# osmr/pytorchcv

Measured on AMD Instinct MI355X. Metric: images/sec @224x224 (resnet50 bs=256/GPU), higher is better.
Workload: dtype bf16; 1 GPU; resnet50_bs256; per_gpu_batch=256, global_batch=256, input=fp32 NCHW 224x224 resident in HBM, parallelism=batch-sharded replicas x1, launcher_choice=timed at capture on this GPU

## Files before the change

include/pcv_amd.h:

```cpp
#ifndef PCV_AMD_H
#define PCV_AMD_H

#include <stddef.h>
#include <stdint.h>

#ifdef __cplusplus
extern "C" {
#endif

#define PCV_ABI_VERSION 5

typedef struct pcv_ctx pcv_ctx;

typedef enum pcv_status {
    PCV_OK = 0,
    PCV_ERR_INVALID = -1,
    PCV_ERR_HIP = -2,
    PCV_ERR_NO_DEVICE = -3,
    PCV_ERR_TOO_LARGE = -4
} pcv_status;

typedef enum pcv_dtype { PCV_F32 = 0, PCV_BF16 = 1, PCV_F16 = 2 } pcv_dtype;

typedef enum pcv_act {
    PCV_ACT_NONE = 0, PCV_ACT_RELU = 1, PCV_ACT_RELU6 = 2, PCV_ACT_SIGMOID = 3,
    PCV_ACT_SWISH = 4, PCV_ACT_HSIGMOID = 5, PCV_ACT_HSWISH = 6
} pcv_act;

typedef struct pcv_conv_desc {
    int32_t struct_size;
    int32_t N, H, W;
    int32_t Cin, Cout;
    int32_t kh, kw;
    int32_t stride_h, stride_w;
    int32_t pad_t, pad_l, pad_b, pad_r;
    int32_t dil_h, dil_w;
    int32_t groups;
    int32_t act;
    int32_t post_act;
    int32_t has_residual;
    int32_t dtype;
    int32_t out_dtype;
    int32_t x_cpitch;
    int32_t x_wpitch;
    int32_t y_cpitch;
} pcv_conv_desc;

int pcv_abi_version(void);
size_t pcv_conv_desc_size(void);
int pcv_create(pcv_ctx** out, int device);
int pcv_destroy(pcv_ctx* ctx);
const char* pcv_last_error(const pcv_ctx* ctx);
int pcv_set_tuning(pcv_ctx* ctx, const char* key, int value);

int pcv_fp16_guard_begin(pcv_ctx* ctx, unsigned* slot, void* stream);
int pcv_fp16_guard_end(pcv_ctx* ctx, const unsigned* slot, float* y, long count, void* stream);
int pcv_fp16_overflow_count(pcv_ctx* ctx, unsigned* count, void* stream);

int pcv_nchw_to_nhwc(pcv_ctx* ctx, const float* x, void* y, int N, int C, int H, int W,
                     int cpitch, int wpitch, int dtype, void* stream);
int pcv_nhwc_to_nchw(pcv_ctx* ctx, const void* x, float* y, int N, int C, int H, int W, int cpitch, int dtype,
                     void* stream);

int pcv_preprocess_u8(pcv_ctx* ctx, const unsigned char* x, void* y, int N, int Hs, int Ws, int C, int top, int left,
                      int H, int W, int wpitch, const float* mean, const float* inv_std, int dtype, void* stream);

int pcv_conv_packed_bytes(const pcv_conv_desc* d, size_t* bytes);
int pcv_conv_pack(pcv_ctx* ctx, const pcv_conv_desc* d, const float* w, void* packed, void* stream);
int pcv_dwconv_packed_bytes(const pcv_conv_desc* d, size_t* bytes);
int pcv_dwconv_pack(pcv_ctx* ctx, const pcv_conv_desc* d, const float* w, void* packed, void* stream);
int pcv_bn_fold(pcv_ctx* ctx, int C, const float* gamma, const float* beta, const float* mean, const float* var,
                float eps, const float* conv_bias, float* scale, float* shift, void* stream);

int pcv_conv2d_fused(pcv_ctx* ctx, const pcv_conv_desc* d, const void* x, const void* packed,
                     const float* scale, const float* shift, const void* residual, void* y, void* stream);

int pcv_conv2d_gated_fused(pcv_ctx* ctx, const pcv_conv_desc* d, const void* x, const void* packed, const float* scale,
                           const float* shift, const float* gate, const void* residual, void* y, void* stream);
int pcv_fc_f32(pcv_ctx* ctx, const float* in, const float* w, const float* b, float* out, int N, int K, int J, int act,
               void* stream);
int pcv_conv2d_maxpool_supported(const pcv_conv_desc* d, int k, int s, int p, int ceil_mode);
int pcv_conv2d_maxpool_fused(pcv_ctx* ctx, const pcv_conv_desc* d, const void* x, const void* packed, const float* scale,
                             const float* shift, void* y, int k, int s, int p, int ceil_mode, void* stream);

int pcv_conv2d_nchw_stem_supported(const pcv_conv_desc* d, int pool);
int pcv_conv2d_nchw_stem_fused(pcv_ctx* ctx, const pcv_conv_desc* d, const float* x_nchw, const void* packed, const float* scale,
                               const float* shift, void* y, int pool, void* stream);
int pcv_dwconv2d_fused(pcv_ctx* ctx, const pcv_conv_desc* d, const void* x, const void* packed,
                       const float* scale, const float* shift, const void* residual, void* y, void* stream);
int pcv_maxpool2d(pcv_ctx* ctx, const void* x, void* y, int N, int H, int W, int C, int k, int s, int p,
                  int ceil_mode, int dtype, void* stream);
int pcv_channel_slice(pcv_ctx* ctx, const void* x, void* y, long rows, int C, int offset, int x_cpitch, int y_cpitch,
                      int dtype, void* stream);
int pcv_channel_interleave2(pcv_ctx* ctx, const void* a, const void* b, void* y, long rows, int Ch, int a_cpitch,
                            int b_cpitch, int y_cpitch, int dtype, void* stream);
int pcv_channel_concat(pcv_ctx* ctx, const void* x, void* y, long rows, int C, int x_cpitch, int y_cpitch, int y_offset,
                       int dtype, void* stream);
// ... 58 lines not shown
```

pytorchcv_amd/_lib.py:

```python

__all__ = ['lib', 'ctx_for', 'check', 'ConvDesc', 'LIB_PATH', 'PcvError', 'PCV_ERR_TOO_LARGE']

import os
import ctypes
import threading

LIB_PATH = os.path.join(os.path.dirname(os.path.abspath(__file__)), "csrc", "libpcv_amd.so")
PCV_ERR_TOO_LARGE = -4

_c = ctypes
_VP = ctypes.c_void_p
_I = ctypes.c_int


class PcvError(RuntimeError):
    def __init__(self, code, msg):
        super(PcvError, self).__init__("pcv_amd error {}: {}".format(code, msg))
        self.code = code


PCV_ABI_VERSION = 5


class ConvDesc(ctypes.Structure):
    _fields_ = [(n, ctypes.c_int32) for n in (
        "struct_size", "N", "H", "W", "Cin", "Cout", "kh", "kw", "stride_h", "stride_w", "pad_t", "pad_l", "pad_b", "pad_r",
        "dil_h", "dil_w", "groups", "act", "post_act", "has_residual", "dtype", "out_dtype", "x_cpitch", "x_wpitch",
        "y_cpitch")]


    def __init__(self, *args, **kw):
        super(ConvDesc, self).__init__(*args, **kw)
        self.struct_size = ctypes.sizeof(ConvDesc)


_SIGS = {
    "pcv_abi_version": (_I, []),
    "pcv_conv_desc_size": (ctypes.c_size_t, []),
    "pcv_create": (_I, [ctypes.POINTER(_VP), _I]),
    "pcv_destroy": (_I, [_VP]),
    "pcv_last_error": (ctypes.c_char_p, [_VP]),
    "pcv_set_tuning": (_I, [_VP, ctypes.c_char_p, _I]),
    "pcv_fp16_guard_begin": (_I, [_VP, _VP, _VP]),
    "pcv_fp16_guard_end": (_I, [_VP, _VP, _VP, ctypes.c_long, _VP]),
    "pcv_fp16_overflow_count": (_I, [_VP, ctypes.POINTER(ctypes.c_uint), _VP]),
    "pcv_rccl_available": (_I, []),
    "pcv_rccl_broadcast": (_I, [_VP, _VP, ctypes.POINTER(_VP), ctypes.POINTER(ctypes.c_size_t), _I, _I, _VP]),
    "pcv_rccl_allgather": (_I, [_VP, _VP, _VP, _VP, ctypes.c_size_t, _VP]),
    "pcv_nchw_to_nhwc": (_I, [_VP, _VP, _VP, _I, _I, _I, _I, _I, _I, _I, _VP]),
    "pcv_nhwc_to_nchw": (_I, [_VP, _VP, _VP, _I, _I, _I, _I, _I, _I, _VP]),
    "pcv_preprocess_u8": (_I, [_VP, _VP, _VP, _I, _I, _I, _I, _I, _I, _I, _I, _I, _VP, _VP, _I, _VP]),
    "pcv_conv_packed_bytes": (_I, [ctypes.POINTER(ConvDesc), ctypes.POINTER(ctypes.c_size_t)]),
    "pcv_conv_pack": (_I, [_VP, ctypes.POINTER(ConvDesc), _VP, _VP, _VP]),
    "pcv_dwconv_packed_bytes": (_I, [ctypes.POINTER(ConvDesc), ctypes.POINTER(ctypes.c_size_t)]),
    "pcv_dwconv_pack": (_I, [_VP, ctypes.POINTER(ConvDesc), _VP, _VP, _VP]),
    "pcv_bn_fold": (_I, [_VP, _I, _VP, _VP, _VP, _VP, ctypes.c_float, _VP, _VP, _VP, _VP]),
    "pcv_conv2d_fused": (_I, [_VP, ctypes.POINTER(ConvDesc), _VP, _VP, _VP, _VP, _VP, _VP, _VP]),
    "pcv_dwconv2d_fused": (_I, [_VP, ctypes.POINTER(ConvDesc), _VP, _VP, _VP, _VP, _VP, _VP, _VP]),
    "pcv_maxpool2d": (_I, [_VP, _VP, _VP, _I, _I, _I, _I, _I, _I, _I, _I, _I, _VP]),
    "pcv_channel_slice": (_I, [_VP, _VP, _VP, ctypes.c_long, _I, _I, _I, _I, _I, _VP]),
    "pcv_channel_interleave2": (_I, [_VP, _VP, _VP, _VP, ctypes.c_long, _I, _I, _I, _I, _I, _VP]),
    "pcv_channel_concat": (_I, [_VP, _VP, _VP, ctypes.c_long, _I, _I, _I, _I, _I, _VP]),
    "pcv_interpolate": (_I, [_VP, _VP, _VP, _I, _I, _I, _I, _I, _I, _I, _I, _I, _VP]),
    "pcv_avgpool2d": (_I, [_VP, _VP, _VP, _I, _I, _I, _I, _I, _I, _I, _I, _VP]),
    "pcv_global_avgpool": (_I, [_VP, _VP, _VP, _I, _I, _I, _I, _I, _VP]),
    "pcv_gemm_bias": (_I, [_VP, _VP, _VP, _VP, _VP, _I, _I, _I, _I, _I, _VP]),
    "pcv_se_squeeze": (_I, [_VP, _VP, _VP, _I, _I, _I, _I, _VP]),
    "pcv_se_excite": (_I, [_VP, _VP, _VP, _VP, _VP, _VP, _VP, _VP, _I, _I, _I, _I, _I, _VP]),
    "pcv_conv2d_gated_fused": (_I, [_VP, ctypes.POINTER(ConvDesc), _VP, _VP, _VP, _VP, _VP, _VP, _VP, _VP]),
    "pcv_fc_f32": (_I, [_VP, _VP, _VP, _VP, _VP, _I, _I, _I, _I, _VP]),
    "pcv_conv2d_maxpool_supported": (_I, [ctypes.POINTER(ConvDesc), _I, _I, _I, _I]),
    "pcv_conv2d_maxpool_fused": (_I, [_VP, ctypes.POINTER(ConvDesc), _VP, _VP, _VP, _VP, _VP, _I, _I, _I, _I, _VP]),
    "pcv_conv2d_nchw_stem_supported": (_I, [ctypes.POINTER(ConvDesc), _I]),
    "pcv_conv2d_nchw_stem_fused": (_I, [_VP, ctypes.POINTER(ConvDesc), _VP, _VP, _VP, _VP, _VP, _I, _VP]),
    "pcv_conv1x1_pair_supported": (_I, [ctypes.POINTER(ConvDesc), ctypes.POINTER(ConvDesc)]),
    "pcv_conv1x1_pair_fused": (_I, [_VP, ctypes.POINTER(ConvDesc), ctypes.POINTER(ConvDesc), _VP, _VP, _VP, _VP, _VP, _VP, _VP,
                                    _VP, _VP, _VP, _VP]),
    "pcv_conv1x1_pair_gated_supported": (_I, [ctypes.POINTER(ConvDesc), ctypes.POINTER(ConvDesc)]),
    "pcv_conv1x1_pair_gated_fused": (_I, [_VP, ctypes.POINTER(ConvDesc), ctypes.POINTER(ConvDesc), _VP, _VP, _VP, _VP, _VP, _VP, _VP,
                                          _VP, _VP, _VP, _VP, _VP]),
    "pcv_conv1x1_pair_idconv_supported": (_I, [ctypes.POINTER(ConvDesc), ctypes.POINTER(ConvDesc), ctypes.POINTER(ConvDesc)]),
# ... 65 lines not shown
```

pytorchcv_amd/csrc/d3q_conv.hpp:

```cpp
#pragma once
#include <type_traits>
#include "pcv_common.hpp"
#include "igemm_conv.hpp"

struct D3Params {
    const void* x;
    const void* w;
    const void* res;
    void* y;
    const float* scale;
    const float* shift;
    uint32_t x_bytes, w_bytes, y_bytes, res_bytes;
    int M;
    int Cout, Ypitch;
    int H, W, Cin, HW;
    FastDiv div_hw, div_w;
    int nk;
    int slices;
    int Kpad;
    int act, post_act;
    int nChTiles, nTiles;
    uint32_t* dbg;
    int stride, Hin, Win;
    uint32_t* ovf;
    int tailN;
    int dbgflags;
};

#ifdef PCV_DBG_FLAGS
#define D3_DBG(bits) ((p.dbgflags & (bits)) != 0)
#else
#define D3_DBG(bits) false
#endif
#ifdef D3X3_STAMPS
#define D3_STAMP(slot)                                                                                     \
    do {                                                                                                   \
        const int q__ = s - 4;                                                                             \
        if (q__ >= -1 && q__ < 27) {                                                                       \
            const int sel__ = (q__ + 9) % 9;                                                               \
            int l__ = -1;                                                                                  \
            if (q__ >= 0 && (slot) == sel__) l__ = 2 * q__ + 1;                                            \
            else if (q__ >= 0 && sel__ > 0 && (slot) == sel__ - 1) l__ = 2 * q__;                          \
            else if ((slot) == 8 && (q__ + 1) % 9 == 0 && q__ + 1 < 27) l__ = 2 * (q__ + 1);               \
            if (l__ >= 0) {                                                                                \
                const uint64_t t__ = __builtin_amdgcn_s_memtime();                                         \
                const int v__ = __builtin_amdgcn_readfirstlane((int)(uint32_t)t__);                        \
                const int i__ = __builtin_amdgcn_readfirstlane(l__);                                       \
                asm volatile("s_mov_b32 m0, %2\n\tv_writelane_b32 %0, %1, m0" : "+v"(stamps) : "s"(v__), "s"(i__) : "m0"); \
            }                                                                                              \
        }                                                                                                  \
    } while (0)
#else
#define D3_STAMP(slot) do { } while (0)
#endif

template <int WC, int WP, int CBW, int PBW, int KS, bool ONE = false> struct D3Cfg {
    static constexpr int NLOAD = 4;
    static constexpr int THREADS = 64 * (8 + NLOAD);
    static constexpr int BM = 16 * CBW * WC;
    static constexpr int BP = 16 * PBW * WP;
    static constexpr int NPA = BM / 8;
    static constexpr int WLW = NPA / NLOAD;
    static constexpr int BROWS = (BP + 2 + 7) / 8 * 8;
    static constexpr int NPB = BROWS / 8;
    static constexpr int XLW = (NPB + NLOAD - 1) / NLOAD;
    static constexpr int NB0 = (XLW + 1) / 2, NB1 = XLW / 2;
    static constexpr int ASZ = BM * 128;
    static constexpr int BSZ = NPB * 1024;
    static constexpr int NSA = 3;
    static constexpr int NSB = ONE ? 3 : 2;
    static constexpr int ZOFF = (NSA * ASZ + NSB * BSZ + 2047) / 2048 * 2048;
    static constexpr int DUMP = ZOFF + 2048;
    static constexpr int LDS = DUMP + 1024;
    static_assert(WC * WP == 8, "eight compute waves");
    static_assert(KS == 1 || KS == 2, "one or two K-halves per section");
    static_assert(NPA % NLOAD == 0 && CBW % 2 == 0, "weight pieces split evenly over the loaders; channel pairs per wave");
    static_assert(LDS <= 160 * 1024, "three weight tiles + two activation tiles must fit the LDS");
    static_assert(XLW <= 20, "row masks of the activation pieces are packed 3 bits each, ten per register, two registers");
};
// ... 285 lines not shown
            for (int j = 0; j < PBW; ++j) {
                lds_cptr bj = bp;
                if constexpr (Q != 1) {
                    const uint32_t t = (uint32_t)__builtin_amdgcn_sbfe((int)(Q == 0 ? hm0 : hm2), j, 1);
                    bj = (lds_cptr)(size_t)((t & (zsel - (uint32_t)(j * 2048))) | (~t & (uint32_t)(size_t)bp));
                }
                b[u][j] = *reinterpret_cast<lds_fptr>(bj + j * 2048);
            }
        }
    };
    auto mfmas = [&]() __attribute__((always_inline)) {
        __builtin_amdgcn_s_setprio(1);
#pragma unroll
        for (int u = 0; u < KS; ++u)
#pragma unroll
            for (int j = 0; j < PBW; ++j)
#pragma unroll
                for (int i = 0; i < CBW; ++i) acc[i][j] = Mma<DT>::run(a[u][i], b[u][j], acc[i][j]);
        __builtin_amdgcn_s_setprio(0);
    };
    auto reads_done = [&]() __attribute__((always_inline)) { __builtin_amdgcn_s_waitcnt(0xC07F); };

    const ActClamp act = make_act(p.act), pact = make_act(p.post_act);
    const bool has_res = p.res != nullptr;
    f32x4 es0[CBW / 2], es1[CBW / 2], eh0[CBW / 2], eh1[CBW / 2];
    auto ep_prefetch = [&](int t) __attribute__((always_inline)) {
        const int chTile = t % p.nChTiles;
#pragma unroll
        for (int ip = 0; ip < CBW / 2; ++ip) {
            const int ch0 = chTile * BM + wc * 16 * CBW + 32 * ip + 8 * fq;
            const int chl = ch0 < p.Cout ? ch0 : 0;
            es0[ip] = *reinterpret_cast<const f32x4*>(p.scale + chl); es1[ip] = *reinterpret_cast<const f32x4*>(p.scale + chl + 4);
            eh0[ip] = *reinterpret_cast<const f32x4*>(p.shift + chl); eh1[ip] = *reinterpret_cast<const f32x4*>(p.shift + chl + 4);
        }
    };
    auto epilogue = [&](int t) __attribute__((always_inline)) {
        if (D3_DBG(2)) return;
        const int chTile = t % p.nChTiles;
        const int tileP0 = (t / p.nChTiles) * BP;
        const int mBase = tileP0 + wp * 16 * PBW + fr;
        F16Guard<DT> guard;
#pragma unroll
        for (int ip = 0; ip < CBW / 2; ++ip) {
            const int ch0 = chTile * BM + wc * 16 * CBW + 32 * ip + 8 * fq;
            const bool chok = ch0 < p.Cout;
            const f32x4 s0 = es0[ip], s1 = es1[ip], h0 = eh0[ip], h1 = eh1[ip];
            u32x4 rr[PBW];
#pragma unroll
            for (int j = 0; j < PBW; ++j) rr[j] = (u32x4){0u, 0u, 0u, 0u};
            if (has_res) {
#pragma unroll
                for (int j = 0; j < PBW; ++j) {
                    const int m = mBase + 16 * j;
                    const uint32_t roff = (chok && m < p.M) ? (uint32_t)(((size_t)m * p.Cout + ch0) * 2) : 0x80000000u;
                    rr[j] = __builtin_amdgcn_raw_buffer_load_b128(rrsrc, roff, 0, 0);
                }
            }
#pragma unroll
            for (int j = 0; j < PBW; ++j) {
                const int m = mBase + 16 * j;
                float v[8];
#pragma unroll
                for (int e = 0; e < 4; ++e) {
                    v[e] = acc[2 * ip][j][e] * s0[e] + h0[e];
                    v[4 + e] = acc[2 * ip + 1][j][e] * s1[e] + h1[e];
                }
                clampn<8>(v, act);
#pragma unroll
                for (int e = 0; e < 4; ++e) {
                    float lo, hi;
                    unpack2<DT>(rr[j][e], lo, hi);
                    v[2 * e] += lo;
                    v[2 * e + 1] += hi;
                }
                clampn<8>(v, pact);
                guard.see(v);
                u32x4 o;
#pragma unroll
                for (int e = 0; e < 4; ++e) o[e] = pack2<DT>(v[2 * e], v[2 * e + 1]);
                const bool ok = chok && m < p.M && !D3_DBG(1);
                const uint32_t boff = ok ? (uint32_t)(((size_t)m * p.Ypitch + ch0) * 2) : 0x80000000u;
                __builtin_amdgcn_raw_buffer_store_b128(o, yrsrc, boff, 0, 0);
            }
        }
        guard.commit(p.ovf);
    };

    zero_acc();
    if constexpr (!ONE) setup_masks(T.tile0);
    d3q_sync();

    int sa = 0, sb = 0, k = 0, cur_tile = T.tile0, ep_tile = T.tile0;
    bool ep = false;
#ifdef D3X3_STAMPS
    int stamps = 0;
#endif
    auto kstep = [&](int s, auto Qc) __attribute__((always_inline)) -> bool {
        constexpr int Q = decltype(Qc)::value;
        if constexpr (GRP == 1) {
            if (s > 0) mfmas();
        }
        if constexpr (ONE || Q == 0) {
            if (ep) {
                epilogue(ep_tile);
                zero_acc();
                if constexpr (!ONE) {
                    if (!D3_DBG(8)) {
// ... 95 lines not shown
```

pytorchcv_amd/csrc/igemm_conv.hpp:

```cpp
#pragma once
#include "pcv_common.hpp"

#define IGEMM_MAX_TAPS 16

struct IgemmParams {
    const void* x;
    const void* w;
    const uint32_t* ktab;
    const void* res;
    void* y;
    const float* scale;
    const float* shift;
    uint32_t x_bytes;
    uint32_t w_bytes;
    uint32_t y_bytes;
    int M;
    int Cout;
    int Cout_total;
    int Ypitch;
    int cout_blk;
    int cin_blk;
    int wrows_blk;
    FastDiv div_howo, div_wo;
    int HoWo, Wo;
    int H, W, Wpitch, Cpitch;
    int sh, sw, pt, pl;
    int nR, nQ;
    int dy[IGEMM_MAX_TAPS];
    int dx[IGEMM_MAX_TAPS];
    int nk;
    int Kpad;
    int act, post_act;
    int nPixTiles, nChTiles;
    int ngb;
    int nTiles;
    int Cin;
    int ksteps_per_tap;
    int korder;
    int wstat;
    const float* gate;
    uint32_t* ovf;
};

template <int DT> struct Mma;
template <> struct Mma<PCV_BF16> {
    typedef s16x8 frag;
    static __device__ __forceinline__ f32x4 run(const frag& a, const frag& b, f32x4 c) {
        return __builtin_amdgcn_mfma_f32_16x16x32_bf16(a, b, c, 0, 0, 0);
    }
};
template <> struct Mma<PCV_F16> {
    typedef f16x8 frag;
    static __device__ __forceinline__ f32x4 run(const frag& a, const frag& b, f32x4 c) {
        return __builtin_amdgcn_mfma_f32_16x16x32_f16(a, b, c, 0, 0, 0);
    }
};
template <> struct Mma<PCV_F32> {
    typedef f32x4 frag;
    static __device__ __forceinline__ f32x4 run(const frag& a, const frag& b, f32x4 c) {
        c = __builtin_amdgcn_mfma_f32_16x16x4f32(a[0], b[0], c, 0, 0, 0);
        c = __builtin_amdgcn_mfma_f32_16x16x4f32(a[1], b[1], c, 0, 0, 0);
        c = __builtin_amdgcn_mfma_f32_16x16x4f32(a[2], b[2], c, 0, 0, 0);
        c = __builtin_amdgcn_mfma_f32_16x16x4f32(a[3], b[3], c, 0, 0, 0);
        return c;
    }
};

template <int DT, int OT, int CB, int PB, int WC, int WP, bool RAGGED, int KHW>
__global__ __launch_bounds__(64 * WC * WP, 2) void igemm_conv_kernel(const IgemmParams p) {
#if defined(__HIP_DEVICE_COMPILE__)
    constexpr int NW = WC * WP;
    constexpr int BM = 16 * CB * WC;
    constexpr int BP = 16 * PB * WP;
    constexpr int ES = Elem<DT>::BYTES;
    constexpr int CE = 16 / ES;
    constexpr int STAGE = (BM + BP) * 128;
    constexpr int WLOADS = BM / (8 * NW);
    constexpr int XLOADS = BP / (8 * NW);
    constexpr int NPAIR = CB / 2;
    static_assert(BM % (8 * NW) == 0 && BP % (8 * NW) == 0, "tile rows must split evenly over the waves");
    typedef typename Mma<DT>::frag frag;

    extern __shared__ __attribute__((aligned(16))) char smem[];

    const int tid = threadIdx.x;
    const int lane = tid & 63;
    const int wave = __builtin_amdgcn_readfirstlane(tid >> 6);
    const int wc = wave / WP, wp = wave % WP;

    const int perXcd = (p.nTiles + 7) >> 3;
    const int xcd = blockIdx.x & 7;
    const int tstride = gridDim.x >> 3;
    int tile = xcd * perXcd + (int)(blockIdx.x >> 3);
    const int tend = min(p.nTiles, (xcd + 1) * perXcd);
    if (tile >= tend) return;

    const int lrow = lane >> 3;
    const int cs = (lane & 7) ^ lrow;
    const int nR = KHW == 9 ? 3 : (KHW == 1 ? 1 : p.nR);
    const int nQ = KHW == 9 ? 3 : (KHW == 1 ? 1 : p.nQ);
    const int fr = lane & 15, fq = lane >> 4;

    struct TileState {
        int rbase[XLOADS];
        uint32_t rmask[XLOADS];
        uint32_t woff[WLOADS];
        int chTile, gb, tileP0;
    };
    auto setup = [&](int t, TileState& S) {
        S.chTile = t % p.nChTiles;
        const int t2 = t / p.nChTiles;
        S.gb = t2 % p.ngb;
        S.tileP0 = (t2 / p.ngb) * BP;
#pragma unroll
        for (int i = 0; i < XLOADS; ++i) {
            const int m = S.tileP0 + 8 * (i * NW + wave) + lrow;
            uint32_t mask = 0;
            int base = 0;
            if (m < p.M) {
                const uint32_t n = fastdiv((uint32_t)m, p.div_howo);
                const uint32_t rem = (uint32_t)m - n * (uint32_t)p.HoWo;
// ... 64 lines not shown
                q = (uint32_t)(k - 3 * grp);
                r = (uint32_t)(grp / p.ksteps_per_tap);
                cslice = grp - (int)r * p.ksteps_per_tap;
            }
            const int c0 = cslice * (8 * CE) + cs * CE;
            koff = ((int)r * p.Wpitch + (int)q) * p.Cpitch + c0;
        } else {
            const u32x2 kd = kd_next;
            const int c0 = (int)(kd[0] & 0xFFFFu);
            r = (kd[0] >> 16) & 15u;
            q = (kd[0] >> 20) & 15u;
            const int dy = (int)(short)(kd[1] & 0xFFFFu), dx = (int)(short)(kd[1] >> 16);
            koff = (dy * p.Wpitch + dx) * p.Cpitch + c0;
        }
#pragma unroll
        for (int i = 0; i < XLOADS; ++i) {
            char* dst = sbase + (BM + 8 * (i * NW + wave)) * 128;
            const bool ok = chunk_ok && (((S.rmask[i] >> r) & (S.rmask[i] >> (16 + q)) & 1u) != 0);
            const uint32_t voff = ok ? (uint32_t)((S.rbase[i] + koff) * ES) : 0x80000000u;
            __builtin_amdgcn_raw_ptr_buffer_load_lds(xrsrc, PCV_LDS(dst), 16, voff, 0, 0, 0);
        }
    };

    const int swz0 = ((fq) ^ (fr & 7)) << 4;
    const int swz1 = ((fq + 4) ^ (fr & 7)) << 4;
    const int wfrag = (wc * 16 * CB + fr) * 128;
    const int xfrag = (BM + wp * 16 * PB + fr) * 128;

    f32x4 acc[CB][PB];
    auto zero_acc = [&]() {
#pragma unroll
        for (int i = 0; i < CB; ++i)
#pragma unroll
            for (int j = 0; j < PB; ++j) acc[i][j] = (f32x4){0.f, 0.f, 0.f, 0.f};
    };
    auto compute = [&](int buf) {
        const char* sbase = smem + buf * STAGE;
        const char* wsbase = wstat ? smem : sbase;
#pragma unroll
        for (int kk = 0; kk < 2; ++kk) {
            const int swz = kk == 0 ? swz0 : swz1;
            frag a[CB], b[PB];
#pragma unroll
            for (int i = 0; i < CB; ++i) a[i] = *reinterpret_cast<const frag*>(wsbase + wfrag + i * 2048 + swz);
#pragma unroll
            for (int j = 0; j < PB; ++j) b[j] = *reinterpret_cast<const frag*>(sbase + xfrag + j * 2048 + swz);
#pragma unroll
            for (int i = 0; i < CB; ++i)
#pragma unroll
                for (int j = 0; j < PB; ++j) acc[i][j] = Mma<DT>::run(a[i], b[j], acc[i][j]);
        }
    };

    const ActClamp act = make_act(p.act), pact = make_act(p.post_act);
    const bool bounded = act_bounded(p.post_act) || (p.post_act == PCV_ACT_NONE && p.res == nullptr && p.gate == nullptr && act_bounded(p.act));
    zero_acc();
    TileState cur, nxt;
    setup(tile, cur);
    const int nk = p.nk;
    if constexpr (KHW == 0) kd_next = load_kdesc(0);
    stage(cur, 0, 0);
    if constexpr (KHW == 0) kd_next = load_kdesc(nk > 1 ? 1 : 0);
    int buf = 0;

    while (true) {
        for (int k = 0; k + 1 < nk; ++k) {
            asm volatile("s_waitcnt vmcnt(0)" ::: "memory");
            __syncthreads();
            stage(cur, k + 1, buf ^ 1);
            if constexpr (KHW == 0) kd_next = load_kdesc(k + 2 < nk ? k + 2 : 0);
            compute(buf);
            buf ^= 1;
        }
        const int ntile = tile + tstride;
        const bool has_next = ntile < tend;
        if (has_next) setup(ntile, nxt);
        asm volatile("s_waitcnt vmcnt(0)" ::: "memory");
        __syncthreads();

        const int chBlk = cur.chTile * BM + wc * 16 * CB;
        const int chGlob0 = cur.gb * p.cout_blk;
        const int mBase = cur.tileP0 + wp * 16 * PB + fr;
        float sc[NPAIR][8], sf[NPAIR][8];
        u32x4 rres[NPAIR][PB];
        f32x4 rres32[DT == PCV_F32 ? NPAIR : 1][DT == PCV_F32 ? PB : 1][2];
        if constexpr (!RAGGED) {
#pragma unroll
            for (int ip = 0; ip < NPAIR; ++ip) {
                const int ch0 = chBlk + 32 * ip + 8 * fq;
                const int chg = chGlob0 + ch0;
                f32x4 s0 = {1.f, 1.f, 1.f, 1.f}, s1 = s0, h0 = {0.f, 0.f, 0.f, 0.f}, h1 = h0;
                if (ch0 < p.Cout) {
                    if (p.scale != nullptr) {
                        s0 = *reinterpret_cast<const f32x4*>(p.scale + chg);
                        s1 = *reinterpret_cast<const f32x4*>(p.scale + chg + 4);
                    }
                    if (p.shift != nullptr) {
                        h0 = *reinterpret_cast<const f32x4*>(p.shift + chg);
                        h1 = *reinterpret_cast<const f32x4*>(p.shift + chg + 4);
                    }
                }
#pragma unroll
                for (int e = 0; e < 4; ++e) { sc[ip][e] = s0[e]; sc[ip][4 + e] = s1[e]; sf[ip][e] = h0[e]; sf[ip][4 + e] = h1[e]; }
#pragma unroll
                for (int j = 0; j < PB; ++j) {
                    const int m = mBase + 16 * j;
                    const bool ok = p.res != nullptr && ch0 < p.Cout && m < p.M;
                    const size_t eoff = (size_t)m * p.Cout_total + chg;
                    if constexpr (DT == PCV_F32) {
                        rres32[ip][j][0] = ok ? *reinterpret_cast<const f32x4*>(reinterpret_cast<const float*>(p.res) + eoff)
                                              : (f32x4){0.f, 0.f, 0.f, 0.f};
                        rres32[ip][j][1] = ok ? *reinterpret_cast<const f32x4*>(reinterpret_cast<const float*>(p.res) + eoff + 4)
                                              : (f32x4){0.f, 0.f, 0.f, 0.f};
                    } else {
                        rres[ip][j] = ok ? *reinterpret_cast<const u32x4*>(reinterpret_cast<const uint16_t*>(p.res) + eoff)
                                         : (u32x4){0u, 0u, 0u, 0u};
                    }
                }
            }
        }

        if (has_next) stage(nxt, 0, buf ^ 1);
        if constexpr (KHW == 0) kd_next = load_kdesc(nk > 1 ? 1 : 0);

        compute(buf);

        F16Guard<OT> guard;
#pragma unroll
        for (int ip = 0; ip < NPAIR; ++ip) {
            const int ch0 = chBlk + 32 * ip + 8 * fq;
            if constexpr (!FAST_STORE) {
                if (ch0 >= p.Cout) continue;
            }
            const int chg = chGlob0 + ch0;
            if constexpr (RAGGED) {
#pragma unroll
                for (int e = 0; e < 8; ++e) {
                    const bool ok = ch0 + e < p.Cout;
                    sc[ip][e] = ok ? (p.scale ? p.scale[chg + e] : 1.f) : 0.f;
                    sf[ip][e] = ok ? (p.shift ? p.shift[chg + e] : 0.f) : 0.f;
                }
            }
#pragma unroll
            for (int j = 0; j < PB; ++j) {
                const int m = mBase + 16 * j;
                if constexpr (!FAST_STORE) {
                    if (m >= p.M) continue;
                }
                const size_t eoff = (size_t)m * p.Cout_total + chg;
                const size_t yoff = (size_t)m * p.Ypitch + chg;
                float v[8];
#pragma unroll
                for (int e = 0; e < 4; ++e) {
                    v[e] = acc[2 * ip][j][e] * sc[ip][e] + sf[ip][e];
                    v[4 + e] = acc[2 * ip + 1][j][e] * sc[ip][4 + e] + sf[ip][4 + e];
                }
                apply_act8(v, act);
                if (p.gate != nullptr) {
#pragma clang fp contract(off)
                    const uint32_t n = fastdiv((uint32_t)(m < p.M ? m : 0), p.div_howo);
                    const float* gp = p.gate + (size_t)n * p.Cout_total + chg;
// ... 58 lines not shown
```

pytorchcv_amd/csrc/pcv_api.hip:

```cpp
#include <hip/hip_runtime.h>
#include <string>
#include <vector>
#include <cstring>
#include <algorithm>
#include <cstdio>
#include <cstdlib>
#include <dlfcn.h>
#include "pcv_common.hpp"
#include "igemm_inst.hpp"
#include "d3q_inst.hpp"
#include "d3w_inst.hpp"
#include "d3c_conv.hpp"
#include "d3k_conv.hpp"
#include "d3i_conv.hpp"
#include "d1i_conv.hpp"
#include "p1r_conv.hpp"
#include "stem_conv.hpp"
#include "pair1x1.hpp"
#include "wpair1x1.hpp"
#include "gconv3x3.hpp"
#include "gconv3x3r.hpp"
#include "mbconv.hpp"
#include "mbw_inst.hpp"
#include "mbr_inst.hpp"
// ... 22 lines not shown
D3WT_SHAPES(D3WT_DECLARE, PCV_BF16)
D3WT_SHAPES(D3WT_DECLARE, PCV_F16)
extern template __global__ void d3c_kernel<PCV_BF16>(const D3Params);
extern template __global__ void d3c_kernel<PCV_F16>(const D3Params);
extern template __global__ void d3k_kernel<PCV_BF16>(const D3Params);
extern template __global__ void d3k_kernel<PCV_F16>(const D3Params);
extern template __global__ void d3i_kernel<PCV_BF16, 256>(const D3Params);
extern template __global__ void d3i_kernel<PCV_F16, 256>(const D3Params);
extern template __global__ void d3i_kernel<PCV_BF16, 512>(const D3Params);
extern template __global__ void d3i_kernel<PCV_F16, 512>(const D3Params);
extern template __global__ void d1i_kernel<PCV_BF16, 1024>(const D3Params);
extern template __global__ void d1i_kernel<PCV_F16, 1024>(const D3Params);
extern template __global__ void d1i_kernel<PCV_BF16, 2048>(const D3Params);
extern template __global__ void d1i_kernel<PCV_F16, 2048>(const D3Params);
#define P1R_DECLARE(CW, CIN)                                                       \
    extern template __global__ void p1r_kernel<PCV_BF16, CW, CIN>(const D3Params); \
    extern template __global__ void p1r_kernel<PCV_F16, CW, CIN>(const D3Params);
P1R_DECLARE(64, 256)
P1R_DECLARE(32, 512)
P1R_DECLARE(32, 256)

enum TileCfg { TILE_C32 = 0, TILE_C64 = 1, TILE_C128 = 2, TILE_C256 = 3, TILE_C64S = 4, TILE_C128S = 5, TILE_COUNT = 6 };

struct pcv_ctx {
    int device = 0;
    std::string err;
    int num_cu = 256;
    int persist_mode = 1;
    int force_tile = -1;
    int use_wstat = 1;
    int use_mbr = 1;
    int use_mbr_xl = 1;
    int use_mbw = 1;
    int use_gconvr = 1;
    int use_d1x1 = -1;
    int use_head = 1;
    int use_stem32 = 1;
    int use_d3x3 = -1;
    unsigned long long dbg_ptr = 0;
    int use_p1r = -1;
    int use_d3k = -1;
    int use_d3i = -1;
    int use_d1i = -1;
    int use_d3c = -1;
    int use_d3w = -1;
    int dbg_flags = 0;
    int dw_flags = 0;
    int dw_th = 0;
    int max_blocks = 0;
    int pair_pb = 2;
    int persist_max_nk = 4;
    uint32_t* ovf = nullptr;
    int igemm_bpc[3][2][TILE_COUNT][3] = {};
    int gconv_bpc[3] = {2, 2, 2};
    int stem_bpc[2] = {1, 1};
    int pair_bpc[2] = {1, 1};
    int pair_idc_bpc = 1;
    int wpair_bpc[4] = {1, 1, 1, 1};
};

static thread_local std::string g_create_err;

static int fail(pcv_ctx* ctx, int code, const std::string& msg) {
    if (ctx) ctx->err = msg; else g_create_err = msg;
    return code;
}
#define HIP_TRY(ctx, expr)                                                                          \
    do {                                                                                            \
        hipError_t e__ = (expr);                                                                    \
        if (e__ != hipSuccess)                                                                      \
            return fail(ctx, PCV_ERR_HIP, std::string(#expr) + ": " + hipGetErrorString(e__));      \
    } while (0)

struct DeviceGuard {
    int prev = -1;
    bool switched = false;
    explicit DeviceGuard(int want) {
        if (hipGetDevice(&prev) == hipSuccess && prev != want) switched = hipSetDevice(want) == hipSuccess;
    }
    ~DeviceGuard() {
        if (switched) (void)hipSetDevice(prev);
    }
};

static inline int round_up(int v, int m) { return (v + m - 1) / m * m; }
static inline long long block_slots(const pcv_ctx* ctx, int per_cu) {
    const long long n = (long long)ctx->num_cu * per_cu;
    return (ctx->max_blocks > 0 && ctx->max_blocks < n) ? ctx->max_blocks : n;
}
static inline int esize(int dt) { return dt == PCV_F32 ? 4 : 2; }
static inline bool dtype_ok(int dt) { return dt == PCV_F32 || dt == PCV_BF16 || dt == PCV_F16; }
static inline bool aligned16(const void* p) { return (reinterpret_cast<uintptr_t>(p) & 15u) == 0; }
static inline bool in_window(unsigned long long bytes) { return bytes < 0x80000000ull; }
static int too_large(pcv_ctx* ctx, const char* fn, const char* what) {
    return fail(ctx, PCV_ERR_TOO_LARGE, std::string(fn) + ": " + what + " exceeds the 2 GiB window of one launch; split the batch");
}
static const char* const kTensorTooLarge = "tensor exceeds the 2 GiB window";

struct Kernel { const void* fn; int threads, lds, BM, BP; };
template <class F> static Kernel kernel_of(F* fn, int threads, int lds, int BM = 0, int BP = 0) {
    return Kernel{reinterpret_cast<const void*>(fn), threads, lds, BM, BP};
}
template <class Params> static int launch(pcv_ctx* ctx, const Kernel& k, unsigned grid, hipStream_t stream, Params& q) {
    void* args[] = {&q};
    HIP_TRY(ctx, hipLaunchKernel(k.fn, dim3(grid), dim3((unsigned)k.threads), args, (size_t)k.lds, stream));
    return PCV_OK;
}
static int blocks_per_cu(pcv_ctx* ctx, const Kernel& k, int* nb) {
    HIP_TRY(ctx, hipOccupancyMaxActiveBlocksPerMultiprocessor(nb, k.fn, k.threads, k.lds));
    if (*nb < 1) *nb = 1;
    return PCV_OK;
}

struct ConvPlan {
    bool stem = false;
    bool conv3 = false;
    int ES = 2, CE = 8;
    bool pair = false;
    int Ho = 0, Wo = 0;
    int ngb = 1;
    int Cg_in = 0, Cg_out = 0;
    int cin_blk = 0, cout_blk = 0;
    int nR = 1, nQ = 1;
    int dy[IGEMM_MAX_TAPS], dx[IGEMM_MAX_TAPS];
    int nchunks = 0, nk = 0, Kpad = 0;
    int wrows = 0;
    size_t ktab_bytes = 0, w_bytes = 0, total_bytes = 0;
    int gconv_kt = 5;
    bool gconv = false;
    bool d3i = false;
    bool d1i = false;
    size_t d3i_off = 0;
    size_t gconv_off = 0;
    std::vector<uint32_t> ktab;
    std::vector<uint32_t> ksrc;
};

static const char* const kStaleDesc = "pcv_conv_desc.struct_size does not match this library (stale binding: compare pcv_conv_desc_size() / PCV_ABI_VERSION)";
static inline bool desc_stale(const pcv_conv_desc& d) { return d.struct_size != (int32_t)sizeof(pcv_conv_desc); }

static const char* plan_conv(const pcv_conv_desc& d, ConvPlan& P, bool tables) {
    if (desc_stale(d)) return kStaleDesc;
    if (!dtype_ok(d.dtype) || !dtype_ok(d.out_dtype)) return "unknown dtype";
    if (d.out_dtype != d.dtype && d.out_dtype != PCV_F32) return "out_dtype must equal dtype or be fp32";
    if (d.Cin <= 0 || d.Cout <= 0 || d.kh <= 0 || d.kw <= 0 || d.groups <= 0) return "non-positive conv dimension";
    constexpr int kMaxChannels = 1 << 20, kMaxExtent = 1 << 24, kMaxGeom = 1 << 12;
    if (d.Cin > kMaxChannels || d.Cout > kMaxChannels || d.groups > kMaxChannels) return "channel count out of range (> 2^20)";
    if (d.N < 0 || d.H < 0 || d.W < 0 || d.N > kMaxExtent || d.H > kMaxExtent || d.W > kMaxExtent) return "N / H / W out of range (> 2^24)";
    if (d.stride_h > kMaxGeom || d.stride_w > kMaxGeom || d.dil_h > kMaxGeom || d.dil_w > kMaxGeom) return "stride / dilation out of range";
    if (d.pad_t < 0 || d.pad_l < 0 || d.pad_b < 0 || d.pad_r < 0 || d.pad_t > kMaxGeom || d.pad_l > kMaxGeom || d.pad_b > kMaxGeom ||
        d.pad_r > kMaxGeom)
        return "padding out of range";
    if (d.x_cpitch < 0 || d.x_cpitch > 8 * kMaxChannels || d.x_wpitch < 0 || d.x_wpitch > 2 * kMaxExtent || d.y_cpitch < 0 ||
        d.y_cpitch > 8 * kMaxChannels)
        return "pitch out of range";
    if (d.kh >= IGEMM_MAX_TAPS || d.kw >= IGEMM_MAX_TAPS) return "kernel size > 15 unsupported";
    if (d.stride_h <= 0 || d.stride_w <= 0 || d.dil_h <= 0 || d.dil_w <= 0) return "non-positive stride/dilation";
    if (d.Cin % d.groups || d.Cout % d.groups) return "channels not divisible by groups";
    P.ES = esize(d.dtype);
    P.CE = 16 / P.ES;
    P.Cg_in = d.Cin / d.groups;
    P.Cg_out = d.Cout / d.groups;
    const int cpitch = d.x_cpitch > 0 ? d.x_cpitch : d.Cin;
    if (cpitch < d.Cin) return "x_cpitch < Cin";
    P.pair = (d.groups == 1 && cpitch == 4 && P.ES == 2);
    if (!P.pair && cpitch % P.CE != 0) return "x_cpitch must be a multiple of 16 bytes (or 4 for a padded 16-bit stem)";

    int gpb = 1;
    if (d.groups > 1) {
        while (gpb < d.groups && ((gpb * P.Cg_out) % 8 != 0 || (gpb * P.Cg_in) % P.CE != 0 || gpb * P.Cg_out < 32)) ++gpb;
        while (gpb < d.groups && d.groups % gpb != 0) ++gpb;
        if (d.groups % gpb != 0 || (gpb * P.Cg_out) % 8 != 0 || (gpb * P.Cg_in) % P.CE != 0)
            return "unsupported group shape (channels per group block not 16-byte aligned)";
    }
    P.ngb = d.groups / gpb;
    P.cin_blk = gpb * P.Cg_in;
    P.cout_blk = gpb * P.Cg_out;
    if (d.groups == 1) P.cin_blk = d.Cin;
    P.wrows = round_up(P.cout_blk, 32);

    P.conv3 = d.groups == 1 && d.kh == 3 && d.kw == 3 && d.stride_h == 1 && d.stride_w == 1 && d.dil_h == 1 && d.dil_w == 1 &&
              d.pad_t == 1 && d.pad_l == 1 && d.pad_b == 1 && d.pad_r == 1 && d.Cin % (8 * P.CE) == 0 && cpitch == d.Cin &&
              (d.x_wpitch <= 0 || d.x_wpitch == d.W) && d.out_dtype == d.dtype && d.Cout % 8 == 0;

    P.stem = P.pair && d.stride_h == 2 && d.stride_w == 2 && d.dil_h == 1 && d.Cout <= 64 && d.Cout % 8 == 0 && d.kh <= 7 &&
             d.kw + (d.pad_l & 1) <= 8 && d.out_dtype == d.dtype;

    if (P.pair) {
        if (d.stride_w % 2 != 0 || d.dil_w != 1) return "padded 4-channel stem needs even stride_w and dilation 1";
        const int wp = d.x_wpitch > 0 ? d.x_wpitch : d.W;
        if (wp % 2 != 0) return "padded 4-channel stem needs an even x_wpitch";
        const int dxs = -(d.pad_l & 1);
        P.nQ = (d.kw - dxs + 1) / 2;
        P.nR = d.kh;
        if (P.nQ >= IGEMM_MAX_TAPS) return "stem too wide";
        for (int r = 0; r < P.nR; ++r) P.dy[r] = r * d.dil_h;
        for (int q = 0; q < P.nQ; ++q) P.dx[q] = dxs + 2 * q;
        P.nchunks = P.nR * P.nQ;
    } else {
        P.nR = d.kh;
        P.nQ = d.kw;
        for (int r = 0; r < P.nR; ++r) P.dy[r] = r * d.dil_h;
        for (int q = 0; q < P.nQ; ++q) P.dx[q] = q * d.dil_w;
        const int cchunks = (P.cin_blk + P.CE - 1) / P.CE;
        if (d.groups == 1 && cchunks * P.CE > cpitch) return "x_cpitch too small for the channel chunks";
        P.nchunks = P.nR * P.nQ * cchunks;
    }
    for (int i = P.nR; i < IGEMM_MAX_TAPS; ++i) P.dy[i] = 0;
    for (int i = P.nQ; i < IGEMM_MAX_TAPS; ++i) P.dx[i] = 0;
    P.nk = (P.nchunks + 7) / 8;
    P.Kpad = P.nk * 8 * P.CE;
    P.ktab_bytes = (size_t)round_up(P.nk * 8 * 8, 256);
    P.w_bytes = (size_t)P.ngb * P.wrows * P.Kpad * P.ES;
    P.total_bytes = P.ktab_bytes + P.w_bytes;
    static const bool gconv_on = !(std::getenv("PCV_AMD_GCONV") && std::atoi(std::getenv("PCV_AMD_GCONV")) == 0);
    P.gconv = gconv_on && d.groups > 1 && d.kh == 3 && d.kw == 3 && d.stride_h == d.stride_w && (d.stride_h == 1 || d.stride_h == 2) &&
              d.dil_h == 1 && d.dil_w == 1 &&
              d.pad_t == 1 && d.pad_l == 1 && d.pad_b == 1 && d.pad_r == 1 && d.Cin == d.Cout && d.Cin % 64 == 0 && P.ES == 2 &&
              (P.Cg_in == 4 || P.Cg_in == 8 || P.Cg_in == 16 || P.Cg_in == 32) && d.out_dtype == d.dtype;
    if (P.gconv) {
        P.gconv_kt = P.Cg_in == 32 ? 9 : 5;
        P.gconv_off = (P.total_bytes + 15) / 16 * 16;
        P.total_bytes = P.gconv_off + (size_t)(d.Cin / 16) * P.gconv_kt * 16 * 32 * P.ES;
    }
    P.d3i = P.conv3 && P.ES == 2 && (d.Cin == 256 || d.Cin == 512) && d.Cout % D3ICfg::CW == 0 && d.out_dtype == d.dtype &&
            P.wrows >= d.Cout && P.Kpad == 9 * d.Cin;
    if (P.d3i) {
        P.d3i_off = (P.total_bytes + 15) / 16 * 16;
        P.total_bytes = P.d3i_off + (size_t)(d.Cout / D3ICfg::CW) * (d.Cin == 256 ? D3ICfgT<256>::WBYTES : D3ICfgT<512>::WBYTES);
    }
    P.d1i = !P.conv3 && !P.pair && !P.stem && P.ES == 2 && d.kh == 1 && d.kw == 1 && d.groups == 1 && d.stride_h == 1 && d.stride_w == 1 &&
            d.pad_t == 0 && d.pad_l == 0 && d.pad_b == 0 && d.pad_r == 0 && (d.Cin == 1024 || d.Cin == 2048) &&
            d.Cout % 64 == 0 && d.out_dtype == d.dtype && P.wrows >= d.Cout && P.Kpad == d.Cin && P.ngb == 1;
    if (P.d1i) {
        P.d3i_off = (P.total_bytes + 15) / 16 * 16;
        P.total_bytes = P.d3i_off + (size_t)(d.Cout / 64) * (size_t)(d.Cin / 32) * 4096;
    }
    if (P.w_bytes >= 0x80000000ull) return "packed weights exceed 2 GiB";

    if (P.stem) {
        P.ktab_bytes = 0;
        P.w_bytes = (size_t)d.kh * 64 * 32 * P.ES;
        P.total_bytes = P.w_bytes;
    }
    P.Ho = (d.H + d.pad_t + d.pad_b - d.dil_h * (d.kh - 1) - 1) / d.stride_h + 1;
    P.Wo = (d.W + d.pad_l + d.pad_r - d.dil_w * (d.kw - 1) - 1) / d.stride_w + 1;

    if (tables) {
        P.ktab.assign((size_t)P.nk * 8 * 2, 0);
        P.ksrc.assign((size_t)P.Kpad, 0xFFFFFFFFu);
        const int khkw = d.kh * d.kw;
        (void)khkw;
        int j = 0;
        auto put = [&](int c0, int r, int q, int dyv, int dxv) {
            P.ktab[2 * j] = (uint32_t)c0 | ((uint32_t)r << 16) | ((uint32_t)q << 20);
            P.ktab[2 * j + 1] = ((uint32_t)dyv & 0xFFFFu) | (((uint32_t)dxv & 0xFFFFu) << 16);
            ++j;
        };
        if (P.pair) {
            for (int r = 0; r < P.nR; ++r)
                for (int q = 0; q < P.nQ; ++q) {
                    for (int e = 0; e < 8; ++e) {
                        const int pix = e >> 2, c = e & 3;
                        const int tap = P.dx[q] + pix;
                        if (tap >= 0 && tap < d.kw && c < d.Cin)
                            P.ksrc[(size_t)j * 8 + e] = (uint32_t)c | ((uint32_t)(r * d.kw + tap) << 16);
                    }
                    put(0, r, q, P.dy[r], P.dx[q]);
                }
        } else if (P.conv3) {
            const int slices = d.Cin / (8 * P.CE);
            for (int r = 0; r < 3; ++r)
                for (int cs = 0; cs < slices; ++cs)
                    for (int q = 0; q < 3; ++q)
                        for (int cc = cs * 8; cc < cs * 8 + 8; ++cc) {
                            for (int e = 0; e < P.CE; ++e)
                                P.ksrc[(size_t)j * P.CE + e] = (uint32_t)(cc * P.CE + e) | ((uint32_t)(r * 3 + q) << 16);
                            put(cc * P.CE, r, q, P.dy[r], P.dx[q]);
                        }
        } else {
            const int cchunks = (P.cin_blk + P.CE - 1) / P.CE;
            for (int r = 0; r < P.nR; ++r)
                for (int q = 0; q < P.nQ; ++q)
                    for (int cc = 0; cc < cchunks; ++cc) {
                        for (int e = 0; e < P.CE; ++e) {
                            const int c = cc * P.CE + e;
                            if (c < P.cin_blk)
                                P.ksrc[(size_t)j * P.CE + e] = (uint32_t)c | ((uint32_t)(r * d.kw + q) << 16);
                        }
                        put(cc * P.CE, r, q, P.dy[r], P.dx[q]);
                    }
        }
        while (j < P.nk * 8) put(0, 15, 0, 0, 0);
    }
    return nullptr;
}

struct TileInfo { int BM, BP, threads, lds; };
static const TileInfo kTiles[TILE_COUNT] = {
    {32, 256, 256, 2 * (32 + 256) * 128},
    {64, 256, 256, 2 * (64 + 256) * 128},
    {128, 128, 256, 2 * (128 + 128) * 128},
    {256, 64, 256, 2 * (256 + 64) * 128},
    {64, 128, 256, 2 * (64 + 128) * 128},
    {128, 64, 256, 2 * (128 + 64) * 128},
};
typedef void (*igemm_fn)(const IgemmParams);

template <int DT, int KHW> static igemm_fn igemm_for_tile(int tile) {
    switch (tile) {
        case TILE_C32: return igemm_conv_kernel<DT, DT, 2, 4, 1, 4, false, KHW>;
        case TILE_C64: return igemm_conv_kernel<DT, DT, 4, 4, 1, 4, false, KHW>;
        case TILE_C128: return igemm_conv_kernel<DT, DT, 4, 4, 2, 2, false, KHW>;
        case TILE_C256: return igemm_conv_kernel<DT, DT, 4, 4, 4, 1, false, KHW>;
        case TILE_C64S: if constexpr (KHW == 1) return igemm_conv_kernel<DT, DT, 4, 2, 1, 4, false, 1>; else return nullptr;
        case TILE_C128S: if constexpr (KHW == 1) return igemm_conv_kernel<DT, DT, 4, 2, 2, 2, false, 1>; else return nullptr;
        default: return nullptr;
    }
}
template <int DT> static igemm_fn igemm_for_taps(int tile, int khw) {
    if (khw == 1) return igemm_for_tile<DT, 1>(tile);
    if (khw == 9) return igemm_for_tile<DT, 9>(tile);
    return igemm_for_tile<DT, 0>(tile);
}
static igemm_fn igemm_fn_for(int dt, int ot, bool ragged, int tile, int khw) {
    if (!ragged && ot == dt) {
        if (dt == PCV_BF16) return igemm_for_taps<PCV_BF16>(tile, khw);
        if (dt == PCV_F16) return igemm_for_taps<PCV_F16>(tile, khw);
        return igemm_for_taps<PCV_F32>(tile, khw);
    }
    if (tile != TILE_C128) return nullptr;
    if (ot == PCV_F32) {
        if (dt == PCV_BF16) return igemm_conv_kernel<PCV_BF16, PCV_F32, 4, 4, 2, 2, true, 0>;
        if (dt == PCV_F16) return igemm_conv_kernel<PCV_F16, PCV_F32, 4, 4, 2, 2, true, 0>;
        return igemm_conv_kernel<PCV_F32, PCV_F32, 4, 4, 2, 2, true, 0>;
    }
    if (dt == PCV_BF16) return igemm_conv_kernel<PCV_BF16, PCV_BF16, 4, 4, 2, 2, true, 0>;
    if (dt == PCV_F16) return igemm_conv_kernel<PCV_F16, PCV_F16, 4, 4, 2, 2, true, 0>;
    return nullptr;
}

static Kernel igemm_kernel(int dt, int ot, bool ragged, int tile, int khw) {
    const TileInfo& T = kTiles[tile];
    return kernel_of(igemm_fn_for(dt, ot, ragged, tile, khw), T.threads, T.lds, T.BM, T.BP);
}
static inline int khw_slot(int khw) { return khw == 1 ? 1 : (khw == 9 ? 2 : 0); }

static inline int gconv_slot(int W) { return W + 1 <= 16 ? 0 : (W + 1 <= 32 ? 1 : 2); }
static Kernel gconv_kernel(int dt, int slot) {
    const bool bf = dt == PCV_BF16;
    if (slot == 0) return kernel_of(bf ? gconv3x3_kernel<PCV_BF16, 16> : gconv3x3_kernel<PCV_F16, 16>, 256, GConvCfg<16>::LDS);
    if (slot == 1) return kernel_of(bf ? gconv3x3_kernel<PCV_BF16, 32> : gconv3x3_kernel<PCV_F16, 32>, 256, GConvCfg<32>::LDS);
    return kernel_of(bf ? gconv3x3_kernel<PCV_BF16, 64> : gconv3x3_kernel<PCV_F16, 64>, 256, GConvCfg<64>::LDS);
}
static const int kGconvRMaxLds = 160 * 1024;
static Kernel gconvr_kernel(int dt, int stride, int kt, int lds = kGconvRMaxLds) {
    const bool bf = dt == PCV_BF16;
    if (stride == 2) {
        if (kt == 9) return kernel_of(bf ? gconv3x3r_kernel<PCV_BF16, 2, 9> : gconv3x3r_kernel<PCV_F16, 2, 9>, 256, lds);
        return kernel_of(bf ? gconv3x3r_kernel<PCV_BF16, 2, 5> : gconv3x3r_kernel<PCV_F16, 2, 5>, 256, lds);
    }
    return kernel_of(bf ? gconv3x3r_kernel<PCV_BF16, 1, 9> : gconv3x3r_kernel<PCV_F16, 1, 9>, 256, lds);
}
struct GConvRPlan { int R, XH, xl, win; };
static bool plan_gconvr(int stride, int H, int W, int Ho, int Wo, GConvRPlan& g) {
    if (stride == 2 && ((H | W) & 1)) return false;
    if (Wo > 64 || Ho <= 0) return false;
    for (int R = 64 / Wo; R >= 1; --R) {
        const int win = stride == 2 ? (2 * R + 1) * W + 2 : (R + 2) * W + 2;
        const int XH = stride == 2 ? ((win + 1) / 2 + 7) / 8 * 8 : 0;
        const int rows = ((stride == 2 ? 2 * XH : win) + 31) / 32 * 32;
        const int lds = 2 * rows * 128;
        if (lds * 2 <= kGconvRMaxLds || (R == 1 && lds <= kGconvRMaxLds)) {
            g.R = R; g.XH = XH; g.xl = rows / 32; g.win = win;
            return true;
        }
    }
    return false;
}
template <class Cfg, class F> static Kernel tile_kernel(F* fn, int threads) { return kernel_of(fn, threads, Cfg::LDS, Cfg::BM, Cfg::BP); }
#define D3Q_ROW(DT, WC, WP, CBW, PBW, KS)                                                                   \
    {tile_kernel<D3Cfg<WC, WP, CBW, PBW, KS>>(d3q_kernel<PCV_BF16, WC, WP, CBW, PBW, KS>, 768),             \
     tile_kernel<D3Cfg<WC, WP, CBW, PBW, KS>>(d3q_kernel<PCV_F16, WC, WP, CBW, PBW, KS>, 768)},
static const Kernel kD3[][2] = {D3Q_SHAPES(D3Q_ROW, 0)};
static const int kD3Count = (int)(sizeof(kD3) / sizeof(kD3[0]));
#define D3Q1_ROW(DT, WC, WP, CBW, PBW, KS)                                                                  \
    {tile_kernel<D3Cfg<WC, WP, CBW, PBW, KS, true>>(d3q_kernel<PCV_BF16, WC, WP, CBW, PBW, KS, true>, 768), \
     tile_kernel<D3Cfg<WC, WP, CBW, PBW, KS, true>>(d3q_kernel<PCV_F16, WC, WP, CBW, PBW, KS, true>, 768)},
static const Kernel kD1[][2] = {D3Q1_SHAPES(D3Q1_ROW, 0)};
static const int kD1Count = (int)(sizeof(kD1) / sizeof(kD1[0]));
#define D3W_ROW(DT, WC, WP, CBW, PBW, KS, NSA)                                                              \
    {tile_kernel<D3WCfg<WC, WP, CBW, PBW, KS, NSA>>(d3w_kernel<PCV_BF16, WC, WP, CBW, PBW, KS, NSA>, 512),  \
     tile_kernel<D3WCfg<WC, WP, CBW, PBW, KS, NSA>>(d3w_kernel<PCV_F16, WC, WP, CBW, PBW, KS, NSA>, 512)},
#define D3WT_ROW(DT, WC, WP, CBW, PBW, KS, NSA, TRIM)                                                                   \
    {tile_kernel<D3WCfg<WC, WP, CBW, PBW, KS, NSA, TRIM>>(d3w_kernel<PCV_BF16, WC, WP, CBW, PBW, KS, NSA, TRIM>, 512),  \
     tile_kernel<D3WCfg<WC, WP, CBW, PBW, KS, NSA, TRIM>>(d3w_kernel<PCV_F16, WC, WP, CBW, PBW, KS, NSA, TRIM>, 512)},
static const Kernel kD3W[][2] = {D3W_SHAPES(D3W_ROW, 0) D3WT_SHAPES(D3WT_ROW, 0)};
// ... 30 lines not shown
static int pick_d3w(long long M, int Cout, long long slots) {
    const int shape = Cout % 256 == 0 ? 1 : (Cout % 128 == 0 ? 2 : -1);
    if (shape < 0) return -1;
    const long long tiles = (long long)(Cout / kD3W[shape][0].BM) * ((M + kD3W[shape][0].BP - 1) / kD3W[shape][0].BP);
    return tiles * 4 >= slots * 3 ? shape : -1;
}

static const int kStemLds = 7 * 64 * 64 + 2 * 768 * 16 + 3 * 2 * 64 * 16;
enum StemForm { STEM_PLAIN = 0, STEM_POOLED = 1, STEM_NARROW = 2 };
#define STEM_ROWS(DT)                                                                                                          \
    {{kernel_of(stem_conv_kernel<DT, false>, 256, kStemLds), kernel_of(stem_conv_kernel<DT, true>, 256, kStemLds),             \
      kernel_of(stem_conv_kernel<DT, false, false, 2>, 256, kStemLds)},                                                        \
     {kernel_of(stem_conv_kernel<DT, false, true>, 256, kStemLds + kStemStageBytes),                                           \
      kernel_of(stem_conv_kernel<DT, true, true>, 256, kStemLds + kStemStageBytes),                                            \
      kernel_of(stem_conv_kernel<DT, false, true, 2>, 256, kStemLds + kStemStageBytes)}}
static const Kernel kStem[2][2][3] = {STEM_ROWS(PCV_BF16), STEM_ROWS(PCV_F16)};

static int pair_lds(int pb, bool idc = false) { return (idc ? 6 : 3) * 16 * pb * 64 * 2 + 16 * 1024 * pb + (idc ? 4096 : 0); }
enum PairForm { PAIR_PB4 = 0, PAIR_PB2 = 1, PAIR_GATED = 2, PAIR_IDCONV = 3 };
#define PAIR_ROW(DT)                                                                                                          \
    {kernel_of(pair1x1_kernel<DT, 4>, 256, pair_lds(4)), kernel_of(pair1x1_kernel<DT, 2>, 256, pair_lds(2)),                  \
     kernel_of(pair1x1_kernel<DT, 2, false, true>, 256, pair_lds(2)), kernel_of(pair1x1_kernel<DT, 2, true>, 256, pair_lds(2, true))}
static const Kernel kPair[2][4] = {PAIR_ROW(PCV_BF16), PAIR_ROW(PCV_F16)};
static int g_wpair_mask = 3;
static int g_mbw_wide = 1;
struct WPairLaunch { Kernel k; int tileP; bool gate_in_lds; };
template <int CM, int C1> static WPairLaunch wpair_launch_for(int dt, bool gated) {
    typedef WPairCfg<CM, C1> G;
    const bool bf = dt == PCV_BF16;
    const int lds = gated ? G::LDS_GATED : G::LDS;
    const Kernel k = gated ? kernel_of(bf ? wpair1x1_kernel<PCV_BF16, CM, C1, true> : wpair1x1_kernel<PCV_F16, CM, C1, true>, 64 * G::NW, lds)
                           : kernel_of(bf ? wpair1x1_kernel<PCV_BF16, CM, C1, false> : wpair1x1_kernel<PCV_F16, CM, C1, false>, 64 * G::NW, lds);
    return WPairLaunch{k, G::P, gated && G::GATE_LDS};
}
static WPairLaunch wpair_launch(int cfg, int dt, bool gated = false) {
    switch (cfg) {
        case 0: return wpair_launch_for<128, 512>(dt, gated);
        case 1: return wpair_launch_for<256, 1024>(dt, gated);
        case 2: return wpair_launch_for<128, 256>(dt, gated);
        default: return wpair_launch_for<256, 512>(dt, gated);
    }
}
static int wpair_cfg(int cm, int c1) {
    if (cm == 128 && c1 == 512) return 0;
    if (cm == 256 && c1 == 1024) return 1;
    if (cm == 128 && c1 == 256) return 2;
    if (cm == 256 && c1 == 512) return 3;
    return -1;
}
static bool plain_1x1(const pcv_conv_desc& d) {
    return d.kh == 1 && d.kw == 1 && d.stride_h == 1 && d.stride_w == 1 && d.pad_t == 0 && d.pad_l == 0 && d.pad_b == 0 &&
           d.pad_r == 0 && d.groups == 1 && d.dil_h == 1 && d.dil_w == 1 && d.out_dtype == d.dtype &&
           (d.x_cpitch == 0 || d.x_cpitch == d.Cin) && (d.x_wpitch == 0 || d.x_wpitch == d.W) &&
           (d.y_cpitch == 0 || d.y_cpitch == d.Cout);
}
static const char* pair_unsupported(const pcv_conv_desc& a, const pcv_conv_desc& b) {
    if (desc_stale(a) || desc_stale(b)) return kStaleDesc;
    if (!plain_1x1(a) || !plain_1x1(b)) return "both convolutions must be plain 1x1 stride 1";
    if (a.dtype != b.dtype || (a.dtype != PCV_BF16 && a.dtype != PCV_F16)) return "16-bit storage only";
    if (a.N != b.N || a.H != b.H || a.W != b.W || a.Cout != b.Cin) return "shapes do not chain";
    const bool narrow = a.Cin == 64 && a.Cout == 256 && b.Cout == 64;
    const bool wide = ((a.Cin == 128 && (g_wpair_mask & 1)) || (a.Cin == 256 && (g_wpair_mask & 2))) &&
                      wpair_cfg(a.Cin, a.Cout) >= 0 && b.Cout == a.Cin;
    if (!narrow && !wide) return "only 64 -> 256 -> 64, 128 -> 512|256 -> 128 and 256 -> 1024|512 -> 256 are instantiated";
    if (!a.has_residual || b.has_residual || b.post_act != PCV_ACT_NONE) return "first conv must carry the residual, second must not";
    if ((long)a.N * a.H * a.W * a.Cout * 2 >= (1L << 31)) return kTensorTooLarge;
    return nullptr;
}

typedef void (*mbconv_fn)(const MbParams);
template <int DT, int RT> static mbconv_fn mbconv_for(int stride, bool expand) {
    if (stride == 1) return expand ? mbconv_kernel<DT, 1, true, RT> : mbconv_kernel<DT, 1, false, RT>;
    return expand ? mbconv_kernel<DT, 2, true, RT> : mbconv_kernel<DT, 2, false, RT>;
}
static const int kMbMaxLds = 150 * 1024, kMbwMaxLds = 160 * 1024;
static Kernel mbconv_kernel(int dt, int stride, bool expand, int nrowt, int lds = kMbMaxLds) {
    if (dt == PCV_BF16) return kernel_of(nrowt <= 2 ? mbconv_for<PCV_BF16, 2>(stride, expand) : mbconv_for<PCV_BF16, 6>(stride, expand), 256, lds);
    return kernel_of(nrowt <= 2 ? mbconv_for<PCV_F16, 2>(stride, expand) : mbconv_for<PCV_F16, 6>(stride, expand), 256, lds);
}
struct MbwEntry { int dt, s, nrt, act, tw, ka, rb; mbconv_fn fn; };
#define MBW_ROW(DT, S, NRT, ACT, TW) {DT, S, NRT, ACT, TW, 1, 0, mbw_kernel<DT, S, NRT, ACT, TW>},
#define MBW2_ROW(DT, S, NRT, ACT, TW, KA) {DT, S, NRT, ACT, TW, KA, 0, mbw_kernel<DT, S, NRT, ACT, TW, KA>},
#define MBW3_ROW(DT, S, NRT, ACT, TW, KA, RB) {DT, S, NRT, ACT, TW, KA, RB, mbw_kernel<DT, S, NRT, ACT, TW, KA, RB>},
static const MbwEntry kMbw[] = {MBW_SHAPES(MBW_ROW, PCV_BF16) MBW_SHAPES(MBW_ROW, PCV_F16) MBW2_SHAPES(MBW2_ROW, PCV_BF16)
                                MBW2_SHAPES(MBW2_ROW, PCV_F16) MBW3_SHAPES(MBW3_ROW, PCV_BF16) MBW3_SHAPES(MBW3_ROW, PCV_F16)};
static const MbwEntry* pick_mbw(int dt, int stride, int nrt, int act, int tw, int ka, int rb) {
    if (act != PCV_ACT_RELU && act != PCV_ACT_RELU6) act = -1;
    for (const MbwEntry& e : kMbw)
        if (e.dt == dt && e.s == stride && e.nrt == nrt && e.act == act && e.tw == tw && e.ka == ka && e.rb == rb) return &e;
    return nullptr;
}
static Kernel mbw_kernel_of(const MbwEntry& e, int waves = 8, int lds = kMbwMaxLds) { return kernel_of(e.fn, 64 * waves, lds); }
struct MbrEntry { int dt, nrt, act, ro, s, ka; bool afl; int waves; bool wel, xl; mbconv_fn fn; };
#define MBR_ROW(DT, NRT, ACT, RO, S, KA, AFL, WV, WEL, XL) {DT, NRT, ACT, RO, S, KA, AFL, WV, WEL, XL, mbr_kernel<DT, NRT, ACT, RO, S, KA, AFL, WV, WEL, XL>},
static int mbr_entry_lds(const MbrEntry& e, int nChunks) {
    const int nr = e.s == 1 ? e.ro + 2 : 2 * e.ro + 1;
    return mbr_lds_layout(e.nrt, nChunks, e.ka, e.afl, e.wel, e.xl ? nr : 0, e.waves).total;
}
static const MbrEntry kMbr[] = {MBR_SHAPES(MBR_ROW, PCV_BF16) MBR_SHAPES(MBR_ROW, PCV_F16)};
static Kernel mbr_kernel_of(const MbrEntry& e, int lds = kMbwMaxLds) { return kernel_of(e.fn, 64 * e.waves, lds); }
static const MbrEntry* pick_mbr(const pcv_ctx* ctx, int dt, int nrt, int act, int stride, int ka, int nChunks) {
    if (act != PCV_ACT_RELU && act != PCV_ACT_RELU6) return nullptr;
    for (const MbrEntry& e : kMbr)
        if (e.dt == dt && e.nrt == nrt && e.act == act && e.s == stride && e.ka == ka &&
            mbr_entry_lds(e, nChunks) <= kMbwMaxLds && (!e.xl || ctx->use_mbr_xl))
            return &e;
    return nullptr;
}
static int mbw_waves(int stride, int nrt, int nChunks, int tw, int ka, int rb) {
    for (int nw = 8; nw >= 4; nw -= 2)
        if (mbw_lds_layout(stride, nrt, nChunks, nw, tw, ka, rb).total <= kMbwMaxLds) return nw;
    return 0;
}
static MbLds mbconv_plan(int stride, bool expand, int ka, int nChunks, int nRowT, int* nbufX) {
    MbLds two = mb_lds_layout(stride, expand, ka, nChunks, nRowT, 2);
    if (!expand || two.total <= 80 * 1024) { *nbufX = 2; return two; }
    MbLds one = mb_lds_layout(stride, expand, ka, nChunks, nRowT, 1);
    if (one.total <= 80 * 1024 || two.total > kMbMaxLds) { *nbufX = 1; return one; }
    *nbufX = 2;
    return two;
}

static int enable_kernel(pcv_ctx* ctx, const Kernel& k, int* bpc) {
    HIP_TRY(ctx, hipFuncSetAttribute(k.fn, hipFuncAttributeMaxDynamicSharedMemorySize, k.lds));
    return bpc ? blocks_per_cu(ctx, k, bpc) : PCV_OK;
}
static int enable_kernels(pcv_ctx* ctx) {
    int rc = PCV_OK;
    auto on = [&](const Kernel& k, int* bpc = nullptr) {
        if (rc == PCV_OK && k.fn != nullptr) rc = enable_kernel(ctx, k, bpc);
    };
    auto report = [&](const Kernel& k, int dt, int tile, int khw, int variant) {
        int nb = 0;
        if (rc == PCV_OK && k.fn != nullptr && std::getenv("PCV_AMD_DEBUG") && blocks_per_cu(ctx, k, &nb) == PCV_OK)
            std::fprintf(stderr, "[pcv] igemm dt=%d tile=%d khw=%d variant=%d: %d blocks/CU\n", dt, tile, khw, variant, nb);
    };
    static const int khws[3] = {0, 1, 9};
    for (int dt = 0; dt < 3; ++dt)
        for (int tile = 0; tile < TILE_COUNT; ++tile) {
            for (int ks = 0; ks < 3; ++ks) {
                const Kernel k = igemm_kernel(dt, dt, false, tile, khws[ks]);
                on(k, &ctx->igemm_bpc[dt][0][tile][ks]);
                report(k, dt, tile, khws[ks], 0);
            }
            const Kernel f32out = igemm_kernel(dt, PCV_F32, true, tile, 0), same = igemm_kernel(dt, dt, true, tile, 0);
            on(f32out);
            report(f32out, dt, tile, 0, 1);
            on(same, &ctx->igemm_bpc[dt][1][tile][0]);
            report(same, dt, tile, 0, 2);
        }
    for (const auto& T : kD3Tables)
        for (int i = 0; i < T.n; ++i)
            for (int t = 0; t < 2; ++t) on(T.rows[i][t]);
    for (int slot = 0; slot < 3; ++slot) {
        on(gconv_kernel(PCV_BF16, slot));
        on(gconv_kernel(PCV_F16, slot), &ctx->gconv_bpc[slot]);
    }
    for (int dt = PCV_BF16; dt <= PCV_F16; ++dt)
        for (int s = 1; s <= 2; ++s)
            for (int kt = 5; kt <= 9; kt += 4) on(gconvr_kernel(dt, s, kt));
    for (int t = 0; t < 2; ++t)
        for (int nchw = 0; nchw < 2; ++nchw)
            for (int form = 0; form < 3; ++form) on(kStem[t][nchw][form], (nchw == 0 && form == STEM_PLAIN) ? &ctx->stem_bpc[t] : nullptr);
    for (int form = 0; form < 4; ++form) {
        on(kPair[0][form]);
        on(kPair[1][form], form == PAIR_GATED ? nullptr : form == PAIR_IDCONV ? &ctx->pair_idc_bpc : &ctx->pair_bpc[form]);
    }
    for (int cfg = 0; cfg < 4; ++cfg)
        for (int gated = 0; gated < 2; ++gated) {
            on(wpair_launch(cfg, PCV_BF16, gated != 0).k);
            on(wpair_launch(cfg, PCV_F16, gated != 0).k, gated ? nullptr : &ctx->wpair_bpc[cfg]);
        }
    for (int dt = PCV_BF16; dt <= PCV_F16; ++dt)
        for (int s = 1; s <= 2; ++s)
            for (int e = 0; e < 2; ++e)
                for (int rt = 2; rt <= 6; rt += 4) on(mbconv_kernel(dt, s, e != 0, rt));
    for (const MbwEntry& e : kMbw) on(mbw_kernel_of(e));
    for (const MbrEntry& e : kMbr) on(mbr_kernel_of(e));
    return rc;
}
static bool mbw_shape(int Cin, int Cout, int stride, int H, int W, int* ka_out, int* nrt_out, int* rb_out = nullptr) {
    const int ka = (Cin + 31) / 32, nrt = Cout <= 32 ? 2 : (Cout <= 64 ? 4 : 6);
    if (ka_out) *ka_out = ka;
    if (nrt_out) *nrt_out = nrt;
    if (rb_out) *rb_out = nrt == 6 ? 2 : 0;
    if (H > 250 || W > 250 || Cout > 96) return false;
    if (nrt == 6) return g_mbw_wide != 0 && stride == 1 && (ka == 2 || ka == 3);
    return ka == 1 || (ka == 2 && stride == 1 && nrt == 4);
}
static const char* mbconv_unsupported(const pcv_conv_desc* de, const pcv_conv_desc& dd, const pcv_conv_desc& dp) {
    if ((de && desc_stale(*de)) || desc_stale(dd) || desc_stale(dp)) return kStaleDesc;
    if (dd.dtype != PCV_BF16 && dd.dtype != PCV_F16) return "16-bit storage only";
    if (dd.kh != 3 || dd.kw != 3 || dd.dil_h != 1 || dd.dil_w != 1 || dd.pad_t != 1 || dd.pad_l != 1 || dd.pad_b != 1 ||
        dd.pad_r != 1 || dd.stride_h != dd.stride_w || (dd.stride_h != 1 && dd.stride_h != 2) || dd.groups != dd.Cin ||
        dd.Cin != dd.Cout || dd.has_residual || dd.out_dtype != dd.dtype || (dd.x_cpitch != 0 && dd.x_cpitch != dd.Cin) ||
        (dd.x_wpitch != 0 && dd.x_wpitch != dd.W))
        return "depthwise stage must be 3x3, pad 1, stride 1 or 2, no residual";
// ... 221 lines not shown
    const RcclApi& R = rccl_api();
    if (!R.ok) return fail(ctx, PCV_ERR_INVALID, "pcv_rccl_allgather: no RCCL in this process (librccl.so.1 not found)");
    const int rc = R.allgather(send, recv, bytes_per_rank, kNcclUint8, comm, (hipStream_t)stream);
    if (rc != 0) return rccl_fail(ctx, "ncclAllGather", rc);
    return PCV_OK;
}

int pcv_fp16_overflow_count(pcv_ctx* ctx, unsigned* count, void* stream) {
    if (!ctx) return PCV_ERR_INVALID;
    DeviceGuard device_guard(ctx->device);
    if (!count) return fail(ctx, PCV_ERR_INVALID, "pcv_fp16_overflow_count: count is NULL");
    HIP_TRY(ctx, hipMemcpyAsync(count, ctx->ovf, sizeof(unsigned), hipMemcpyDeviceToHost, (hipStream_t)stream));
    HIP_TRY(ctx, hipStreamSynchronize((hipStream_t)stream));
    return PCV_OK;
}

int pcv_nchw_to_nhwc(pcv_ctx* ctx, const float* x, void* y, int N, int C, int H, int W, int cpitch, int wpitch,
                     int dtype, void* stream) {
    if (!ctx) return PCV_ERR_INVALID;
    DeviceGuard device_guard(ctx->device);
    if (!x || !y || N <= 0 || C <= 0 || H <= 0 || W <= 0 || cpitch < C || wpitch < W || !dtype_ok(dtype))
        return fail(ctx, PCV_ERR_INVALID, "pcv_nchw_to_nhwc: bad argument");
    if (!(cpitch == 4 || cpitch % 8 == 0) && !(dtype == PCV_F32 && cpitch % 4 == 0))
        return fail(ctx, PCV_ERR_INVALID, "pcv_nchw_to_nhwc: cpitch must be 4 or a multiple of 8");
    const long npix = (long)N * H * wpitch;
    dim3 grid((unsigned)((npix + 255) / 256), (unsigned)((cpitch + 7) / 8));
    hipStream_t s = (hipStream_t)stream;
    if (dtype == PCV_BF16) nchw_to_nhwc_kernel<PCV_BF16><<<grid, 256, 0, s>>>(x, y, N, C, H, W, cpitch, wpitch, ctx->ovf);
    else if (dtype == PCV_F16) nchw_to_nhwc_kernel<PCV_F16><<<grid, 256, 0, s>>>(x, y, N, C, H, W, cpitch, wpitch, ctx->ovf);
    else nchw_to_nhwc_kernel<PCV_F32><<<grid, 256, 0, s>>>(x, y, N, C, H, W, cpitch, wpitch, ctx->ovf);
    HIP_TRY(ctx, hipGetLastError());
    return PCV_OK;
}

int pcv_nhwc_to_nchw(pcv_ctx* ctx, const void* x, float* y, int N, int C, int H, int W, int cpitch, int dtype, void* stream) {
    if (!ctx) return PCV_ERR_INVALID;
    DeviceGuard device_guard(ctx->device);
    if (cpitch <= 0) cpitch = C;
    if (!x || !y || N <= 0 || C <= 0 || H <= 0 || W <= 0 || cpitch < C || !dtype_ok(dtype))
        return fail(ctx, PCV_ERR_INVALID, "pcv_nhwc_to_nchw: bad argument");
    const long total = (long)N * C * H * W;
    const unsigned grid = (unsigned)((total + 255) / 256);
    hipStream_t s = (hipStream_t)stream;
    if (dtype == PCV_BF16) nhwc_to_nchw_kernel<PCV_BF16><<<grid, 256, 0, s>>>(x, y, N, C, H, W, cpitch);
    else if (dtype == PCV_F16) nhwc_to_nchw_kernel<PCV_F16><<<grid, 256, 0, s>>>(x, y, N, C, H, W, cpitch);
    else nhwc_to_nchw_kernel<PCV_F32><<<grid, 256, 0, s>>>(x, y, N, C, H, W, cpitch);
    HIP_TRY(ctx, hipGetLastError());
    return PCV_OK;
}

int pcv_conv_packed_bytes(const pcv_conv_desc* d, size_t* bytes) {
    if (!d || !bytes) return PCV_ERR_INVALID;
    ConvPlan P;
    if (plan_conv(*d, P, false) != nullptr) return PCV_ERR_INVALID;
    *bytes = P.total_bytes;
    return PCV_OK;
}

int pcv_conv_pack(pcv_ctx* ctx, const pcv_conv_desc* d, const float* w, void* packed, void* stream) {
    if (!ctx) return PCV_ERR_INVALID;
    DeviceGuard device_guard(ctx->device);
    if (!d || !w || !packed) return fail(ctx, PCV_ERR_INVALID, "pcv_conv_pack: NULL argument");
    if (!aligned16(packed)) return fail(ctx, PCV_ERR_INVALID, "pcv_conv_pack: packed buffer must be 16-byte aligned");
    ConvPlan P;
    const char* why = plan_conv(*d, P, true);
    if (why) return fail(ctx, PCV_ERR_INVALID, std::string("pcv_conv_pack: ") + why);
    hipStream_t s = (hipStream_t)stream;
    if (P.stem) {
        const int total = d->kh * 64 * 32;
        if (d->dtype == PCV_BF16) pack_stem_kernel<PCV_BF16><<<(total + 255) / 256, 256, 0, s>>>(w, packed, d->Cout, d->Cin, d->kh, d->kw, d->pad_l & 1);
        else pack_stem_kernel<PCV_F16><<<(total + 255) / 256, 256, 0, s>>>(w, packed, d->Cout, d->Cin, d->kh, d->kw, d->pad_l & 1);
        HIP_TRY(ctx, hipGetLastError());
        return PCV_OK;
    }
    uint32_t* ksrc_dev = nullptr;
    HIP_TRY(ctx, hipStreamSynchronize(s));
    HIP_TRY(ctx, hipMalloc(reinterpret_cast<void**>(&ksrc_dev), P.ksrc.size() * sizeof(uint32_t)));
    hipError_t e = hipMemcpy(ksrc_dev, P.ksrc.data(), P.ksrc.size() * sizeof(uint32_t), hipMemcpyHostToDevice);
    if (e == hipSuccess) e = hipMemcpy(packed, P.ktab.data(), P.ktab.size() * sizeof(uint32_t), hipMemcpyHostToDevice);
    if (e != hipSuccess) {
        (void)hipFree(ksrc_dev);
        return fail(ctx, PCV_ERR_HIP, std::string("pcv_conv_pack: table upload: ") + hipGetErrorString(e));
    }
    PackParams pp;
    pp.w = w;
    pp.out = static_cast<char*>(packed) + P.ktab_bytes;
    pp.ksrc = ksrc_dev;
    pp.ngb = P.ngb;
    pp.wrows = P.wrows;
    pp.Kpad = P.Kpad;
    pp.cout_blk = P.cout_blk;
    pp.cin_blk = d->groups == 1 ? 0 : P.cin_blk;
    pp.Cg_in = P.Cg_in;
    pp.Cg_out = P.Cg_out;
    pp.khkw = d->kh * d->kw;
    const long total = (long)P.ngb * P.wrows * P.Kpad;
    const unsigned grid = (unsigned)((total + 255) / 256);
    if (d->dtype == PCV_BF16) pack_conv_kernel<PCV_BF16><<<grid, 256, 0, s>>>(pp);
    else if (d->dtype == PCV_F16) pack_conv_kernel<PCV_F16><<<grid, 256, 0, s>>>(pp);
    else pack_conv_kernel<PCV_F32><<<grid, 256, 0, s>>>(pp);
    if (P.gconv) {
        const long gtotal = (long)(d->Cin / 16) * P.gconv_kt * 16 * 32;
        const unsigned ggrid = (unsigned)((gtotal + 255) / 256);
        void* gout = static_cast<char*>(packed) + P.gconv_off;
        const bool bf = d->dtype == PCV_BF16;
        if (P.gconv_kt == 9) {
            if (bf) pack_gconv32_kernel<PCV_BF16><<<ggrid, 256, 0, s>>>(w, gout, d->Cin);
            else pack_gconv32_kernel<PCV_F16><<<ggrid, 256, 0, s>>>(w, gout, d->Cin);
        } else if (bf) pack_gconv_kernel<PCV_BF16><<<ggrid, 256, 0, s>>>(w, gout, d->Cin, P.Cg_in);
        else pack_gconv_kernel<PCV_F16><<<ggrid, 256, 0, s>>>(w, gout, d->Cin, P.Cg_in);
    }
    if (P.d3i || P.d1i) {
        const int total = (int)((P.total_bytes - P.d3i_off) / 16);
        pack_d3i_kernel<<<(unsigned)((total + 255) / 256), 256, 0, s>>>(reinterpret_cast<const u32x4*>(pp.out),
                                                                        reinterpret_cast<u32x4*>(static_cast<char*>(packed) + P.d3i_off), P.Kpad, total);
    }
    e = hipGetLastError();
    if (e == hipSuccess) e = hipStreamSynchronize(s);
    (void)hipFree(ksrc_dev);
    if (e != hipSuccess) return fail(ctx, PCV_ERR_HIP, std::string("pcv_conv_pack: ") + hipGetErrorString(e));
    return PCV_OK;
}

static const char* check_dw(const pcv_conv_desc& d) {
    if (desc_stale(d)) return kStaleDesc;
    if (!dtype_ok(d.dtype) || d.out_dtype != d.dtype) return "depthwise: out_dtype must equal dtype";
    if (d.groups != d.Cin || d.Cin != d.Cout) return "depthwise: needs groups == Cin == Cout";
    if (d.Cin % 8 != 0) return "depthwise: channels must be a multiple of 8";
    if (d.kh != d.kw || (d.kh != 3 && d.kh != 5)) return "depthwise: only 3x3 and 5x5";
    if (d.stride_h != d.stride_w || (d.stride_h != 1 && d.stride_h != 2)) return "depthwise: stride 1 or 2";
    if (d.dil_h != 1 || d.dil_w != 1) return "depthwise: dilation unsupported";
    if (d.x_cpitch > 0 && d.x_cpitch != d.Cin) return "depthwise: padded channel pitch unsupported";
    if (d.x_wpitch > 0 && d.x_wpitch != d.W) return "depthwise: padded row pitch unsupported";
    if (d.y_cpitch > 0 && d.y_cpitch != d.Cout) return "depthwise: y must be dense";
    return nullptr;
}

static size_t dw_taps_bytes(const pcv_conv_desc& d) { return (((size_t)d.kh * d.kw * d.Cin * esize(d.dtype)) + 15) & ~(size_t)15; }
static size_t dw_sparse_bytes(const pcv_conv_desc& d) {
    return (d.kh == 3 && d.dtype != PCV_F32) ? (size_t)((d.Cin + 31) / 32) * 6 * 1024 : 0;
}
int pcv_dwconv_packed_bytes(const pcv_conv_desc* d, size_t* bytes) {
    if (!d || !bytes || check_dw(*d)) return PCV_ERR_INVALID;
    *bytes = dw_taps_bytes(*d) + dw_sparse_bytes(*d);
    return PCV_OK;
}

int pcv_dwconv_pack(pcv_ctx* ctx, const pcv_conv_desc* d, const float* w, void* packed, void* stream) {
    if (!ctx) return PCV_ERR_INVALID;
    DeviceGuard device_guard(ctx->device);
    if (!d || !w || !packed) return fail(ctx, PCV_ERR_INVALID, "pcv_dwconv_pack: NULL argument");
    const char* why = check_dw(*d);
    if (why) return fail(ctx, PCV_ERR_INVALID, std::string("pcv_dwconv_pack: ") + why);
    const int total = d->Cin * d->kh * d->kw;
    const unsigned grid = (unsigned)((total + 255) / 256);
    hipStream_t s = (hipStream_t)stream;
    if (d->dtype == PCV_BF16) pack_dw_kernel<PCV_BF16><<<grid, 256, 0, s>>>(w, packed, d->Cin, d->kh * d->kw);
    else if (d->dtype == PCV_F16) pack_dw_kernel<PCV_F16><<<grid, 256, 0, s>>>(w, packed, d->Cin, d->kh * d->kw);
    else pack_dw_kernel<PCV_F32><<<grid, 256, 0, s>>>(w, packed, d->Cin, d->kh * d->kw);
    if (dw_sparse_bytes(*d) != 0) {
        const int nChunks = (d->Cin + 31) / 32;
        pack_dw_sparse_kernel<<<(unsigned)((nChunks * 6 * 64 + 255) / 256), 256, 0, s>>>(
            static_cast<const uint16_t*>(packed), reinterpret_cast<u32x4*>(static_cast<char*>(packed) + dw_taps_bytes(*d)), d->Cin, nChunks);
    }
    HIP_TRY(ctx, hipGetLastError());
    return PCV_OK;
}

int pcv_bn_fold(pcv_ctx* ctx, int C, const float* gamma, const float* beta, const float* mean, const float* var,
                float eps, const float* conv_bias, float* scale, float* shift, void* stream) {
    if (!ctx) return PCV_ERR_INVALID;
    DeviceGuard device_guard(ctx->device);
    if (C <= 0 || !scale || !shift) return fail(ctx, PCV_ERR_INVALID, "pcv_bn_fold: bad argument");
    const bool any = gamma || beta || mean || var;
    const bool all = gamma && beta && mean && var;
    if (any && !all) return fail(ctx, PCV_ERR_INVALID, "pcv_bn_fold: gamma/beta/mean/var must be all set or all NULL");
    bn_fold_kernel<<<(C + 255) / 256, 256, 0, (hipStream_t)stream>>>(C, gamma, beta, mean, var, eps, conv_bias, scale, shift);
    HIP_TRY(ctx, hipGetLastError());
    return PCV_OK;
}

static int pool_out(int in, int k, int s, int p, int ceil_mode);
static void launch_se_fc(const float* in, const float* w, const float* b, float* out, int N, int K, int J, int act, hipStream_t st);

enum ConvKernel {
    CK_STEM,
    CK_GCONV_ROWS,
    CK_GCONV_FLAT,
    CK_D3I,
    CK_D1I,
    CK_D3K,
    CK_D3C,
    CK_D3W,
    CK_D3Q,
    CK_P1R,
    CK_D3Q_1X1,
    CK_HEAD,
    CK_IGEMM
};
struct ConvRoute {
    ConvKernel kernel = CK_IGEMM;
    int shape = -1;
    GConvRPlan rows{};
    int tile = TILE_C128, khw = 0;
    bool special = false;
};
struct ConvArgs {
    const void* x; const void* packed; const float* scale; const float* shift; const void* residual; void* y;
    const float* gate; hipStream_t stream;
    bool pool;
    bool x_nchw;
};
struct ConvGeom {
    int cpitch, wpitch;
    unsigned long long xbytes, M64;
    bool sliced_y;
};

static void route_igemm(const pcv_ctx* ctx, const pcv_conv_desc* d, const ConvPlan& P, ConvRoute& R) {
    const bool ragged = (d->Cout % 8 != 0) || (P.cout_blk % 8 != 0);
    int tile;
    if (ragged || d->out_dtype != d->dtype) tile = TILE_C128;
    else if (P.cout_blk <= 32) tile = TILE_C32;
    else if (P.cout_blk <= 64) tile = TILE_C64;
    else if (P.cout_blk <= 128) tile = TILE_C128;
    else if (P.cout_blk <= 256) tile = (d->kh * d->kw > 1) ? TILE_C128 : TILE_C256;
    else tile = TILE_C128;
    R.special = ragged || d->out_dtype != d->dtype;
    int khw = 0;
    if (!R.special && !P.pair && d->dil_h == 1 && d->dil_w == 1) {
        if (d->kh == 1 && d->kw == 1 && d->pad_t == 0 && d->pad_l == 0 && d->pad_b == 0 && d->pad_r == 0) khw = 1;
        else if (d->kh == 3 && d->kw == 3 && P.cin_blk % (8 * P.CE) == 0) khw = 9;
    }
    if (khw == 1) {
        if (tile == TILE_C64 && d->Cin >= 256) tile = TILE_C64S;
        else if (tile == TILE_C128 && P.cout_blk <= 128 && d->Cin >= 512) tile = TILE_C128S;
        else if (tile == TILE_C256 && d->Cin > 128) tile = TILE_C128;
        if ((d->act == PCV_ACT_SWISH || d->act == PCV_ACT_SIGMOID) && P.nk <= 2 && P.ngb == 1 && !d->has_residual) {
            const int pad64 = round_up(P.cout_blk, 64), pad128 = round_up(P.cout_blk, 128);
            tile = pad64 < pad128 ? TILE_C64S : TILE_C128S;
        }
    }
    if (ctx->force_tile >= 0 && ctx->force_tile < TILE_COUNT && !R.special && (ctx->force_tile < TILE_C64S || khw == 1))
        tile = ctx->force_tile;
    R.tile = tile;
    R.khw = khw;
}

static ConvRoute route_conv(const pcv_ctx* ctx, const pcv_conv_desc* d, const ConvPlan& P, const ConvGeom& G, const ConvArgs& A) {
    ConvRoute R;
    if (P.stem) { R.kernel = CK_STEM; return R; }
    const bool gconv_ok = P.gconv && !A.gate && !G.sliced_y && !d->has_residual && d->post_act == PCV_ACT_NONE && G.cpitch == d->Cin &&
                          G.wpitch == d->W && G.M64 * (unsigned long long)d->Cin * 2ull < 0x80000000ull;
    if (gconv_ok && ctx->use_gconvr != 0 && (d->stride_h == 2 || P.gconv_kt == 9) &&
        plan_gconvr(d->stride_h, d->H, d->W, P.Ho, P.Wo, R.rows)) { R.kernel = CK_GCONV_ROWS; return R; }
    if (gconv_ok && d->stride_h == 1 && P.gconv_kt == 5 && d->W <= 63) { R.kernel = CK_GCONV_FLAT; return R; }
    const bool clamp_acts = d->act <= PCV_ACT_RELU6 && d->post_act <= PCV_ACT_RELU6;
    if (P.conv3 && !A.gate && ctx->use_d3x3 != 0 && d->dtype != PCV_F32 && clamp_acts && A.scale && A.shift &&
        G.M64 * (unsigned long long)d->Cout * 2ull < 0x80000000ull &&
        G.xbytes + 2ull * (unsigned long long)d->W * d->Cin * 2ull < 0x80000000ull) {
        if (ctx->use_d3c != 0 && (ctx->use_d3x3 < 0 || ctx->use_d3c > 0) && (ctx->use_d3w <= 0 || ctx->use_d3c > 0) && d->Cin == D3CCfg::BM &&
            d->W == D3CCfg::W && G.cpitch == d->Cin && G.wpitch == d->W) {
            const long long tiles = (long long)((d->Cout + 63) / 64) * d->N * ((d->H + D3CCfg::ROWS - 1) / D3CCfg::ROWS);
            if (ctx->use_d3c > 0 || tiles >= 2ll * block_slots(ctx, 1)) { R.kernel = CK_D3C; return R; }
        }
        if (ctx->use_d3k != 0 && (ctx->use_d3x3 < 0 || ctx->use_d3k > 0) && (ctx->use_d3w <= 0 || ctx->use_d3k > 0) && d->Cin == D3KCfg::CIN &&
            d->W == D3KCfg::W && G.cpitch == d->Cin && G.wpitch == d->W) {
            const long long tiles = (long long)((d->Cout + D3KCfg::BM - 1) / D3KCfg::BM) * d->N * ((d->H + D3KCfg::ROWS - 1) / D3KCfg::ROWS);
            if (ctx->use_d3k > 0 || tiles >= 2ll * block_slots(ctx, 1)) { R.kernel = CK_D3K; return R; }
        }
        const int d3i_maxw = d->Cin == 256 ? D3ICfgT<256>::MAXW : D3ICfgT<512>::MAXW, d3i_nimg = d->Cin == 256 ? 1 : 2;
        if (P.d3i && ctx->use_d3i != 0 && (ctx->use_d3x3 < 0 || ctx->use_d3i > 0) && (ctx->use_d3w <= 0 || ctx->use_d3i > 0) &&
            d->H <= d3i_maxw && d->W <= d3i_maxw && G.cpitch == d->Cin && G.wpitch == d->W) {
            const long long tiles = (long long)((d->Cout + D3ICfg::BM - 1) / D3ICfg::BM) * ((d->N + d3i_nimg - 1) / d3i_nimg);
            const bool full = d3i_nimg * d->H * d->W > 16 * ((d->Cin == 256 ? D3ICfgT<256>::NBLK : D3ICfgT<512>::NBLK) - 1) - 16;
            if (ctx->use_d3i > 0 || (full && 4 * tiles >= 3ll * ctx->num_cu)) { R.kernel = CK_D3I; return R; }
        }
        if (ctx->use_d3w != 0 && (ctx->use_d3x3 < 0 || ctx->use_d3w > 0)) {
            R.shape = ctx->use_d3w > 0 ? std::min(ctx->use_d3w - 1, kD3WCount - 1)
                                       : pick_d3w((long long)G.M64, d->Cout, (long long)block_slots(ctx, 1));
            if (R.shape >= 0) { R.kernel = CK_D3W; return R; }
        }
        R.shape = ctx->use_d3x3 > 0 ? std::min(ctx->use_d3x3 - 1, kD3Count - 1)
                                    : pick_d3x3((long long)G.M64, d->Cout, P.nk, (long long)ctx->num_cu);
        if (R.shape >= 0) { R.kernel = CK_D3Q; return R; }
    }
    if (ctx->use_d1x1 != 0 && !A.gate && !P.pair && d->dtype != PCV_F32 && d->out_dtype == d->dtype && d->kh == 1 && d->kw == 1 &&
        d->stride_h == d->stride_w && d->stride_h <= 2 && d->pad_t == 0 && d->pad_l == 0 && d->pad_b == 0 && d->pad_r == 0 && d->groups == 1 &&
        G.cpitch == d->Cin && G.wpitch == d->W && d->Cin % 64 == 0 && d->Cout % 8 == 0 && clamp_acts && A.scale && A.shift &&
        G.M64 * (unsigned long long)d->Cout * 2ull < 0x80000000ull) {
        if (P.d1i && ctx->use_d1i != 0 && (ctx->use_d1x1 < 0 || ctx->use_d1i > 0) && G.xbytes < 0x80000000ull) {
            const long long tiles = ((long long)G.M64 + D1ICfgT<1024>::BP - 1) / D1ICfgT<1024>::BP * ((d->Cout + 255) / 256);
            if (ctx->use_d1i > 0 || (d->Cin >= 1024 && !d->has_residual && 4 * tiles >= 3ll * ctx->num_cu)) { R.kernel = CK_D1I; return R; }
        }
        if (ctx->use_p1r != 0 && (ctx->use_d1x1 < 0 || ctx->use_p1r > 0) && (d->Cin == 256 || d->Cin == 512) && G.xbytes < 0x80000000ull) {
            const int shape = d->Cin == 512 ? 1 : ((d->has_residual || d->Cout < 384) ? 2 : 0);
            const Kernel& S = kP1R[shape][0];
            const long long groups = (d->Cout + S.BM - 1) / S.BM, tiles = ((long long)G.M64 + S.BP - 1) / S.BP * groups;
            if (ctx->use_p1r > 0 || (d->Cout * 4 >= groups * S.BM * 3 && tiles >= 2ll * block_slots(ctx, 1))) {
                R.kernel = CK_P1R;
                R.shape = shape;
                return R;
            }
        }
        R.shape = ctx->use_d1x1 > 0 ? std::min(ctx->use_d1x1 - 1, kD1Count - 1)
                                    : pick_d1x1((long long)G.M64, d->Cout, d->Cin, (long long)block_slots(ctx, 1));
        if (R.shape >= 0) { R.kernel = CK_D3Q_1X1; return R; }
    }
    if (ctx->use_head && d->dtype == PCV_F32 && d->out_dtype == PCV_F32 && d->kh == 1 && d->kw == 1 && d->H == 1 && d->W == 1 &&
        P.Ho == 1 && P.Wo == 1 && d->pad_t == 0 && d->pad_l == 0 && d->pad_b == 0 && d->pad_r == 0 && d->groups == 1 && !A.gate &&
        !d->has_residual && d->post_act == PCV_ACT_NONE && d->Cin % 16 == 0) { R.kernel = CK_HEAD; return R; }
    route_igemm(ctx, d, P, R);
    return R;
}

static int launch_stem(pcv_ctx* ctx, const pcv_conv_desc* d, const ConvPlan& P, const ConvGeom& G, const ConvArgs& A) {
    const bool pool = A.pool, x_nchw = A.x_nchw;
    StemParams q;
    q.x = A.x; q.w = A.packed; q.y = A.y; q.scale = A.scale; q.shift = A.shift; q.ovf = ctx->ovf;
    q.x_bytes = x_nchw ? (uint32_t)((unsigned long long)d->N * d->Cin * d->H * d->W * 4ull) : (uint32_t)G.xbytes;
    q.w_bytes = (uint32_t)P.w_bytes; q.Cin = d->Cin;
    q.Hq = pool ? pool_out(P.Ho, 3, 2, 1, 0) : P.Ho;
    q.Wq = pool ? pool_out(P.Wo, 3, 2, 1, 0) : P.Wo;
    const unsigned long long ybytes = (unsigned long long)d->N * q.Hq * q.Wq * (unsigned long long)d->Cout * P.ES;
    if (!in_window(ybytes)) return too_large(ctx, "pcv_conv2d_fused", "output");
    q.y_bytes = (uint32_t)ybytes;
    q.N = d->N; q.H = d->H; q.W = d->W; q.Wp = G.wpitch; q.Ho = P.Ho; q.Wo = P.Wo; q.Cout = d->Cout;
    q.kh = d->kh; q.pt = d->pad_t; q.x0off = -(d->pad_l + (d->pad_l & 1));
    q.tilesH = pool ? (q.Hq + 6) / 7 : (P.Ho + 15) / 16;
    q.tilesW = pool ? (q.Wq + 6) / 7 : (P.Wo + 15) / 16;
    const long long nT = (long long)d->N * q.tilesH * q.tilesW;
    if (nT >= 0x7FFFFFFFll) return fail(ctx, PCV_ERR_TOO_LARGE, "pcv_conv2d_fused: too many tiles; split the batch");
    q.nTiles = (int)nT;
    q.act = d->act;
    if (d->has_residual || d->post_act != PCV_ACT_NONE)
        return fail(ctx, PCV_ERR_INVALID, "pcv_conv2d_fused: the stem kernel has no residual / post-activation path");
    const int t = d->dtype == PCV_BF16 ? 0 : 1;
    long long nb = block_slots(ctx, ctx->stem_bpc[t]);
    if (nb > nT) nb = nT;
    nb = (nb + 7) / 8 * 8;
    const bool narrow = !pool && d->Cout <= 32 && ctx->use_stem32;
    return launch(ctx, kStem[t][x_nchw ? 1 : 0][narrow ? STEM_NARROW : (pool ? STEM_POOLED : STEM_PLAIN)], (unsigned)nb, A.stream, q);
}

static int launch_gconv_rows(pcv_ctx* ctx, const pcv_conv_desc* d, const ConvPlan& P, const ConvGeom& G, const ConvArgs& A,
                             const GConvRPlan& gr) {
    GConvRParams q;
    std::memset(&q, 0, sizeof(q));
// ... 33 lines not shown
    const long long nT = (long long)q.nPixTiles * (d->Cin / 64);
    if (nT >= 0x7FFFFFFFll) return fail(ctx, PCV_ERR_TOO_LARGE, "pcv_conv2d_fused: too many tiles; split the batch");
    q.nTiles = (int)nT;
    q.act = d->act;
    const int slot = gconv_slot(d->W);
    long long nb = block_slots(ctx, ctx->gconv_bpc[slot]);
    if (nb > nT) nb = nT;
    nb = (nb + 7) / 8 * 8;
    return launch(ctx, gconv_kernel(d->dtype, slot), (unsigned)nb, A.stream, q);
}

enum YPitchRule { Y_ALIGNED, Y_DENSE_ANY };
static int y_pitch(pcv_ctx* ctx, const pcv_conv_desc* d, const ConvGeom& G, YPitchRule rule, int* ypitch, unsigned long long* ybytes) {
    const int es = esize(d->out_dtype);
    *ypitch = d->y_cpitch > 0 ? d->y_cpitch : d->Cout;
    if (*ypitch < d->Cout || (!(rule == Y_DENSE_ANY && *ypitch == d->Cout) && (*ypitch * es) % 16 != 0))
        return fail(ctx, PCV_ERR_INVALID, "pcv_conv2d_fused: y_cpitch must be >= Cout and a multiple of 16 bytes");
    *ybytes = ((G.M64 - 1) * (unsigned long long)*ypitch + d->Cout) * es;
    return PCV_OK;
}

static const Kernel kNoKernel = {nullptr, 0, 0, 0, 0};
static const Kernel& d3_kernel(const ConvRoute& R, const pcv_conv_desc* d) {
    const int t = d->dtype == PCV_BF16 ? 0 : 1;
    switch (R.kernel) {
        case CK_D3C: return kD3C[0][t];
        case CK_D3K: return kD3K[0][t];
        case CK_D3I: return kD3I[d->Cin == 256 ? 0 : 1][t];
        case CK_D1I: return kD1I[d->Cin == 1024 ? 0 : 1][t];
        case CK_D3W: return kD3W[R.shape][t];
        case CK_P1R: return kP1R[R.shape][t];
        case CK_D3Q_1X1: return kD1[R.shape][t];
        case CK_D3Q: return kD3[R.shape][t];
        default: return kNoKernel;
    }
}
static int launch_d3(pcv_ctx* ctx, const pcv_conv_desc* d, const ConvPlan& P, const ConvGeom& G, const ConvArgs& A, const ConvRoute& R) {
    const ConvKernel ck = R.kernel;
    const Kernel& K = d3_kernel(R, d);
    if (!K.fn) return fail(ctx, PCV_ERR_INVALID, "pcv_conv2d_fused: no kernel for this route");
    const bool one = ck == CK_P1R || ck == CK_D1I || ck == CK_D3Q_1X1;
    const bool own_blob = ck == CK_D3I || ck == CK_D1I;
    int ypitch = 0;
    unsigned long long ybytes = 0;
    if (int rc = y_pitch(ctx, d, G, Y_ALIGNED, &ypitch, &ybytes)) return rc;
    if (!in_window(ybytes)) return too_large(ctx, "pcv_conv2d_fused", "output");
    D3Params q;
    std::memset(&q, 0, sizeof(q));
    q.x = A.x; q.res = d->has_residual ? A.residual : nullptr; q.y = A.y;
    q.w = static_cast<const char*>(A.packed) + (own_blob ? P.d3i_off : P.ktab_bytes);
    q.scale = A.scale; q.shift = A.shift; q.ovf = ctx->ovf;
    if (!own_blob) q.dbgflags = ctx->dbg_flags;
    q.x_bytes = (uint32_t)G.xbytes; q.w_bytes = (uint32_t)(own_blob ? P.total_bytes - P.d3i_off : P.w_bytes); q.y_bytes = (uint32_t)ybytes;
    q.res_bytes = (uint32_t)(G.M64 * (unsigned long long)d->Cout * 2ull);
    q.M = (int)G.M64; q.Cout = d->Cout; q.Ypitch = ypitch; q.Cin = d->Cin; q.Kpad = P.Kpad;
    q.Hin = d->H; q.Win = d->W;
    if (one) {
        q.H = P.Ho; q.W = P.Wo; q.HW = P.Ho * P.Wo;
        q.div_w = make_fastdiv((uint32_t)P.Wo);
        q.stride = d->stride_h;
        q.nk = d->Cin / 64; q.slices = q.nk;
    } else {
        q.H = d->H; q.W = d->W; q.HW = d->H * d->W;
        q.div_w = make_fastdiv((uint32_t)d->W);
        q.stride = 1;
        q.nk = P.nk; q.slices = d->Cin / 64;
    }
    if (ck != CK_D3Q_1X1) q.dbg = reinterpret_cast<uint32_t*>(ctx->dbg_ptr);
    q.div_hw = make_fastdiv((uint32_t)q.HW);
    q.act = d->act; q.post_act = d->post_act;
    q.nChTiles = (d->Cout + K.BM - 1) / K.BM;
    static_assert(D3CCfg::ROWS == D3KCfg::ROWS, "launch_d3 computes the tile count of d3c AND d3k from one ROWS constant");
    long long nT;
    switch (ck) {
        case CK_D3C:
        case CK_D3K:
            nT = (long long)d->N * ((d->H + D3CCfg::ROWS - 1) / D3CCfg::ROWS) * q.nChTiles;
            break;
        case CK_D3I: {
            const int nimg = d->Cin == 256 ? D3ICfgT<256>::NIMG : D3ICfgT<512>::NIMG;
            nT = (long long)((d->N + nimg - 1) / nimg) * q.nChTiles;
            break;
        }
        default: nT = ((long long)((G.M64 + K.BP - 1) / K.BP)) * q.nChTiles;
    }
    if (nT >= 0x7FFFFFFFll) return fail(ctx, PCV_ERR_TOO_LARGE, "pcv_conv2d_fused: too many tiles; split the batch");
    q.nTiles = (int)nT;
    long long nb = nT;
    if (!own_blob) {
        const long long slots = block_slots(ctx, 1);
        nb = slots < nT ? slots : nT;
        nb = (nb + 7) / 8 * 8;
    }
    if (ck == CK_P1R && nT > nb) {
        const long long nCG = q.nChTiles, TP = K.BP / 16, rem = nT % nb;
        if (rem > 0 && nb % (8 * nCG) == 0 && rem % nCG == 0 && rem * TP <= nb && ctx->use_p1r != 3 && ctx->use_p1r != -3) {
            q.nTiles = (int)(nT - rem);
            q.tailN = (int)rem;
        }
    }
    return launch(ctx, K, (unsigned)nb, A.stream, q);
}

static int launch_head(pcv_ctx* ctx, const pcv_conv_desc* d, const ConvPlan& P, const ConvGeom& G, const ConvArgs& A) {
    const int ypitch = d->y_cpitch > 0 ? d->y_cpitch : d->Cout;
    if (ypitch < d->Cout) return fail(ctx, PCV_ERR_INVALID, "pcv_conv2d_fused: y_cpitch must be >= Cout");
    HeadParams q;
    q.x = static_cast<const float*>(A.x); q.w = reinterpret_cast<const float*>(static_cast<const char*>(A.packed) + P.ktab_bytes);
    q.scale = A.scale; q.shift = A.shift; q.y = static_cast<float*>(A.y);
    q.M = d->N; q.K = d->Cin; q.Kpad = P.Kpad; q.Cout = d->Cout; q.Xpitch = G.cpitch; q.Ypitch = ypitch; q.act = d->act;
    const unsigned gx = (unsigned)(P.wrows / 32);
    const bool wide = (long long)gx * ((d->N + 31) / 32) >= 2ll * ctx->num_cu;
    if (wide) hipLaunchKernelGGL(head_gemm_f32_kernel<32>, dim3(gx, (unsigned)((d->N + 31) / 32)), dim3(256), 0, A.stream, q);
    else hipLaunchKernelGGL(head_gemm_f32_kernel<16>, dim3(gx, (unsigned)((d->N + 15) / 16)), dim3(256), 0, A.stream, q);
    HIP_TRY(ctx, hipGetLastError());
    return PCV_OK;
}

static int launch_igemm(pcv_ctx* ctx, const pcv_conv_desc* d, const ConvPlan& P, const ConvGeom& G, const ConvArgs& A, const ConvRoute& R) {
    if (R.special && P.ngb != 1 && ((d->Cout % 8 != 0) || (P.cout_blk % 8 != 0)))
        return fail(ctx, PCV_ERR_INVALID, "pcv_conv2d_fused: ragged channel count with groups unsupported");
    const int tile = R.tile, khw = R.khw;
    const Kernel T = igemm_kernel(d->dtype, d->out_dtype, R.special, tile, khw);
    if (!T.fn) return fail(ctx, PCV_ERR_INVALID, "pcv_conv2d_fused: no kernel for this dtype combination");

    IgemmParams p;
    p.x = A.x;
    p.ktab = reinterpret_cast<const uint32_t*>(A.packed);
    p.w = static_cast<const char*>(A.packed) + P.ktab_bytes;
    p.res = d->has_residual ? A.residual : nullptr;
    p.gate = A.gate;
    p.ovf = ctx->ovf;
    p.y = A.y;
    p.scale = A.scale;
    p.shift = A.shift;
    p.x_bytes = (uint32_t)G.xbytes;
    p.w_bytes = (uint32_t)P.w_bytes;
    int ypitch = 0;
    unsigned long long ybytes = 0;
    if (int rc = y_pitch(ctx, d, G, Y_DENSE_ANY, &ypitch, &ybytes)) return rc;
    if (!in_window(ybytes) && d->out_dtype != PCV_F32) return too_large(ctx, "pcv_conv2d_fused", "output");
    p.y_bytes = ybytes >= 0xFFFFFFFFull ? 0xFFFFFFFFu : (uint32_t)ybytes;
    p.M = (int)G.M64;
    p.Cout = P.cout_blk;
    p.Cout_total = d->Cout;
    p.Ypitch = ypitch;
    p.cout_blk = P.cout_blk;
    p.cin_blk = d->groups == 1 ? 0 : P.cin_blk;
    p.wrows_blk = P.wrows;
    p.HoWo = P.Ho * P.Wo;
    p.Wo = P.Wo;
    p.div_howo = make_fastdiv((uint32_t)p.HoWo);
    p.div_wo = make_fastdiv((uint32_t)p.Wo);
    p.H = d->H;
    p.W = d->W;
    p.Wpitch = G.wpitch;
    p.Cpitch = G.cpitch;
    p.sh = d->stride_h;
    p.sw = d->stride_w;
    p.pt = d->pad_t;
    p.pl = d->pad_l;
    p.nR = P.nR;
    p.nQ = P.nQ;
    for (int i = 0; i < IGEMM_MAX_TAPS; ++i) { p.dy[i] = P.dy[i]; p.dx[i] = P.dx[i]; }
    p.nk = P.nk;
    p.Kpad = P.Kpad;
    p.act = d->act;
    p.post_act = d->post_act;
    p.nPixTiles = (p.M + T.BP - 1) / T.BP;
    p.nChTiles = (P.cout_blk + T.BM - 1) / T.BM;
    p.ngb = P.ngb;
    p.Cin = P.cin_blk;
    p.ksteps_per_tap = P.cin_blk / (8 * P.CE) > 0 ? P.cin_blk / (8 * P.CE) : 1;
    p.korder = P.conv3 ? 1 : 0;
    const long long nTiles = (long long)p.nPixTiles * p.nChTiles * P.ngb;
    if (nTiles >= 0x7FFFFFFFll) return fail(ctx, PCV_ERR_TOO_LARGE, "pcv_conv2d_fused: too many tiles; split the batch");
    p.nTiles = (int)nTiles;
    const int bpc = R.special ? ctx->igemm_bpc[d->dtype][1][tile][0] : ctx->igemm_bpc[d->dtype][0][tile][khw_slot(khw)];
    const bool persistent = ctx->persist_mode == 1 || (ctx->persist_mode < 0 && P.nk <= ctx->persist_max_nk);
    long long nblocks = persistent ? block_slots(ctx, bpc) : nTiles;
    if (nblocks > nTiles) nblocks = nTiles;
    nblocks = (nblocks + 7) / 8 * 8;
    p.wstat = (ctx->use_wstat && persistent && P.nk == 1 && p.nChTiles == 1 && P.ngb == 1) ? 1 : 0;
    return launch(ctx, T, (unsigned)nblocks, A.stream, p);
}

static int conv2d_impl(pcv_ctx* ctx, const pcv_conv_desc* d, const void* x, const void* packed, const float* scale,
                       const float* shift, const void* residual, void* y, void* stream, bool pool, const float* gate = nullptr,
                       bool x_nchw = false) {
    if (!ctx) return PCV_ERR_INVALID;
    DeviceGuard device_guard(ctx->device);
    if (!d || !x || !packed || !y) return fail(ctx, PCV_ERR_INVALID, "pcv_conv2d_fused: NULL argument");
    if (d->has_residual && !residual) return fail(ctx, PCV_ERR_INVALID, "pcv_conv2d_fused: has_residual but residual is NULL");
    if (d->N <= 0 || d->H <= 0 || d->W <= 0) return fail(ctx, PCV_ERR_INVALID, "pcv_conv2d_fused: empty input");
    if (d->groups > 1 && d->groups == d->Cin && d->Cin == d->Cout)
        return fail(ctx, PCV_ERR_INVALID, "pcv_conv2d_fused: depthwise convolution goes through pcv_dwconv2d_fused");
    ConvPlan P;
    const char* why = plan_conv(*d, P, false);
    if (why) return fail(ctx, PCV_ERR_INVALID, std::string("pcv_conv2d_fused: ") + why);
    if (P.Ho <= 0 || P.Wo <= 0) return fail(ctx, PCV_ERR_INVALID, "pcv_conv2d_fused: empty output");
    ConvGeom G;
    G.cpitch = d->x_cpitch > 0 ? d->x_cpitch : d->Cin;
    G.wpitch = d->x_wpitch > 0 ? d->x_wpitch : d->W;
    G.xbytes = (unsigned long long)d->N * d->H * G.wpitch * G.cpitch * P.ES;
    G.M64 = (unsigned long long)d->N * P.Ho * P.Wo;
    G.sliced_y = d->y_cpitch > 0 && d->y_cpitch != d->Cout;
    if (!in_window(G.xbytes) || G.M64 >= 0x7FFFFFFFull) return too_large(ctx, "pcv_conv2d_fused", "input");
    if (!aligned16(x) || !aligned16(packed) || !aligned16(y) || (residual && !aligned16(residual)) ||
        (scale && !aligned16(scale)) || (shift && !aligned16(shift)))
        return fail(ctx, PCV_ERR_INVALID, "pcv_conv2d_fused: pointers must be 16-byte aligned");
    if (P.stem && G.sliced_y) return fail(ctx, PCV_ERR_INVALID, "pcv_conv2d_fused: the stem kernel writes a dense y only");
    if (gate && (P.stem || pool)) return fail(ctx, PCV_ERR_INVALID, "pcv_conv2d_gated_fused: the stem kernel has no gate");
    if (pool && !P.stem) return fail(ctx, PCV_ERR_INVALID, "pcv_conv2d_maxpool_fused: only the stem convolution has a fused max-pool");
    if (x_nchw && (!P.stem || d->Cin > 3 || d->W % 4 != 0))
        return fail(ctx, PCV_ERR_INVALID, "pcv_conv2d_nchw_stem_fused: only the stem convolution (<= 3 input planes, W a multiple of 4)");
    if (x_nchw && !in_window((unsigned long long)d->N * d->Cin * d->H * d->W * 4ull))
        return too_large(ctx, "pcv_conv2d_nchw_stem_fused", "the fp32 image batch");

    const ConvArgs A{x, packed, scale, shift, residual, y, gate, (hipStream_t)stream, pool, x_nchw};
    const ConvRoute R = route_conv(ctx, d, P, G, A);
    switch (R.kernel) {
        case CK_STEM: return launch_stem(ctx, d, P, G, A);
        case CK_GCONV_ROWS: return launch_gconv_rows(ctx, d, P, G, A, R.rows);
        case CK_GCONV_FLAT: return launch_gconv_flat(ctx, d, P, G, A);
        case CK_D3I: case CK_D1I: case CK_D3K: case CK_D3C: case CK_D3W: case CK_D3Q: case CK_P1R: case CK_D3Q_1X1:
            return launch_d3(ctx, d, P, G, A, R);
        case CK_HEAD: return launch_head(ctx, d, P, G, A);
        default: return launch_igemm(ctx, d, P, G, A, R);
    }
}

int pcv_conv2d_fused(pcv_ctx* ctx, const pcv_conv_desc* d, const void* x, const void* packed, const float* scale,
                     const float* shift, const void* residual, void* y, void* stream) {
    return conv2d_impl(ctx, d, x, packed, scale, shift, residual, y, stream, false);
}

int pcv_conv2d_gated_fused(pcv_ctx* ctx, const pcv_conv_desc* d, const void* x, const void* packed, const float* scale,
                           const float* shift, const float* gate, const void* residual, void* y, void* stream) {
    if (!ctx) return PCV_ERR_INVALID;
    if (!gate || !aligned16(gate)) return fail(ctx, PCV_ERR_INVALID, "pcv_conv2d_gated_fused: gate must be a 16-byte aligned [N][Cout] fp32 array");
    if (d && d->Cout % 4 != 0) return fail(ctx, PCV_ERR_INVALID, "pcv_conv2d_gated_fused: Cout must be a multiple of 4");
    return conv2d_impl(ctx, d, x, packed, scale, shift, residual, y, stream, false, gate);
}

int pcv_fc_f32(pcv_ctx* ctx, const float* in, const float* w, const float* b, float* out, int N, int K, int J, int act,
               void* stream) {
    if (!ctx) return PCV_ERR_INVALID;
    DeviceGuard device_guard(ctx->device);
    if (!in || !w || !b || !out || N <= 0 || K <= 0 || J <= 0) return fail(ctx, PCV_ERR_INVALID, "pcv_fc_f32: bad argument");
    launch_se_fc(in, w, b, out, N, K, J, act, (hipStream_t)stream);
    HIP_TRY(ctx, hipGetLastError());
    return PCV_OK;
}

int pcv_conv2d_maxpool_supported(const pcv_conv_desc* d, int k, int s, int p, int ceil_mode) {
    if (!d || k != 3 || s != 2 || p != 1 || ceil_mode) return 0;
    ConvPlan P;
    if (plan_conv(*d, P, false) != nullptr || !P.stem) return 0;
    if (d->act != PCV_ACT_RELU && d->act != PCV_ACT_RELU6) return 0;
    return (d->has_residual || d->post_act != PCV_ACT_NONE || (d->y_cpitch > 0 && d->y_cpitch != d->Cout)) ? 0 : 1;
// ... 610 lines not shown
```

pytorchcv_amd/engine.py:

```python

__all__ = ['NHWC', 'DTYPES', 'default_dtype', 'set_compute_dtype', 'compute_dtype_of', 'Fp16Guard', 'fp16_overflow_count', 'from_nchw', 'to_nchw', 'ConvRunner',
           'BnActRunner', 'maxpool2d', 'avgpool2d', 'avgpool2d_pad', 'global_avgpool', 'se_forward', 'splat_forward', 'channel_slice', 'cat_shuffle2', 'act_code',
           'boundary', 'round8', 'channel_concat_into', 'interpolate', 'add']

import os
import ctypes
import torch
import torch.nn as nn
import torch.nn.functional as F
from . import _lib
from ._lib import ConvDesc

DTYPES = {"fp32": (0, torch.float32), "bf16": (1, torch.bfloat16), "fp16": (2, torch.float16)}
_CODE_OF_TORCH = {torch.float32: 0, torch.bfloat16: 1, torch.float16: 2}
_NAME_OF_TORCH = {torch.float32: "fp32", torch.bfloat16: "bf16", torch.float16: "fp16"}


def default_dtype() -> str:
    d = os.environ.get("PCV_AMD_DTYPE", "auto")
    if d not in DTYPES and d != "auto":
        raise ValueError("PCV_AMD_DTYPE must be one of {}".format(sorted(DTYPES) + ["auto"]))
    return d


def set_compute_dtype(net: nn.Module, dtype: str) -> nn.Module:
    if dtype not in DTYPES and dtype != "auto":
        raise ValueError("dtype must be one of {}".format(sorted(DTYPES) + ["auto"]))
    for m in net.modules():
        m._pcv_dtype = dtype
    return net


def stamp_family_dtype(net: nn.Module) -> nn.Module:
    mode = getattr(net, "pcv_16bit", None)
    if mode is not None:
        for m in net.modules():
            if m is not net:
                m.pcv_16bit = mode
    return net


def compute_dtype_of(module: nn.Module) -> str:
    d = getattr(module, "_pcv_dtype", None) or default_dtype()
    if d == "auto":
        d = getattr(module, "pcv_16bit", None) or "bf16"
    return d


class Fp16Guard(object):
    __slots__ = ("slot", "device")

    def __init__(self, device, torch_dtype):
        self.slot = None
        self.device = device
# ... 46 lines not shown
        s = (self.N, self.C, self.H, self.W)
        return s if dim is None else s[dim]


class _ShapeOnly(object):
    __slots__ = ("N", "H", "W", "C", "dtype", "wpitch", "cpitch")

    def __init__(self, N, H, W, C, dtype):
        self.N, self.H, self.W, self.C, self.dtype, self.wpitch, self.cpitch = N, H, W, C, dtype, W, round8(C)


def _stream(device) -> ctypes.c_void_p:
    return ctypes.c_void_p(torch.cuda.current_stream(device).cuda_stream)


def _ctx(device):
    if device.type != "cuda":
        raise RuntimeError("pytorchcv_amd runs on MI355X (gfx950) only: got a tensor on '{}'. Move the model and the input "
                           "to a CUDA/HIP device; there is no CPU path in this package.".format(device))
    idx = device.index if device.index is not None else torch.cuda.current_device()
    return _lib.ctx_for(idx)


def _ptr(t):
    return ctypes.c_void_p(t.data_ptr()) if t is not None else None


class LazyNCHW(NHWC):
    __slots__ = ("src", "_conv", "_dtype_name")

    def __init__(self, x: torch.Tensor, dtype: str):
        N, C, H, W = x.shape
        self.src, self._conv, self._dtype_name = x, None, dtype
        self.N, self.H, self.W, self.C = N, H, W, C
        self.wpitch, self.cpitch = (W + 1) // 2 * 2, 4

    @property
    def t(self):
        if self._conv is None:
            self._conv = from_nchw(self.src, self._dtype_name, stem=True).t
        return self._conv

    @property
    def materialized(self) -> bool:
        return self._conv is not None

    @property
    def dtype(self):
        return DTYPES[self._dtype_name][1]

    @property
    def device(self):
        return self.src.device


def network_input(x: torch.Tensor, dtype: str) -> NHWC:
    if x.dim() != 4:
        raise ValueError("expected a 4-D NCHW tensor")
    if x.shape[1] <= 3 and x.shape[3] % 4 == 0 and STEM_FROM_NCHW:
        return LazyNCHW(x.contiguous().float(), dtype)
    return from_nchw(x, dtype, stem=True)


def from_nchw(x: torch.Tensor, dtype: str, stem: bool = True) -> NHWC:
    if x.dim() != 4:
        raise ValueError("expected a 4-D NCHW tensor")
    x = x.contiguous().float()
    N, C, H, W = x.shape
    code, tdt = DTYPES[dtype]
    if C <= 4 and stem:
        cp, wp = 4, (W + 1) // 2 * 2
    else:
        cp, wp = (C + 7) // 8 * 8, W
    y = torch.empty((N, H, wp, cp), dtype=tdt, device=x.device)
    ctx = _ctx(x.device)
    _lib.check(_lib.lib().pcv_nchw_to_nhwc(ctx, _ptr(x), _ptr(y), N, C, H, W, cp, wp, code, _stream(x.device)), ctx)
    return NHWC(y, N, H, W, C, wpitch=wp, cpitch=cp)


def to_nchw(a: NHWC) -> torch.Tensor:
    if a.wpitch != a.W:
        raise RuntimeError("cannot convert a row-padded input handle back to NCHW")
    y = torch.empty((a.N, a.C, a.H, a.W), dtype=torch.float32, device=a.device)
    ctx = _ctx(a.device)
    _lib.check(_lib.lib().pcv_nhwc_to_nchw(ctx, _ptr(a.t), _ptr(y), a.N, a.C, a.H, a.W, a.cpitch, _CODE_OF_TORCH[a.dtype],
                                           _stream(a.device)), ctx)
    return y


def boundary(module: nn.Module, x, fn, stem: bool = False):
    if isinstance(x, NHWC):
        return fn(x)
    if not torch.is_tensor(x):
        raise TypeError("expected a torch.Tensor or an NHWC handle")
    dtype = compute_dtype_of(module)
    guard = Fp16Guard(x.device, DTYPES[dtype][1])
    y = fn(from_nchw(x, dtype, stem=stem))
    if isinstance(y, tuple):
        return tuple(guard.finish(to_nchw(v)) if isinstance(v, NHWC) else v for v in y)
    y = to_nchw(y) if isinstance(y, NHWC) else y
    return guard.finish(y) if torch.is_tensor(y) and y.dtype == torch.float32 else y


def act_code(activ) -> int:
    from .models.common.activ import Swish, HSigmoid, HSwish
    if activ is None:
        return 0
    if isinstance(activ, nn.ReLU):
        return 1
    if isinstance(activ, nn.ReLU6):
        return 2
    if isinstance(activ, nn.Sigmoid):
        return 3
    if isinstance(activ, Swish):
        return 4
    if isinstance(activ, HSigmoid):
        return 5
    if isinstance(activ, HSwish):
        return 6
    raise NotImplementedError("activation {} has no fused MI355X epilogue yet".format(type(activ).__name__))


def _pair(v):
    return (int(v[0]), int(v[1])) if isinstance(v, (tuple, list)) else (int(v), int(v))


class ConvRunner(object):
    def __init__(self, conv: nn.Conv2d, bn, pad4=None):
        self.conv, self.bn, self.pad4 = conv, bn, pad4
        self._key = None
        self._foreign = False
        self.packed = self.scale = self.shift = None
        self.depthwise = (conv.groups > 1 and conv.groups == conv.in_channels == conv.out_channels)
        if 1 < conv.groups and not self.depthwise and (conv.in_channels % 8 or conv.out_channels % 8):
            raise NotImplementedError("grouped convolution with channel counts that are not multiples of 8")

    def _phys(self, x_cpitch: int, out_fp32: bool):
        c = self.conv
        cin = c.in_channels if x_cpitch == 4 and c.in_channels <= 4 else round8(c.in_channels)
        cout = c.out_channels if out_fp32 else round8(c.out_channels)
        groups = cin if self.depthwise else c.groups
        return cin, cout, groups

    def _sources(self):
        ts = [self.conv.weight, self.conv.bias]
        if self.bn is not None:
            ts += [self.bn.weight, self.bn.bias, self.bn.running_mean, self.bn.running_var]
        return ts

    def _state_key(self, dtype, cpitch, d: ConvDesc):
        return (dtype, cpitch, d.Cin, d.Cout, d.groups, d.out_dtype, d.pad_l & 1) + \
            tuple((t.data_ptr(), t._version) if t is not None else None for t in self._sources())

    def desc(self, x: NHWC, act, post_act, has_res, out_code=None, logits=False, pad4=None) -> ConvDesc:
        c = self.conv
        kh, kw = _pair(c.kernel_size)
        sh, sw = _pair(c.stride)
        dh, dw = _pair(c.dilation)
        pad4 = pad4 if pad4 is not None else self.pad4
        if pad4 is not None:
            pl, pr, pt, pb = [int(v) for v in pad4]
        else:
            ph, pw = _pair(c.padding)
            pt = pb = ph
            pl = pr = pw
        code = _CODE_OF_TORCH[x.dtype]
        cin, cout, groups = self._phys(x.cpitch, logits)
        if x.cpitch != cin and not (x.cpitch == 4 and cin <= 4):
            raise RuntimeError("input handle has {} physical channels, this convolution expects {}".format(x.cpitch, cin))
        d = ConvDesc(N=x.N, H=x.H, W=x.W, Cin=cin, Cout=cout, kh=kh, kw=kw, stride_h=sh, stride_w=sw,
                     pad_t=pt, pad_l=pl, pad_b=pb, pad_r=pr, dil_h=dh, dil_w=dw, groups=groups, act=act, post_act=post_act,
                     has_residual=1 if has_res else 0, dtype=code, out_dtype=code if out_code is None else out_code,
                     x_cpitch=x.cpitch, x_wpitch=x.wpitch)
        return d

    def prepare(self, x: NHWC, d: ConvDesc):
        if isinstance(c_mode := self.conv.padding_mode, str) and c_mode != "zeros":
            raise NotImplementedError("padding_mode {}".format(c_mode))
        key = self._state_key(x.dtype, x.cpitch, d)
        if key == self._key:
            return
        if self._foreign:
            raise RuntimeError(
                "this convolution's packed weights were received by parallel.broadcast_packed_state and would have to be re-packed "
                "(the input's dtype / channel pitch / padding parity or a parameter changed), but this rank's fp32 parameters are "
                "not the source's. Call parallel.broadcast_module_state(net) (or load_state_dict on every rank) before running "
                "another configuration.")
        dev = x.device
        w = self.conv.weight
        if w.device != dev:
            raise RuntimeError("model parameters are on {} but the input is on {}".format(w.device, dev))
        L, ctx, st = _lib.lib(), _ctx(dev), _stream(dev)
        nbytes = ctypes.c_size_t(0)
        fn_bytes = L.pcv_dwconv_packed_bytes if self.depthwise else L.pcv_conv_packed_bytes
        if fn_bytes(ctypes.byref(d), ctypes.byref(nbytes)) != 0:
            raise _lib.PcvError(-1, "unsupported convolution configuration: {}".format(
                {f[0]: getattr(d, f[0]) for f in d._fields_}))
        packed = torch.empty((nbytes.value + 15) // 16 * 16, dtype=torch.uint8, device=dev)
        w32 = w.detach().float()
        if w32.dim() == 2:
            w32 = w32[:, :, None, None]
        C, Cl = d.Cout, self.conv.out_channels
        cin_g = d.Cin // d.groups
        if w32.shape[0] != C or w32.shape[1] != cin_g:
            w32 = F.pad(w32, (0, 0, 0, 0, 0, cin_g - w32.shape[1], 0, C - w32.shape[0]))
        w32 = w32.contiguous()
        fn_pack = L.pcv_dwconv_pack if self.depthwise else L.pcv_conv_pack
        _lib.check(fn_pack(ctx, ctypes.byref(d), _ptr(w32), _ptr(packed), st), ctx)

        def padded(t, fill):
            t = t.detach().float()
            return (F.pad(t, (0, C - Cl), value=fill) if C != Cl else t).contiguous()
        scale = torch.empty(C, dtype=torch.float32, device=dev)
        shift = torch.empty(C, dtype=torch.float32, device=dev)
        bias = padded(self.conv.bias, 0.0) if self.conv.bias is not None else None
        if self.bn is not None:
            if not isinstance(self.bn, nn.BatchNorm2d):
                raise NotImplementedError("only BatchNorm2d folds into the conv epilogue, got {}".format(type(self.bn).__name__))
            g = padded(self.bn.weight, 0.0) if self.bn.weight is not None else padded(torch.ones(Cl, device=dev), 0.0)
            b = padded(self.bn.bias, 0.0) if self.bn.bias is not None else torch.zeros(C, device=dev)
            m = padded(self.bn.running_mean, 0.0)
            v = padded(self.bn.running_var, 1.0)
            _lib.check(L.pcv_bn_fold(ctx, C, _ptr(g), _ptr(b), _ptr(m), _ptr(v), ctypes.c_float(self.bn.eps), _ptr(bias),
                                     _ptr(scale), _ptr(shift), st), ctx)
        else:
            _lib.check(L.pcv_bn_fold(ctx, C, None, None, None, None, ctypes.c_float(0.0), _ptr(bias), _ptr(scale),
                                     _ptr(shift), st), ctx)
        torch.cuda.current_stream(dev).synchronize()
        self.packed, self.scale, self.shift, self._key = packed, scale, shift, key

    def adopt_foreign_state(self):
        self._foreign = True
        self._sq_key = None

    def local_state_restored(self):
        self._foreign = False
        self._key = None

    def run(self, x: NHWC, act=0, residual: NHWC | None = None, post_act=0, out_fp32=False, pad4=None, out=None, gate=None) -> NHWC:
        if self.bn is not None and self.bn.training:
            raise RuntimeError("pytorchcv_amd is an inference path: call net.eval() first (BatchNorm is folded)")
        if isinstance(x, LazyNCHW) and not x.materialized and residual is None and out is None and gate is None and not out_fp32 \
                and post_act == 0 and pad4 is None:
            y = self._stem_from_nchw(x, act, pool=False)
            if y is not None:
                return y
        d = self.desc(x, act, post_act, residual is not None, out_code=0 if out_fp32 else None, logits=out_fp32, pad4=pad4)
        self.prepare(x, d)
        return self._launch(x, d, residual, out, gate)

    def _stem_from_nchw(self, x: "LazyNCHW", act: int, pool: bool):
        if self.depthwise or self.pad4 is not None or x.src.numel() * 4 >= (1 << 31):
            return None
        d = self.desc(x, act, 0, False)
        L, ctx = _lib.lib(), _ctx(x.device)
        if not L.pcv_conv2d_nchw_stem_supported(ctypes.byref(d), 1 if pool else 0):
            return None
        self.prepare(x, d)
        Ho = (x.H + d.pad_t + d.pad_b - d.dil_h * (d.kh - 1) - 1) // d.stride_h + 1
        Wo = (x.W + d.pad_l + d.pad_r - d.dil_w * (d.kw - 1) - 1) // d.stride_w + 1
        if pool:
            Ho, Wo = (Ho + 2 - 3) // 2 + 1, (Wo + 2 - 3) // 2 + 1
        if Ho <= 0 or Wo <= 0:
            return None
        y = torch.empty((x.N, Ho, Wo, d.Cout), dtype=x.dtype, device=x.device)
        _lib.check(L.pcv_conv2d_nchw_stem_fused(ctx, ctypes.byref(d), _ptr(x.src), _ptr(self.packed), _ptr(self.scale), _ptr(self.shift),
                                                _ptr(y), 1 if pool else 0, _stream(x.device)), ctx)
        return NHWC(y, x.N, Ho, Wo, self.conv.out_channels, cpitch=d.Cout)

    def run_maxpool(self, x: NHWC, act: int, k: int, s: int, p: int, ceil_mode: bool = False):
        if not FUSE_UNITS or self.depthwise or self.pad4 is not None:
            return None
        if self.bn is not None and self.bn.training:
            raise RuntimeError("pytorchcv_amd is an inference path: call net.eval() first (BatchNorm is folded)")
        if isinstance(x, LazyNCHW) and not x.materialized and (k, s, p) == (3, 2, 1) and not ceil_mode:
            y = self._stem_from_nchw(x, act, pool=True)
            if y is not None:
                return y
        d = self.desc(x, act, 0, False)
        L, ctx = _lib.lib(), _ctx(x.device)
        if not L.pcv_conv2d_maxpool_supported(ctypes.byref(d), k, s, p, 1 if ceil_mode else 0):
            return None
        self.prepare(x, d)
        Ho = (x.H + d.pad_t + d.pad_b - d.dil_h * (d.kh - 1) - 1) // d.stride_h + 1
        Wo = (x.W + d.pad_l + d.pad_r - d.dil_w * (d.kw - 1) - 1) // d.stride_w + 1
        Hq, Wq = (Ho + 2 * p - k) // s + 1, (Wo + 2 * p - k) // s + 1
        if Hq <= 0 or Wq <= 0:
            return None
        y = torch.empty((x.N, Hq, Wq, d.Cout), dtype=x.dtype, device=x.device)
        _lib.check(L.pcv_conv2d_maxpool_fused(ctx, ctypes.byref(d), _ptr(x.t), _ptr(self.packed), _ptr(self.scale), _ptr(self.shift),
                                              _ptr(y), k, s, p, 1 if ceil_mode else 0, _stream(x.device)), ctx)
        return NHWC(y, x.N, Hq, Wq, self.conv.out_channels, cpitch=d.Cout)

    def run_pair(self, x: NHWC, residual: NHWC, act: int, post_act: int, nxt: "ConvRunner", nxt_act: int, gate=None):
        if not FUSE_UNITS or residual is None or self.depthwise or nxt.depthwise or self.pad4 is not None or nxt.pad4 is not None:
            return None
        if (self.bn is not None and self.bn.training) or (nxt.bn is not None and nxt.bn.training):
            raise RuntimeError("pytorchcv_amd is an inference path: call net.eval() first (BatchNorm is folded)")
        c = self.conv
        L, ctx, st = _lib.lib(), _ctx(x.device), _stream(x.device)
        d1 = self.desc(x, act, post_act, True)
# ... 13 lines not shown
        if gate is not None:
            _lib.check(L.pcv_conv1x1_pair_gated_fused(ctx, ctypes.byref(d1), ctypes.byref(d2), _ptr(x.t), _ptr(self.packed),
                                                      _ptr(self.scale), _ptr(self.shift), _ptr(gate), _ptr(residual.t), _ptr(t1),
                                                      _ptr(nxt.packed), _ptr(nxt.scale), _ptr(nxt.shift), _ptr(t2), st), ctx)
        else:
            _lib.check(L.pcv_conv1x1_pair_fused(ctx, ctypes.byref(d1), ctypes.byref(d2), _ptr(x.t), _ptr(self.packed),
                                                _ptr(self.scale), _ptr(self.shift), _ptr(residual.t), _ptr(t1), _ptr(nxt.packed),
                                                _ptr(nxt.scale), _ptr(nxt.shift), _ptr(t2), st), ctx)
        return y1, NHWC(t2, x.N, x.H, x.W, nxt.conv.out_channels, cpitch=d2.Cout)

    def run_pair_idconv(self, x: NHWC, x0: NHWC, idr: "ConvRunner", act: int, post_act: int, nxt: "ConvRunner", nxt_act: int):
        if not FUSE_UNITS or any(r.depthwise or r.pad4 is not None for r in (self, idr, nxt)):
            return None
        if any(r.bn is not None and r.bn.training for r in (self, idr, nxt)):
            raise RuntimeError("pytorchcv_amd is an inference path: call net.eval() first (BatchNorm is folded)")
        if not x0.dense or x0.dtype != x.dtype or (x0.N, x0.H, x0.W) != (x.N, x.H, x.W):
            return None
        c = self.conv
        L, ctx, st = _lib.lib(), _ctx(x.device), _stream(x.device)
        di = idr.desc(x0, 0, 0, False)
        d1 = self.desc(x, act, post_act, True)
        d2 = nxt.desc(_ShapeOnly(x.N, x.H, x.W, c.out_channels, x.dtype), nxt_act, 0, False)
        if not L.pcv_conv1x1_pair_idconv_supported(ctypes.byref(di), ctypes.byref(d1), ctypes.byref(d2)):
            return None
        t1 = torch.empty((x.N, x.H, x.W, d1.Cout), dtype=x.dtype, device=x.device)
        t2 = torch.empty((x.N, x.H, x.W, d2.Cout), dtype=x.dtype, device=x.device)
        y1 = NHWC(t1, x.N, x.H, x.W, c.out_channels, cpitch=d1.Cout)
        idr.prepare(x0, di)
        self.prepare(x, d1)
        nxt.prepare(y1, d2)
        _lib.check(L.pcv_conv1x1_pair_idconv_fused(ctx, ctypes.byref(di), ctypes.byref(d1), ctypes.byref(d2), _ptr(x0.t),
                                                   _ptr(idr.packed), _ptr(idr.scale), _ptr(idr.shift), _ptr(x.t), _ptr(self.packed),
                                                   _ptr(self.scale), _ptr(self.shift), _ptr(t1), _ptr(nxt.packed), _ptr(nxt.scale),
                                                   _ptr(nxt.shift), _ptr(t2), st), ctx)
        return y1, NHWC(t2, x.N, x.H, x.W, nxt.conv.out_channels, cpitch=d2.Cout)

    def _launch(self, x: NHWC, d: ConvDesc, residual, out=None, gate=None):
        c = self.conv
        kh, kw = d.kh, d.kw
        Ho = (x.H + d.pad_t + d.pad_b - d.dil_h * (kh - 1) - 1) // d.stride_h + 1
        Wo = (x.W + d.pad_l + d.pad_r - d.dil_w * (kw - 1) - 1) // d.stride_w + 1
        if Ho <= 0 or Wo <= 0:
            raise RuntimeError("convolution output would be empty")
        out_dt = torch.float32 if d.out_dtype == 0 else x.dtype
        if out is not None:
            buf, coff = out
            if self.depthwise or tuple(buf.shape[:3]) != (x.N, Ho, Wo) or buf.dtype != out_dt or not buf.is_contiguous() or \
                    coff % 8 != 0 or c.out_channels % 8 != 0 or coff + c.out_channels > buf.shape[3] or buf.device != x.device:
                raise RuntimeError("bad concatenation slice for a convolution output (channel counts must be multiples of 8)")
            d.y_cpitch = int(buf.shape[3])
            y = buf[:, :, :, coff:]
        else:
            y = torch.empty((x.N, Ho, Wo, d.Cout), dtype=out_dt, device=x.device)
        if residual is not None:
            if not residual.dense or tuple(residual.t.shape) != (x.N, Ho, Wo, d.Cout) or residual.dtype != x.dtype:
                raise RuntimeError("residual shape/dtype mismatch: {} vs {}".format(
                    tuple(residual.t.shape), (x.N, Ho, Wo, d.Cout)))
        if gate is not None:
            if self.depthwise or gate.dtype != torch.float32 or tuple(gate.shape) != (x.N, d.Cout) or not gate.is_contiguous():
                raise RuntimeError("gate must be a contiguous fp32 [N, {}] tensor of a dense convolution".format(d.Cout))
        self._launch_range(x, d, residual, y, 0, x.N, gate)
        return None if out is not None else NHWC(y, x.N, Ho, Wo, c.out_channels, cpitch=d.Cout)

    def _launch_range(self, x, d, residual, y, n0, n1, gate=None):
        L, ctx, st = _lib.lib(), _ctx(x.device), _stream(x.device)
        d.N = n1 - n0
        rp = _ptr(residual.t[n0:n1]) if residual is not None else None
        if gate is not None:
            rc = L.pcv_conv2d_gated_fused(ctx, ctypes.byref(d), _ptr(x.t[n0:n1]), _ptr(self.packed), _ptr(self.scale),
                                          _ptr(self.shift), _ptr(gate[n0:n1]), rp, _ptr(y[n0:n1]), st)
        else:
            fn = L.pcv_dwconv2d_fused if self.depthwise else L.pcv_conv2d_fused
            rc = fn(ctx, ctypes.byref(d), _ptr(x.t[n0:n1]), _ptr(self.packed), _ptr(self.scale), _ptr(self.shift), rp, _ptr(y[n0:n1]), st)
        if rc == _lib.PCV_ERR_TOO_LARGE and n1 - n0 > 1:
            mid = (n0 + n1) // 2
            self._launch_range(x, d, residual, y, n0, mid, gate)
            self._launch_range(x, d, residual, y, mid, n1, gate)
            return
        _lib.check(rc, ctx)

    def squeezed_excite(self, z: NHWC, w1, b1, w2, b2, mid_act: int, out_act: int) -> torch.Tensor:
        c = self.conv
        if self.depthwise or c.groups != 1 or tuple(_pair(c.kernel_size)) != (1, 1) or tuple(_pair(c.stride)) != (1, 1) or \
                self.pad4 is not None or tuple(_pair(c.padding)) != (0, 0):
            raise RuntimeError("squeezed_excite needs a plain 1x1 stride-1 convolution")
        d = self.desc(z, 0, 0, False)
        self.prepare(z, d)
        key = ("sq", self._key) + tuple((t.data_ptr(), t._version) for t in (w1, w2, b1, b2))
        if getattr(self, "_sq_key", None) != key:
            Cl, CP = c.out_channels, d.Cout
            w = c.weight.detach().float().reshape(Cl, -1)
            w = F.pad(w, (0, d.Cin - w.shape[1], 0, CP - Cl)) * self.scale[:, None]
            w1p = F.pad(w1.float(), (0, CP - Cl))
            self._sq_w1 = (w1p @ w).contiguous()
            self._sq_b1 = (w1p @ self.shift + b1.float()).contiguous()
            self._sq_w2 = F.pad(w2.float(), (0, 0, 0, CP - Cl)).contiguous()
            self._sq_b2 = F.pad(b2.float(), (0, CP - Cl)).contiguous()
            self._sq_key = key
        L, ctx, st = _lib.lib(), _ctx(z.device), _stream(z.device)
        M = self._sq_w1.shape[0]
        mean = torch.empty((z.N, d.Cin), dtype=torch.float32, device=z.device)
        _lib.check(L.pcv_se_squeeze(ctx, _ptr(z.t), _ptr(mean), z.N, z.H * z.W, d.Cin, _CODE_OF_TORCH[z.dtype], st), ctx)
        mid = torch.empty((z.N, M), dtype=torch.float32, device=z.device)
        gate = torch.empty((z.N, d.Cout), dtype=torch.float32, device=z.device)
        _lib.check(L.pcv_fc_f32(ctx, _ptr(mean), _ptr(self._sq_w1), _ptr(self._sq_b1), _ptr(mid), z.N, d.Cin, M, mid_act, st), ctx)
        _lib.check(L.pcv_fc_f32(ctx, _ptr(mid), _ptr(self._sq_w2), _ptr(self._sq_b2), _ptr(gate), z.N, M, d.Cout, out_act, st), ctx)
        return gate
# ... 50 lines not shown

def cat_shuffle2(a: NHWC, b: NHWC, half: int) -> NHWC:
    if (a.N, a.H, a.W) != (b.N, b.H, b.W) or a.dtype != b.dtype or a.wpitch != a.W or b.wpitch != b.W or half > a.C or half > b.C:
        raise RuntimeError("cat/shuffle operands do not match")
    cp = round8(2 * half)
    y = torch.empty((a.N, a.H, a.W, cp), dtype=a.dtype, device=a.device)
    ctx = _ctx(a.device)
    _lib.check(_lib.lib().pcv_channel_interleave2(ctx, _ptr(a.t), _ptr(b.t), _ptr(y), a.N * a.H * a.W, half, a.cpitch, b.cpitch,
                                                  cp, _CODE_OF_TORCH[a.dtype], _stream(a.device)), ctx)
    return NHWC(y, a.N, a.H, a.W, 2 * half, cpitch=cp)


def maxpool2d(x: NHWC, k: int, s: int, p: int, ceil_mode: bool = False) -> NHWC:
    if not x.dense:
        raise RuntimeError("max-pool on a padded handle")
    Ho, Wo = _pool_out(x.H, k, s, p, ceil_mode), _pool_out(x.W, k, s, p, ceil_mode)
    y = torch.empty((x.N, Ho, Wo, x.cpitch), dtype=x.dtype, device=x.device)
    ctx = _ctx(x.device)
    _lib.check(_lib.lib().pcv_maxpool2d(ctx, _ptr(x.t), _ptr(y), x.N, x.H, x.W, x.cpitch, k, s, p, 1 if ceil_mode else 0,
                                        _CODE_OF_TORCH[x.dtype], _stream(x.device)), ctx)
    return NHWC(y, x.N, Ho, Wo, x.C, cpitch=x.cpitch)


def avgpool2d(x: NHWC, k: int, s: int, out_fp32: bool = False) -> NHWC:
    if not x.dense:
        raise RuntimeError("avg-pool on a padded handle")
    if k > x.H or k > x.W:
        raise RuntimeError("AvgPool2d kernel {} larger than the {}x{} map".format(k, x.H, x.W))
    Ho, Wo = (x.H - k) // s + 1, (x.W - k) // s + 1
    y = torch.empty((x.N, Ho, Wo, x.cpitch), dtype=torch.float32 if out_fp32 else x.dtype, device=x.device)
    ctx = _ctx(x.device)
    code = _CODE_OF_TORCH[x.dtype]
    _lib.check(_lib.lib().pcv_avgpool2d(ctx, _ptr(x.t), _ptr(y), x.N, x.H, x.W, x.cpitch, k, s, code, 0 if out_fp32 else code,
                                        _stream(x.device)), ctx)
    return NHWC(y, x.N, Ho, Wo, x.C, cpitch=x.cpitch)


def avgpool2d_pad(x: NHWC, k: int, s: int, p: int = 0, ceil_mode: bool = False, count_include_pad: bool = True) -> NHWC:
    if not x.dense:
        raise RuntimeError("avg-pool on a padded handle")
    Ho, Wo = _pool_out(x.H, k, s, p, ceil_mode), _pool_out(x.W, k, s, p, ceil_mode)
    if Ho <= 0 or Wo <= 0:
        raise RuntimeError("AvgPool2d({}, {}, {}) output of a {}x{} map would be empty".format(k, s, p, x.H, x.W))
    y = torch.empty((x.N, Ho, Wo, x.cpitch), dtype=x.dtype, device=x.device)
    ctx = _ctx(x.device)
    code = _CODE_OF_TORCH[x.dtype]
    _lib.check(_lib.lib().pcv_avgpool2d_pad(ctx, _ptr(x.t), _ptr(y), x.N, x.H, x.W, x.cpitch, k, s, p, 1 if ceil_mode else 0,
                                            1 if count_include_pad else 0, code, code, _stream(x.device)), ctx)
    return NHWC(y, x.N, Ho, Wo, x.C, cpitch=x.cpitch)


FP32_HEAD = os.environ.get("PCV_AMD_FP32_HEAD", "1") != "0"
STEM_FROM_NCHW = os.environ.get("PCV_AMD_STEM_NCHW", "1") != "0"


FUSE_UNITS = os.environ.get("PCV_AMD_FUSE_UNITS", "1") != "0"


def mbconv_fused(exp, exp_act: int, dw, dw_act: int, proj, proj_act: int, x: NHWC, residual, post_act: int):
    if not FUSE_UNITS or not x.dense or not dw.depthwise or proj.depthwise or (exp is not None and exp.depthwise):
        return None
    if any(r is not None and r.pad4 is not None for r in (exp, dw, proj)):
        return None
    for r in (exp, dw, proj):
        if r is not None and r.bn is not None and r.bn.training:
            raise RuntimeError("pytorchcv_amd is an inference path: call net.eval() first (BatchNorm is folded)")
    L, ctx, st = _lib.lib(), _ctx(x.device), _stream(x.device)
    cur = x
    d_exp = None
    if exp is not None:
        d_exp = exp.desc(x, exp_act, 0, False)
        cur = _ShapeOnly(x.N, x.H, x.W, exp.conv.out_channels, x.dtype)
    d_dw = dw.desc(cur, dw_act, 0, False)
    Ho = (cur.H + d_dw.pad_t + d_dw.pad_b - d_dw.dil_h * (d_dw.kh - 1) - 1) // d_dw.stride_h + 1
    Wo = (cur.W + d_dw.pad_l + d_dw.pad_r - d_dw.dil_w * (d_dw.kw - 1) - 1) // d_dw.stride_w + 1
    mid = _ShapeOnly(x.N, Ho, Wo, dw.conv.out_channels, x.dtype)
    d_proj = proj.desc(mid, proj_act, post_act, residual is not None)
    if not L.pcv_mbconv_supported(ctypes.byref(d_exp) if d_exp is not None else None, ctypes.byref(d_dw), ctypes.byref(d_proj)):
        return None
    Cout = d_proj.Cout
    if residual is not None and (not residual.dense or residual.dtype != x.dtype or
                                 tuple(residual.t.shape) != (x.N, Ho, Wo, Cout)):
        raise RuntimeError("residual shape/dtype mismatch")
    if exp is not None:
        exp.prepare(x, d_exp)
    dw.prepare(_PrepHandle(cur, x.device), d_dw)
    proj.prepare(_PrepHandle(mid, x.device), d_proj)
    y = torch.empty((x.N, Ho, Wo, Cout), dtype=x.dtype, device=x.device)
    _lib.check(L.pcv_mbconv_fused(ctx, ctypes.byref(d_exp) if d_exp is not None else None, ctypes.byref(d_dw), ctypes.byref(d_proj),
                                  _ptr(x.t), _ptr(exp.packed) if exp is not None else None,
                                  _ptr(exp.scale) if exp is not None else None, _ptr(exp.shift) if exp is not None else None,
                                  _ptr(dw.packed), _ptr(dw.scale), _ptr(dw.shift), _ptr(proj.packed), _ptr(proj.scale),
                                  _ptr(proj.shift), _ptr(residual.t) if residual is not None else None, _ptr(y), st), ctx)
    return NHWC(y, x.N, Ho, Wo, proj.conv.out_channels, cpitch=Cout)


class _PrepHandle(object):
    __slots__ = ("dtype", "cpitch", "device")

    def __init__(self, shape_only, device):
        self.dtype, self.cpitch, self.device = shape_only.dtype, shape_only.cpitch, device


class BnActRunner(object):
    def __init__(self, bn):
        self.bn = bn
# ... 120 lines not shown
```

pytorchcv_amd/models/common/conv.py:

```python

__all__ = ['conv1x1', 'conv3x3', 'depthwise_conv3x3', 'ConvBlock', 'conv1x1_block', 'conv3x3_block', 'conv5x5_block',
           'conv7x7_block', 'dwconv_block', 'dwconv3x3_block', 'dwconv5x5_block', 'DwsConvBlock', 'dwsconv3x3_block', 'BareConv', 'PreConvBlock',
           'pre_conv1x1_block', 'pre_conv3x3_block', 'conv_block_pair', 'conv_block_maxpool', 'mbconv_chain']

import torch.nn as nn
from .activ import lambda_relu, create_activation_layer
from .norm import lambda_batchnorm2d, create_normalization_layer
from ... import engine


class BareConv(nn.Conv2d):
    def forward(self, x, out_fp32: bool = False, act: int = 0):
        if getattr(self, "_pcv_runner", None) is None:
            self._pcv_runner = engine.ConvRunner(self, None)
        return engine.boundary(self, x, lambda a: self._pcv_runner.run(a, act=act, out_fp32=out_fp32))


def conv1x1(in_channels, out_channels, stride=1, groups=1, bias=False):
    return BareConv(in_channels=in_channels, out_channels=out_channels, kernel_size=1, stride=stride, groups=groups, bias=bias)


def conv3x3(in_channels, out_channels, stride=1, padding=1, dilation=1, groups=1, bias=False):
    return BareConv(in_channels=in_channels, out_channels=out_channels, kernel_size=3, stride=stride, padding=padding,
                    dilation=dilation, groups=groups, bias=bias)


def depthwise_conv3x3(channels, stride=1, padding=1, dilation=1, bias=False):
    return BareConv(in_channels=channels, out_channels=channels, kernel_size=3, stride=stride, padding=padding,
                    dilation=dilation, groups=channels, bias=bias)


class ConvBlock(nn.Module):
    def __init__(self, in_channels, out_channels, kernel_size, stride=1, padding=0, dilation=1, groups=1, bias=False,
                 normalization=lambda_batchnorm2d(), activation=lambda_relu()):
        super(ConvBlock, self).__init__()
        self.normalize = (normalization is not None)
        self.activate = (activation is not None)
        self.use_pad = (isinstance(padding, (list, tuple)) and (len(padding) == 4))
        self._pad4 = tuple(int(p) for p in padding) if self.use_pad else None
        self.conv = nn.Conv2d(in_channels=in_channels, out_channels=out_channels, kernel_size=kernel_size, stride=stride,
                              padding=(0 if self.use_pad else padding), dilation=dilation, groups=groups, bias=bias)
        if self.normalize:
            self.bn = create_normalization_layer(normalization=normalization, num_features=out_channels)
            if self.bn is None:
                self.normalize = False
            else:
                assert isinstance(self.bn, nn.Module)
        if self.activate:
            self.activ = create_activation_layer(activation)
            if self.activ is None:
                self.activate = False
            else:
                assert isinstance(self.activ, nn.Module)
        self._pcv_runner = None

    def forward(self, x, residual=None, post_act=None, pad4=None, out=None):
        if self._pcv_runner is None:
            self._pcv_runner = engine.ConvRunner(self.conv, self.bn if self.normalize else None, pad4=self._pad4)
        act = engine.act_code(self.activ) if self.activate else 0
        pact = engine.act_code(post_act)
        return engine.boundary(self, x, lambda a: self._pcv_runner.run(a, act=act, residual=residual, post_act=pact,
                                                                       pad4=pad4, out=out))


def conv_block_maxpool(block, x, pool):
    if isinstance(block, ConvBlock) and isinstance(x, engine.NHWC) and not block.use_pad:
        if block._pcv_runner is None:
            block._pcv_runner = engine.ConvRunner(block.conv, block.bn if block.normalize else None, pad4=block._pad4)
        y = block._pcv_runner.run_maxpool(x, engine.act_code(block.activ) if block.activate else 0, pool.kernel_size,
                                          pool.stride, pool.padding, pool.ceil_mode)
        if y is not None:
            return y
    return pool(block(x))


def conv_block_pair(first, x, residual, post_act, second, id_block=None, x0=None):
    if not (isinstance(first, ConvBlock) and isinstance(second, ConvBlock) and isinstance(x, engine.NHWC)):
        return None
    for blk in (first, second) + ((id_block,) if id_block is not None else ()):
        if not isinstance(blk, ConvBlock):
            return None
        if blk._pcv_runner is None:
            blk._pcv_runner = engine.ConvRunner(blk.conv, blk.bn if blk.normalize else None, pad4=blk._pad4)
    if id_block is not None:
        if id_block.activate or not isinstance(x0, engine.NHWC):
            return None
        return first._pcv_runner.run_pair_idconv(x, x0, id_block._pcv_runner, engine.act_code(first.activ) if first.activate else 0,
                                                 engine.act_code(post_act), second._pcv_runner,
                                                 engine.act_code(second.activ) if second.activate else 0)
    return first._pcv_runner.run_pair(x, residual, engine.act_code(first.activ) if first.activate else 0,
                                      engine.act_code(post_act), second._pcv_runner,
                                      engine.act_code(second.activ) if second.activate else 0)


def mbconv_chain(exp_block, dw_block, proj_block, x, residual=None, post_act=None):
    blocks = [b for b in (exp_block, dw_block, proj_block) if b is not None]
    if not isinstance(x, engine.NHWC) or not all(isinstance(b, ConvBlock) for b in blocks):
        return None
    for blk in blocks:
        if blk._pcv_runner is None:
            blk._pcv_runner = engine.ConvRunner(blk.conv, blk.bn if blk.normalize else None, pad4=blk._pad4)

    def code(blk):
        return engine.act_code(blk.activ) if blk.activate else 0
    return engine.mbconv_fused(exp_block._pcv_runner if exp_block is not None else None,
                               code(exp_block) if exp_block is not None else 0, dw_block._pcv_runner, code(dw_block),
                               proj_block._pcv_runner, code(proj_block), x, residual, engine.act_code(post_act))


def conv1x1_block(padding=0, **kwargs):
    return ConvBlock(kernel_size=1, padding=padding, **kwargs)


def conv3x3_block(padding=1, **kwargs):
    return ConvBlock(kernel_size=3, padding=padding, **kwargs)
# ... 113 lines not shown
```

pytorchcv_amd/models/resnet.py:

```python

__all__ = ['ResNet', 'resnet10', 'resnet12', 'resnet14', 'resnetbc14b', 'resnet16', 'resnet18', 'resnet26', 'resnetbc26b',
           'resnet34', 'resnetbc38b', 'resnet50', 'resnet50b', 'resnet101', 'resnet101b', 'resnet152', 'resnet152b',
           'ResBlock', 'ResBottleneck', 'ResUnit', 'ResStage', 'ResInitBlock', 'get_resnet']

import torch.nn as nn
from .common.activ import lambda_relu
from .common.norm import lambda_batchnorm2d
from .common.conv import conv1x1_block, conv3x3_block, conv7x7_block, conv_block_pair, conv_block_maxpool
from ._tail import MaxPool2dNHWC, AvgPool2dNHWC, LinearHead, run_net, maybe_load_pretrained, init_conv_params, DEFAULT_ROOT
from .. import engine


class ResBlock(nn.Module):
    def __init__(self, in_channels, out_channels, stride, bias=False, normalization=lambda_batchnorm2d(),
                 activation=lambda_relu(), final_activation=None):
        super(ResBlock, self).__init__()
        self.conv1 = conv3x3_block(in_channels=in_channels, out_channels=out_channels, stride=stride, bias=bias,
                                   normalization=normalization, activation=activation)
        self.conv2 = conv3x3_block(in_channels=out_channels, out_channels=out_channels, bias=bias,
                                   normalization=normalization, activation=final_activation)

    def forward(self, x, residual=None, post_act=None):
        return engine.boundary(self, x, lambda a: self.conv2(self.conv1(a), residual=residual, post_act=post_act))


class ResBottleneck(nn.Module):
    def __init__(self, in_channels, out_channels, stride, padding=1, dilation=1, bias=False,
                 normalization=lambda_batchnorm2d(), conv1_stride=False, bottleneck_factor=4, activation=lambda_relu(),
                 final_activation=None):
        super(ResBottleneck, self).__init__()
        mid_channels = out_channels // bottleneck_factor
        self.conv1 = conv1x1_block(in_channels=in_channels, out_channels=mid_channels, stride=(stride if conv1_stride else 1),
                                   bias=bias, normalization=normalization, activation=activation)
        self.conv2 = conv3x3_block(in_channels=mid_channels, out_channels=mid_channels,
                                   stride=(1 if conv1_stride else stride), padding=padding, dilation=dilation, bias=bias,
                                   normalization=normalization, activation=activation)
        self.conv3 = conv1x1_block(in_channels=mid_channels, out_channels=out_channels, bias=bias,
                                   normalization=normalization, activation=final_activation)

    def forward(self, x, residual=None, post_act=None):
        return engine.boundary(self, x, lambda a: self.conv3(self.conv2(self.conv1(a)), residual=residual, post_act=post_act))


class ResUnit(nn.Module):
    def __init__(self, in_channels, out_channels, stride=1, padding=1, dilation=1, bias=False,
                 normalization=lambda_batchnorm2d(), bottleneck=True, conv1_stride=False, activation=lambda_relu(),
                 final_body_activation=None, final_activation=lambda_relu()):
        super(ResUnit, self).__init__()
        self.resize_identity = (in_channels != out_channels) or (stride != 1)
        if bottleneck:
            self.body = ResBottleneck(in_channels=in_channels, out_channels=out_channels, stride=stride, padding=padding,
                                      dilation=dilation, bias=bias, normalization=normalization, conv1_stride=conv1_stride,
                                      activation=activation, final_activation=final_body_activation)
        else:
            self.body = ResBlock(in_channels=in_channels, out_channels=out_channels, stride=stride, bias=bias,
                                 normalization=normalization, activation=activation, final_activation=final_body_activation)
        if self.resize_identity:
            self.identity_conv = conv1x1_block(in_channels=in_channels, out_channels=out_channels, stride=stride, bias=bias,
                                               normalization=normalization, activation=None)
        self.activ = final_activation()

    def _run(self, a):
        identity = self.identity_conv(a) if self.resize_identity else a
        return self.body(a, residual=identity, post_act=self.activ)

    def run_chained(self, a, conv1_out=None, next_unit=None):
        body = self.body
        y = body.conv2(conv1_out if conv1_out is not None else body.conv1(a))
        if next_unit is not None and self.resize_identity:
            pair = conv_block_pair(body.conv3, y, None, self.activ, next_unit.body.conv1, id_block=self.identity_conv, x0=a)
            if pair is not None:
                return pair
        identity = self.identity_conv(a) if self.resize_identity else a
        if next_unit is not None:
            pair = conv_block_pair(body.conv3, y, identity, self.activ, next_unit.body.conv1)
            if pair is not None:
                return pair
        return body.conv3(y, residual=identity, post_act=self.activ), None

    def forward(self, x):
        return engine.boundary(self, x, self._run)


class ResStage(nn.Sequential):
    def forward(self, x):
        units = list(self.children())
        chainable = all((isinstance(u, ResUnit) and isinstance(u.body, ResBottleneck)) or getattr(u, "pcv_chainable", False) for u in units)
        if not isinstance(x, engine.NHWC) or not chainable:
            return super(ResStage, self).forward(x)
        conv1_out = None
        for i, unit in enumerate(units):
            x, conv1_out = unit.run_chained(x, conv1_out, units[i + 1] if i + 1 < len(units) else None)
        return x


class ResInitBlock(nn.Module):
    def __init__(self, in_channels, out_channels, normalization=lambda_batchnorm2d()):
        super(ResInitBlock, self).__init__()
        self.conv = conv7x7_block(in_channels=in_channels, out_channels=out_channels, stride=2, normalization=normalization)
        self.pool = MaxPool2dNHWC(kernel_size=3, stride=2, padding=1)

    def forward(self, x):
        return engine.boundary(self, x, lambda a: conv_block_maxpool(self.conv, a, self.pool), stem=True)


class ResNet(nn.Module):
    def __init__(self, channels, init_block_channels, bottleneck, conv1_stride, in_channels=3, in_size=(224, 224),
                 num_classes=1000):
        super(ResNet, self).__init__()
        self.in_size = in_size
        self.num_classes = num_classes
        self.features = nn.Sequential()
        self.features.add_module("init_block", ResInitBlock(in_channels=in_channels, out_channels=init_block_channels))
        in_channels = init_block_channels
        for i, channels_per_stage in enumerate(channels):
            stage = ResStage()
            for j, out_channels in enumerate(channels_per_stage):
                stride = 2 if (j == 0) and (i != 0) else 1
                stage.add_module("unit{}".format(j + 1), ResUnit(in_channels=in_channels, out_channels=out_channels,
                                                                 stride=stride, bottleneck=bottleneck,
                                                                 conv1_stride=conv1_stride))
                in_channels = out_channels
            self.features.add_module("stage{}".format(i + 1), stage)
        self.features.add_module("final_pool", AvgPool2dNHWC(kernel_size=7, stride=1, fp32_out=True))
        self.output = LinearHead(in_features=in_channels, out_features=num_classes)
        init_conv_params(self)

    def forward(self, x):
        return run_net(self, x, self.output)


# ... 101 lines not shown
```

Measured before the change: 96160 images/sec.

## Defer stage-tail conv2/conv3 and compute only pixels read by strided next stage

The last bottleneck unit of each stage now returns a lazy tail. When the next stage's first unit reads only every second pixel (stride-2 1x1 conv1 and identity conv), the tail's 3x3 conv2 runs at stride 2 and conv3 reads a strided residual directly, so only a quarter of the tail pixels are computed. This adds res_stride/pack_stride descriptor fields, a strided-residual igemm/d3q variant and packing-order handling. Strided residuals fall back from the specialised p1r/d1i kernels to the generic igemm path, which may be slower per pixel.

```diff
diff --git a/include/pcv_amd.h b/include/pcv_amd.h
--- a/include/pcv_amd.h
+++ b/include/pcv_amd.h
@@ -43,6 +43,9 @@
     int32_t out_dtype;
     int32_t x_cpitch;
     int32_t x_wpitch;
+    int32_t res_stride;
+    int32_t res_H, res_W;
+    int32_t pack_stride;
     int32_t y_cpitch;
 } pcv_conv_desc;
 
diff --git a/pytorchcv_amd/_lib.py b/pytorchcv_amd/_lib.py
--- a/pytorchcv_amd/_lib.py
+++ b/pytorchcv_amd/_lib.py
@@ -26,7 +26,7 @@
     _fields_ = [(n, ctypes.c_int32) for n in (
         "struct_size", "N", "H", "W", "Cin", "Cout", "kh", "kw", "stride_h", "stride_w", "pad_t", "pad_l", "pad_b", "pad_r",
         "dil_h", "dil_w", "groups", "act", "post_act", "has_residual", "dtype", "out_dtype", "x_cpitch", "x_wpitch",
-        "y_cpitch")]
+        "res_stride", "res_H", "res_W", "pack_stride", "y_cpitch")]
 
 
     def __init__(self, *args, **kw):
diff --git a/pytorchcv_amd/csrc/d3q_conv.hpp b/pytorchcv_amd/csrc/d3q_conv.hpp
--- a/pytorchcv_amd/csrc/d3q_conv.hpp
+++ b/pytorchcv_amd/csrc/d3q_conv.hpp
@@ -25,6 +25,7 @@
     uint32_t* ovf;
     int tailN;
     int dbgflags;
+    int res_s, res_H, res_W;
 };
 
 #ifdef PCV_DBG_FLAGS
@@ -416,7 +417,17 @@
 #pragma unroll
                 for (int j = 0; j < PBW; ++j) {
                     const int m = mBase + 16 * j;
-                    const uint32_t roff = (chok && m < p.M) ? (uint32_t)(((size_t)m * p.Cout + ch0) * 2) : 0x80000000u;
+                    size_t mr = (size_t)m;
+                    if constexpr (ONE) {
+                        if (p.res_s > 1) {
+                            const uint32_t n = fastdiv((uint32_t)m, p.div_hw);
+                            const uint32_t rem = (uint32_t)m - n * (uint32_t)p.HW;
+                            const uint32_t ho = fastdiv(rem, p.div_w);
+                            const uint32_t wo = rem - ho * (uint32_t)p.W;
+                            mr = ((size_t)n * p.res_H + ho * (uint32_t)p.res_s) * p.res_W + wo * (uint32_t)p.res_s;
+                        }
+                    }
+                    const uint32_t roff = (chok && m < p.M) ? (uint32_t)((mr * p.Cout + ch0) * 2) : 0x80000000u;
                     rr[j] = __builtin_amdgcn_raw_buffer_load_b128(rrsrc, roff, 0, 0);
                 }
             }
diff --git a/pytorchcv_amd/csrc/igemm_conv.hpp b/pytorchcv_amd/csrc/igemm_conv.hpp
--- a/pytorchcv_amd/csrc/igemm_conv.hpp
+++ b/pytorchcv_amd/csrc/igemm_conv.hpp
@@ -40,6 +40,7 @@
     int wstat;
     const float* gate;
     uint32_t* ovf;
+    int res_s, res_H, res_W;
 };
 
 template <int DT> struct Mma;
@@ -66,7 +67,7 @@
     }
 };
 
-template <int DT, int OT, int CB, int PB, int WC, int WP, bool RAGGED, int KHW>
+template <int DT, int OT, int CB, int PB, int WC, int WP, bool RAGGED, int KHW, bool RS = false>
 __global__ __launch_bounds__(64 * WC * WP, 2) void igemm_conv_kernel(const IgemmParams p) {
 #if defined(__HIP_DEVICE_COMPILE__)
     constexpr int NW = WC * WP;
@@ -237,6 +238,14 @@
         }
     };
 
+    auto res_row = [&](int m) -> size_t {
+        if constexpr (!RS) return (size_t)m;
+        const uint32_t n = fastdiv((uint32_t)m, p.div_howo);
+        const uint32_t rem = (uint32_t)m - n * (uint32_t)p.HoWo;
+        const uint32_t ho = fastdiv(rem, p.div_wo);
+        const uint32_t wo = rem - ho * (uint32_t)p.Wo;
+        return ((size_t)n * p.res_H + ho * (uint32_t)p.res_s) * p.res_W + wo * (uint32_t)p.res_s;
+    };
     const ActClamp act = make_act(p.act), pact = make_act(p.post_act);
     const bool bounded = act_bounded(p.post_act) || (p.post_act == PCV_ACT_NONE && p.res == nullptr && p.gate == nullptr && act_bounded(p.act));
     zero_acc();
@@ -291,7 +300,7 @@
                 for (int j = 0; j < PB; ++j) {
                     const int m = mBase + 16 * j;
                     const bool ok = p.res != nullptr && ch0 < p.Cout && m < p.M;
-                    const size_t eoff = (size_t)m * p.Cout_total + chg;
+                    const size_t eoff = (RS ? (ok ? res_row(m) : (size_t)0) : (size_t)m) * p.Cout_total + chg;
                     if constexpr (DT == PCV_F32) {
                         rres32[ip][j][0] = ok ? *reinterpret_cast<const f32x4*>(reinterpret_cast<const float*>(p.res) + eoff)
                                               : (f32x4){0.f, 0.f, 0.f, 0.f};
diff --git a/pytorchcv_amd/csrc/pcv_api.hip b/pytorchcv_amd/csrc/pcv_api.hip
--- a/pytorchcv_amd/csrc/pcv_api.hip
+++ b/pytorchcv_amd/csrc/pcv_api.hip
@@ -98,6 +98,7 @@
     int persist_max_nk = 4;
     uint32_t* ovf = nullptr;
     int igemm_bpc[3][2][TILE_COUNT][3] = {};
+    int igemm_rs_bpc[3][TILE_COUNT] = {};
     int gconv_bpc[3] = {2, 2, 2};
     int stem_bpc[2] = {1, 1};
     int pair_bpc[2] = {1, 1};
@@ -161,6 +162,7 @@
 struct ConvPlan {
     bool stem = false;
     bool conv3 = false;
+    bool conv3_order = false;
     int ES = 2, CE = 8;
     bool pair = false;
     int Ho = 0, Wo = 0;
@@ -200,6 +202,11 @@
     if (d.x_cpitch < 0 || d.x_cpitch > 8 * kMaxChannels || d.x_wpitch < 0 || d.x_wpitch > 2 * kMaxExtent || d.y_cpitch < 0 ||
         d.y_cpitch > 8 * kMaxChannels)
         return "pitch out of range";
+    if (d.res_stride < 0 || d.res_stride > kMaxGeom || d.res_H < 0 || d.res_W < 0 || d.res_H > kMaxExtent || d.res_W > kMaxExtent)
+        return "res_stride / res_H / res_W out of range";
+    if (d.res_stride > 1 && !d.has_residual) return "res_stride without a residual";
+    if (d.pack_stride < 0 || d.pack_stride > kMaxGeom) return "pack_stride out of range";
+    if (tables && d.pack_stride != 0) return "pack_stride is a launch-time field: pack under the layer's own stride";
     if (d.kh >= IGEMM_MAX_TAPS || d.kw >= IGEMM_MAX_TAPS) return "kernel size > 15 unsupported";
     if (d.stride_h <= 0 || d.stride_w <= 0 || d.dil_h <= 0 || d.dil_w <= 0) return "non-positive stride/dilation";
     if (d.Cin % d.groups || d.Cout % d.groups) return "channels not divisible by groups";
@@ -225,9 +232,11 @@
     if (d.groups == 1) P.cin_blk = d.Cin;
     P.wrows = round_up(P.cout_blk, 32);
 
-    P.conv3 = d.groups == 1 && d.kh == 3 && d.kw == 3 && d.stride_h == 1 && d.stride_w == 1 && d.dil_h == 1 && d.dil_w == 1 &&
+    const bool conv3_but_stride = d.groups == 1 && d.kh == 3 && d.kw == 3 && d.dil_h == 1 && d.dil_w == 1 &&
               d.pad_t == 1 && d.pad_l == 1 && d.pad_b == 1 && d.pad_r == 1 && d.Cin % (8 * P.CE) == 0 && cpitch == d.Cin &&
               (d.x_wpitch <= 0 || d.x_wpitch == d.W) && d.out_dtype == d.dtype && d.Cout % 8 == 0;
+    P.conv3 = conv3_but_stride && d.stride_h == 1 && d.stride_w == 1;
+    P.conv3_order = conv3_but_stride && (d.pack_stride > 0 ? d.pack_stride == 1 : P.conv3);
 
     P.stem = P.pair && d.stride_h == 2 && d.stride_w == 2 && d.dil_h == 1 && d.Cout <= 64 && d.Cout % 8 == 0 && d.kh <= 7 &&
              d.kw + (d.pad_l & 1) <= 8 && d.out_dtype == d.dtype;
@@ -276,6 +285,7 @@
         P.total_bytes = P.d3i_off + (size_t)(d.Cout / D3ICfg::CW) * (d.Cin == 256 ? D3ICfgT<256>::WBYTES : D3ICfgT<512>::WBYTES);
     }
     P.d1i = !P.conv3 && !P.pair && !P.stem && P.ES == 2 && d.kh == 1 && d.kw == 1 && d.groups == 1 && d.stride_h == 1 && d.stride_w == 1 &&
+            d.pack_stride <= 1 &&
             d.pad_t == 0 && d.pad_l == 0 && d.pad_b == 0 && d.pad_r == 0 && (d.Cin == 1024 || d.Cin == 2048) &&
             d.Cout % 64 == 0 && d.out_dtype == d.dtype && P.wrows >= d.Cout && P.Kpad == d.Cin && P.ngb == 1;
     if (P.d1i) {
@@ -353,6 +363,17 @@
 };
 typedef void (*igemm_fn)(const IgemmParams);
 
+template <int DT> static igemm_fn igemm_strided_res(int tile) {
+    switch (tile) {
+        case TILE_C32: return igemm_conv_kernel<DT, DT, 2, 4, 1, 4, false, 1, true>;
+        case TILE_C64: return igemm_conv_kernel<DT, DT, 4, 4, 1, 4, false, 1, true>;
+        case TILE_C128: return igemm_conv_kernel<DT, DT, 4, 4, 2, 2, false, 1, true>;
+        case TILE_C256: return igemm_conv_kernel<DT, DT, 4, 4, 4, 1, false, 1, true>;
+        case TILE_C64S: return igemm_conv_kernel<DT, DT, 4, 2, 1, 4, false, 1, true>;
+        case TILE_C128S: return igemm_conv_kernel<DT, DT, 4, 2, 2, 2, false, 1, true>;
+        default: return nullptr;
+    }
+}
 template <int DT, int KHW> static igemm_fn igemm_for_tile(int tile) {
     switch (tile) {
         case TILE_C32: return igemm_conv_kernel<DT, DT, 2, 4, 1, 4, false, KHW>;
@@ -369,7 +390,11 @@
     if (khw == 9) return igemm_for_tile<DT, 9>(tile);
     return igemm_for_tile<DT, 0>(tile);
 }
-static igemm_fn igemm_fn_for(int dt, int ot, bool ragged, int tile, int khw) {
+static igemm_fn igemm_fn_for(int dt, int ot, bool ragged, int tile, int khw, bool res_strided = false) {
+    if (res_strided) {
+        if (ragged || ot != dt || khw != 1) return nullptr;
+        return dt == PCV_BF16 ? igemm_strided_res<PCV_BF16>(tile) : (dt == PCV_F16 ? igemm_strided_res<PCV_F16>(tile) : igemm_strided_res<PCV_F32>(tile));
+    }
     if (!ragged && ot == dt) {
         if (dt == PCV_BF16) return igemm_for_taps<PCV_BF16>(tile, khw);
         if (dt == PCV_F16) return igemm_for_taps<PCV_F16>(tile, khw);
@@ -386,9 +411,9 @@
     return nullptr;
 }
 
-static Kernel igemm_kernel(int dt, int ot, bool ragged, int tile, int khw) {
+static Kernel igemm_kernel(int dt, int ot, bool ragged, int tile, int khw, bool res_strided = false) {
     const TileInfo& T = kTiles[tile];
-    return kernel_of(igemm_fn_for(dt, ot, ragged, tile, khw), T.threads, T.lds, T.BM, T.BP);
+    return kernel_of(igemm_fn_for(dt, ot, ragged, tile, khw, res_strided), T.threads, T.lds, T.BM, T.BP);
 }
 static inline int khw_slot(int khw) { return khw == 1 ? 1 : (khw == 9 ? 2 : 0); }
 
@@ -525,7 +550,7 @@
     return d.kh == 1 && d.kw == 1 && d.stride_h == 1 && d.stride_w == 1 && d.pad_t == 0 && d.pad_l == 0 && d.pad_b == 0 &&
            d.pad_r == 0 && d.groups == 1 && d.dil_h == 1 && d.dil_w == 1 && d.out_dtype == d.dtype &&
            (d.x_cpitch == 0 || d.x_cpitch == d.Cin) && (d.x_wpitch == 0 || d.x_wpitch == d.W) &&
-           (d.y_cpitch == 0 || d.y_cpitch == d.Cout);
+           (d.y_cpitch == 0 || d.y_cpitch == d.Cout) && d.res_stride <= 1 && d.pack_stride == 0;
 }
 static const char* pair_unsupported(const pcv_conv_desc& a, const pcv_conv_desc& b) {
     if (desc_stale(a) || desc_stale(b)) return kStaleDesc;
@@ -616,6 +641,7 @@
                 on(k, &ctx->igemm_bpc[dt][0][tile][ks]);
                 report(k, dt, tile, khws[ks], 0);
             }
+            on(igemm_kernel(dt, dt, false, tile, 1, true), &ctx->igemm_rs_bpc[dt][tile]);
             const Kernel f32out = igemm_kernel(dt, PCV_F32, true, tile, 0), same = igemm_kernel(dt, dt, true, tile, 0);
             on(f32out);
             report(f32out, dt, tile, 0, 1);
@@ -943,7 +969,7 @@
 int pcv_conv_packed_bytes(const pcv_conv_desc* d, size_t* bytes) {
     if (!d || !bytes) return PCV_ERR_INVALID;
     ConvPlan P;
-    if (plan_conv(*d, P, false) != nullptr) return PCV_ERR_INVALID;
+    if (plan_conv(*d, P, false) != nullptr || d->pack_stride != 0) return PCV_ERR_INVALID;
     *bytes = P.total_bytes;
     return PCV_OK;
 }
@@ -1024,6 +1050,7 @@
     if (d.x_cpitch > 0 && d.x_cpitch != d.Cin) return "depthwise: padded channel pitch unsupported";
     if (d.x_wpitch > 0 && d.x_wpitch != d.W) return "depthwise: padded row pitch unsupported";
     if (d.y_cpitch > 0 && d.y_cpitch != d.Cout) return "depthwise: y must be dense";
+    if (d.res_stride > 1 || d.pack_stride != 0) return "depthwise: the residual must be dense (res_stride), no pack_stride";
     return nullptr;
 }
 
@@ -1106,6 +1133,8 @@
     int cpitch, wpitch;
     unsigned long long xbytes, M64;
     bool sliced_y;
+    int res_s;
+    unsigned long long res_rows;
 };
 
 static void route_igemm(const pcv_ctx* ctx, const pcv_conv_desc* d, const ConvPlan& P, ConvRoute& R) {
@@ -1180,11 +1209,11 @@
         d->stride_h == d->stride_w && d->stride_h <= 2 && d->pad_t == 0 && d->pad_l == 0 && d->pad_b == 0 && d->pad_r == 0 && d->groups == 1 &&
         G.cpitch == d->Cin && G.wpitch == d->W && d->Cin % 64 == 0 && d->Cout % 8 == 0 && clamp_acts && A.scale && A.shift &&
         G.M64 * (unsigned long long)d->Cout * 2ull < 0x80000000ull) {
-        if (P.d1i && ctx->use_d1i != 0 && (ctx->use_d1x1 < 0 || ctx->use_d1i > 0) && G.xbytes < 0x80000000ull) {
+        if (P.d1i && !G.res_s && ctx->use_d1i != 0 && (ctx->use_d1x1 < 0 || ctx->use_d1i > 0) && G.xbytes < 0x80000000ull) {
             const long long tiles = ((long long)G.M64 + D1ICfgT<1024>::BP - 1) / D1ICfgT<1024>::BP * ((d->Cout + 255) / 256);
             if (ctx->use_d1i > 0 || (d->Cin >= 1024 && !d->has_residual && 4 * tiles >= 3ll * ctx->num_cu)) { R.kernel = CK_D1I; return R; }
         }
-        if (ctx->use_p1r != 0 && (ctx->use_d1x1 < 0 || ctx->use_p1r > 0) && (d->Cin == 256 || d->Cin == 512) && G.xbytes < 0x80000000ull) {
+        if (!G.res_s && ctx->use_p1r != 0 && (ctx->use_d1x1 < 0 || ctx->use_p1r > 0) && (d->Cin == 256 || d->Cin == 512) && G.xbytes < 0x80000000ull) {
             const int shape = d->Cin == 512 ? 1 : ((d->has_residual || d->Cout < 384) ? 2 : 0);
             const Kernel& S = kP1R[shape][0];
             const long long groups = (d->Cout + S.BM - 1) / S.BM, tiles = ((long long)G.M64 + S.BP - 1) / S.BP * groups;
@@ -1324,7 +1353,11 @@
     q.scale = A.scale; q.shift = A.shift; q.ovf = ctx->ovf;
     if (!own_blob) q.dbgflags = ctx->dbg_flags;
     q.x_bytes = (uint32_t)G.xbytes; q.w_bytes = (uint32_t)(own_blob ? P.total_bytes - P.d3i_off : P.w_bytes); q.y_bytes = (uint32_t)ybytes;
-    q.res_bytes = (uint32_t)(G.M64 * (unsigned long long)d->Cout * 2ull);
+    q.res_bytes = (uint32_t)(G.res_rows * (unsigned long long)d->Cout * 2ull);
+    if (G.res_s) {
+        if (ck != CK_D3Q_1X1) return fail(ctx, PCV_ERR_INVALID, "pcv_conv2d_fused: this kernel reads a dense residual only");
+        q.res_s = G.res_s; q.res_H = d->res_H; q.res_W = d->res_W;
+    }
     q.M = (int)G.M64; q.Cout = d->Cout; q.Ypitch = ypitch; q.Cin = d->Cin; q.Kpad = P.Kpad;
     q.Hin = d->H; q.Win = d->W;
     if (one) {
@@ -1393,14 +1426,16 @@
     if (R.special && P.ngb != 1 && ((d->Cout % 8 != 0) || (P.cout_blk % 8 != 0)))
         return fail(ctx, PCV_ERR_INVALID, "pcv_conv2d_fused: ragged channel count with groups unsupported");
     const int tile = R.tile, khw = R.khw;
-    const Kernel T = igemm_kernel(d->dtype, d->out_dtype, R.special, tile, khw);
-    if (!T.fn) return fail(ctx, PCV_ERR_INVALID, "pcv_conv2d_fused: no kernel for this dtype combination");
+    const Kernel T = igemm_kernel(d->dtype, d->out_dtype, R.special, tile, khw, G.res_s != 0);
+    if (!T.fn) return fail(ctx, PCV_ERR_INVALID, G.res_s ? "pcv_conv2d_fused: no kernel reads a strided residual for this configuration"
+                                                        : "pcv_conv2d_fused: no kernel for this dtype combination");
 
     IgemmParams p;
     p.x = A.x;
     p.ktab = reinterpret_cast<const uint32_t*>(A.packed);
     p.w = static_cast<const char*>(A.packed) + P.ktab_bytes;
     p.res = d->has_residual ? A.residual : nullptr;
+    p.res_s = G.res_s; p.res_H = G.res_s ? d->res_H : 0; p.res_W = G.res_s ? d->res_W : 0;
     p.gate = A.gate;
     p.ovf = ctx->ovf;
     p.y = A.y;
@@ -1444,11 +1479,12 @@
     p.ngb = P.ngb;
     p.Cin = P.cin_blk;
     p.ksteps_per_tap = P.cin_blk / (8 * P.CE) > 0 ? P.cin_blk / (8 * P.CE) : 1;
-    p.korder = P.conv3 ? 1 : 0;
+    p.korder = P.conv3_order ? 1 : 0;
     const long long nTiles = (long long)p.nPixTiles * p.nChTiles * P.ngb;
     if (nTiles >= 0x7FFFFFFFll) return fail(ctx, PCV_ERR_TOO_LARGE, "pcv_conv2d_fused: too many tiles; split the batch");
     p.nTiles = (int)nTiles;
-    const int bpc = R.special ? ctx->igemm_bpc[d->dtype][1][tile][0] : ctx->igemm_bpc[d->dtype][0][tile][khw_slot(khw)];
+    const int bpc = G.res_s ? ctx->igemm_rs_bpc[d->dtype][tile]
+                            : (R.special ? ctx->igemm_bpc[d->dtype][1][tile][0] : ctx->igemm_bpc[d->dtype][0][tile][khw_slot(khw)]);
     const bool persistent = ctx->persist_mode == 1 || (ctx->persist_mode < 0 && P.nk <= ctx->persist_max_nk);
     long long nblocks = persistent ? block_slots(ctx, bpc) : nTiles;
     if (nblocks > nTiles) nblocks = nTiles;
@@ -1478,6 +1514,19 @@
     G.M64 = (unsigned long long)d->N * P.Ho * P.Wo;
     G.sliced_y = d->y_cpitch > 0 && d->y_cpitch != d->Cout;
     if (!in_window(G.xbytes) || G.M64 >= 0x7FFFFFFFull) return too_large(ctx, "pcv_conv2d_fused", "input");
+    if (d->pack_stride != 0 && (P.stem || pool || gate || d->groups != 1 || d->kh != d->kw || (d->kh != 1 && d->kh != 3)))
+        return fail(ctx, PCV_ERR_INVALID, "pcv_conv2d_fused: pack_stride needs a dense, ungated 1x1 or 3x3 convolution (not the stem)");
+    G.res_s = d->has_residual && d->res_stride > 1 ? d->res_stride : 0;
+    G.res_rows = G.M64;
+    if (G.res_s) {
+        if (d->kh != 1 || d->kw != 1 || d->groups != 1 || gate || pool || P.stem || P.pair || d->Cout % 8 != 0 || d->out_dtype != d->dtype ||
+            d->pad_t != 0 || d->pad_l != 0 || d->pad_b != 0 || d->pad_r != 0 || d->dil_h != 1 || d->dil_w != 1)
+            return fail(ctx, PCV_ERR_INVALID, "pcv_conv2d_fused: res_stride > 1 needs an ungrouped, ungated, unpadded 1x1 convolution with Cout % 8 == 0");
+        if ((long long)(P.Ho - 1) * G.res_s >= d->res_H || (long long)(P.Wo - 1) * G.res_s >= d->res_W)
+            return fail(ctx, PCV_ERR_INVALID, "pcv_conv2d_fused: res_H / res_W do not cover the output map at res_stride");
+        G.res_rows = (unsigned long long)d->N * d->res_H * d->res_W;
+        if (!in_window(G.res_rows * (unsigned long long)d->Cout * P.ES)) return too_large(ctx, "pcv_conv2d_fused", "residual");
+    }
     if (!aligned16(x) || !aligned16(packed) || !aligned16(y) || (residual && !aligned16(residual)) ||
         (scale && !aligned16(scale)) || (shift && !aligned16(shift)))
         return fail(ctx, PCV_ERR_INVALID, "pcv_conv2d_fused: pointers must be 16-byte aligned");
diff --git a/pytorchcv_amd/engine.py b/pytorchcv_amd/engine.py
--- a/pytorchcv_amd/engine.py
+++ b/pytorchcv_amd/engine.py
@@ -1,5 +1,5 @@
 
-__all__ = ['NHWC', 'DTYPES', 'default_dtype', 'set_compute_dtype', 'compute_dtype_of', 'Fp16Guard', 'fp16_overflow_count', 'from_nchw', 'to_nchw', 'ConvRunner',
+__all__ = ['NHWC', 'SampledNHWC', 'LazyStageTail', 'DTYPES', 'default_dtype', 'set_compute_dtype', 'compute_dtype_of', 'Fp16Guard', 'fp16_overflow_count', 'from_nchw', 'to_nchw', 'ConvRunner',
            'BnActRunner', 'maxpool2d', 'avgpool2d', 'avgpool2d_pad', 'global_avgpool', 'se_forward', 'splat_forward', 'channel_slice', 'cat_shuffle2', 'act_code',
            'boundary', 'round8', 'channel_concat_into', 'interpolate', 'add']
 
@@ -152,6 +152,57 @@
     @property
     def device(self):
         return self.src.device
+
+
+class SampledNHWC(NHWC):
+    __slots__ = ("stride", "full_H", "full_W")
+
+    def __init__(self, full: NHWC, stride: int):
+        if not full.dense or stride < 1:
+            raise RuntimeError("only a dense handle can be sampled at a stride")
+        NHWC.__init__(self, full.t, full.N, (full.H - 1) // stride + 1, (full.W - 1) // stride + 1, full.C, cpitch=full.cpitch)
+        self.stride, self.full_H, self.full_W = int(stride), full.H, full.W
+
+
+class LazyStageTail(NHWC):
+    __slots__ = ("_run_full", "_run_sub", "_full", "_subs", "_dtype", "_device")
+
+    def __init__(self, N, H, W, C, cpitch, dtype, device, run_full, run_sub):
+        self.N, self.H, self.W, self.C = N, H, W, C
+        self.wpitch, self.cpitch = W, cpitch
+        self._dtype, self._device = dtype, device
+        self._run_full, self._run_sub = run_full, run_sub
+        self._full, self._subs = None, {}
+
+    @property
+    def t(self):
+        if self._full is None:
+            y = self._run_full()
+            if (y.N, y.H, y.W, y.cpitch) != (self.N, self.H, self.W, self.cpitch) or not y.dense:
+                raise RuntimeError("deferred stage tail produced an unexpected shape")
+            self._full = y.t
+        return self._full
+
+    def subsampled(self, s: int) -> NHWC:
+        s = int(s)
+        if s not in self._subs:
+            y = self._run_sub(s)
+            if (y.N, y.H, y.W, y.cpitch) != (self.N, (self.H - 1) // s + 1, (self.W - 1) // s + 1, self.cpitch) or not y.dense:
+                raise RuntimeError("deferred stage tail produced an unexpected shape")
+            self._subs[s] = y
+        return self._subs[s]
+
+    @property
+    def materialized(self) -> bool:
+        return self._full is not None
+
+    @property
+    def dtype(self):
+        return self._dtype
+
+    @property
+    def device(self):
+        return self._device
 
 
 def network_input(x: torch.Tensor, dtype: str) -> NHWC:
@@ -252,10 +303,10 @@
         return (dtype, cpitch, d.Cin, d.Cout, d.groups, d.out_dtype, d.pad_l & 1) + \
             tuple((t.data_ptr(), t._version) if t is not None else None for t in self._sources())
 
-    def desc(self, x: NHWC, act, post_act, has_res, out_code=None, logits=False, pad4=None) -> ConvDesc:
+    def desc(self, x: NHWC, act, post_act, has_res, out_code=None, logits=False, pad4=None, stride=None) -> ConvDesc:
         c = self.conv
         kh, kw = _pair(c.kernel_size)
-        sh, sw = _pair(c.stride)
+        sh, sw = _pair(c.stride) if stride is None else _pair(stride)
         dh, dw = _pair(c.dilation)
         pad4 = pad4 if pad4 is not None else self.pad4
         if pad4 is not None:
@@ -337,7 +388,8 @@
         self._foreign = False
         self._key = None
 
-    def run(self, x: NHWC, act=0, residual: NHWC | None = None, post_act=0, out_fp32=False, pad4=None, out=None, gate=None) -> NHWC:
+    def run(self, x: NHWC, act=0, residual: NHWC | None = None, post_act=0, out_fp32=False, pad4=None, out=None, gate=None,
+            stride=None) -> NHWC:
         if self.bn is not None and self.bn.training:
             raise RuntimeError("pytorchcv_amd is an inference path: call net.eval() first (BatchNorm is folded)")
         if isinstance(x, LazyNCHW) and not x.materialized and residual is None and out is None and gate is None and not out_fp32 \
@@ -345,8 +397,15 @@
             y = self._stem_from_nchw(x, act, pool=False)
             if y is not None:
                 return y
-        d = self.desc(x, act, post_act, residual is not None, out_code=0 if out_fp32 else None, logits=out_fp32, pad4=pad4)
-        self.prepare(x, d)
+        d = self.desc(x, act, post_act, residual is not None, out_code=0 if out_fp32 else None, logits=out_fp32, pad4=pad4,
+                      stride=stride)
+        own = d
+        if stride is not None and _pair(stride) != _pair(self.conv.stride):
+            own = self.desc(x, act, post_act, residual is not None, out_code=0 if out_fp32 else None, logits=out_fp32, pad4=pad4)
+            if own.stride_h != own.stride_w or self.depthwise:
+                raise RuntimeError("a stride override needs a dense convolution with a square stride")
+            d.pack_stride = own.stride_h
+        self.prepare(x, own)
         return self._launch(x, d, residual, out, gate)
 
     def _stem_from_nchw(self, x: "LazyNCHW", act: int, pool: bool):
@@ -466,7 +525,13 @@
             y = buf[:, :, :, coff:]
         else:
             y = torch.empty((x.N, Ho, Wo, d.Cout), dtype=out_dt, device=x.device)
-        if residual is not None:
+        if isinstance(residual, SampledNHWC) and residual.stride > 1:
+            if (residual.N, residual.H, residual.W) != (x.N, Ho, Wo) or residual.dtype != x.dtype or self.depthwise or gate is not None or \
+                    tuple(residual.t.shape) != (x.N, residual.full_H, residual.full_W, d.Cout):
+                raise RuntimeError("strided residual shape/dtype mismatch: {} at stride {} vs {}".format(
+                    tuple(residual.t.shape), residual.stride, (x.N, Ho, Wo, d.Cout)))
+            d.res_stride, d.res_H, d.res_W = residual.stride, residual.full_H, residual.full_W
+        elif residual is not None:
             if not residual.dense or tuple(residual.t.shape) != (x.N, Ho, Wo, d.Cout) or residual.dtype != x.dtype:
                 raise RuntimeError("residual shape/dtype mismatch: {} vs {}".format(
                     tuple(residual.t.shape), (x.N, Ho, Wo, d.Cout)))
@@ -623,6 +688,7 @@
 
 FP32_HEAD = os.environ.get("PCV_AMD_FP32_HEAD", "1") != "0"
 STEM_FROM_NCHW = os.environ.get("PCV_AMD_STEM_NCHW", "1") != "0"
+STAGE_TAIL_SUBSAMPLE = os.environ.get("PCV_AMD_STAGE_TAIL", "1") != "0"
 
 
 FUSE_UNITS = os.environ.get("PCV_AMD_FUSE_UNITS", "1") != "0"
diff --git a/pytorchcv_amd/models/common/conv.py b/pytorchcv_amd/models/common/conv.py
--- a/pytorchcv_amd/models/common/conv.py
+++ b/pytorchcv_amd/models/common/conv.py
@@ -54,13 +54,13 @@
                 assert isinstance(self.activ, nn.Module)
         self._pcv_runner = None
 
-    def forward(self, x, residual=None, post_act=None, pad4=None, out=None):
+    def forward(self, x, residual=None, post_act=None, pad4=None, out=None, stride=None):
         if self._pcv_runner is None:
             self._pcv_runner = engine.ConvRunner(self.conv, self.bn if self.normalize else None, pad4=self._pad4)
         act = engine.act_code(self.activ) if self.activate else 0
         pact = engine.act_code(post_act)
         return engine.boundary(self, x, lambda a: self._pcv_runner.run(a, act=act, residual=residual, post_act=pact,
-                                                                       pad4=pad4, out=out))
+                                                                       pad4=pad4, out=out, stride=stride))
 
 
 def conv_block_maxpool(block, x, pool):
diff --git a/pytorchcv_amd/models/resnet.py b/pytorchcv_amd/models/resnet.py
--- a/pytorchcv_amd/models/resnet.py
+++ b/pytorchcv_amd/models/resnet.py
@@ -3,12 +3,19 @@
            'resnet34', 'resnetbc38b', 'resnet50', 'resnet50b', 'resnet101', 'resnet101b', 'resnet152', 'resnet152b',
            'ResBlock', 'ResBottleneck', 'ResUnit', 'ResStage', 'ResInitBlock', 'get_resnet']
 
+import torch
 import torch.nn as nn
 from .common.activ import lambda_relu
 from .common.norm import lambda_batchnorm2d
 from .common.conv import conv1x1_block, conv3x3_block, conv7x7_block, conv_block_pair, conv_block_maxpool
 from ._tail import MaxPool2dNHWC, AvgPool2dNHWC, LinearHead, run_net, maybe_load_pretrained, init_conv_params, DEFAULT_ROOT
 from .. import engine
+
+
+def _plain_conv(block, k, stride, pad):
+    c = getattr(block, "conv", None)
+    return c is not None and not block.use_pad and tuple(c.kernel_size) == (k, k) and tuple(c.stride) == (stride, stride) and \
+        tuple(c.padding) == (pad, pad) and tuple(c.dilation) == (1, 1) and c.groups == 1
 
 
 class ResBlock(nn.Module):
@@ -66,7 +73,16 @@
 
     def run_chained(self, a, conv1_out=None, next_unit=None):
         body = self.body
-        y = body.conv2(conv1_out if conv1_out is not None else body.conv1(a))
+        s1 = None
+        if isinstance(a, engine.LazyStageTail) and self.reads_every_second_pixel():
+            a, s1 = a.subsampled(2), 1
+        if next_unit is None and self.tail_deferrable(a):
+            return self._deferred_tail(a, conv1_out), None
+        y = body.conv2(conv1_out if conv1_out is not None else body.conv1(a, stride=s1))
+        if s1 is not None:
+            identity = self.identity_conv(a, stride=s1)
+            pair = conv_block_pair(body.conv3, y, identity, self.activ, next_unit.body.conv1) if next_unit is not None else None
+            return pair if pair is not None else (body.conv3(y, residual=identity, post_act=self.activ), None)
         if next_unit is not None and self.resize_identity:
             pair = conv_block_pair(body.conv3, y, None, self.activ, next_unit.body.conv1, id_block=self.identity_conv, x0=a)
             if pair is not None:
@@ -77,6 +93,30 @@
             if pair is not None:
                 return pair
         return body.conv3(y, residual=identity, post_act=self.activ), None
+
+    def reads_every_second_pixel(self) -> bool:
+        return engine.STAGE_TAIL_SUBSAMPLE and self.resize_identity and isinstance(self.body, ResBottleneck) and \
+            _plain_conv(self.body.conv1, 1, 2, 0) and _plain_conv(self.identity_conv, 1, 2, 0)
+
+    def tail_deferrable(self, a) -> bool:
+        body = self.body
+        return engine.STAGE_TAIL_SUBSAMPLE and engine.FUSE_UNITS and isinstance(body, ResBottleneck) and isinstance(a, engine.NHWC) and \
+            a.dense and _plain_conv(body.conv2, 3, 1, 1) and _plain_conv(body.conv3, 1, 1, 0) and \
+            (not self.resize_identity or _plain_conv(self.identity_conv, 1, 1, 0)) and \
+            (a.dtype != torch.float32) and body.conv3.conv.out_channels % 8 == 0
+
+    def _deferred_tail(self, a, conv1_out):
+        unit, blk = self, self.body
+        y1 = conv1_out if conv1_out is not None else blk.conv1(a)
+        identity = unit.identity_conv(a) if unit.resize_identity else a
+
+        def full():
+            return blk.conv3(blk.conv2(y1), residual=identity, post_act=unit.activ)
+
+        def sub(s):
+            return blk.conv3(blk.conv2(y1, stride=s), residual=engine.SampledNHWC(identity, s), post_act=unit.activ)
+        cout = blk.conv3.conv.out_channels
+        return engine.LazyStageTail(y1.N, y1.H, y1.W, cout, engine.round8(cout), y1.dtype, y1.device, full, sub)
 
     def forward(self, x):
         return engine.boundary(self, x, self._run)
```

After: 105,700 images/sec (median of 6 runs). 9.9% higher.
